# FedericoCos/PathTracer_GaussianSplatting

Hardware: AMD Instinct MI355X
Metric: Mrays/s (path trace) + Gsplats/s (3DGS) at 1920×1080, 1/2/4/8 MI355X (higher is better)
Workload: dtype f32; 1 GPU; C3 path trace: 250000-tri Sponza-like atrium, 1920x1080, 64 spp per GPU; width=1920, height=1080, spp_per_gpu=64, triangles=250000, bvh_nodes=58627, bvh_depth=13, bvh_build=host binned SAH, 113.1 ms, parallelism=single GPU

## Files before the change

include/ptgs/ptgs.h:

```cpp
#ifndef PTGS_H_
#define PTGS_H_

#include <stddef.h>
#include <stdint.h>

#ifdef __cplusplus
extern "C" {
#endif

#define PTGS_ABI_VERSION 4

#define PTGS_OK 0
#define PTGS_EINVAL (-1)
#define PTGS_EHIP (-2)
#define PTGS_ENOSCENE (-3)
#define PTGS_ERANGE (-4)
#define PTGS_EIO (-5)
#define PTGS_EINCOMPLETE (-6)
#define PTGS_EBADIDS (-7)


typedef struct ptgs_vertex {
    float pos[3];
    float pad1;
// ... 128 lines not shown
PTGS_AT(ptgs_material, uv_albedo, 144);
PTGS_AT(ptgs_material, emissive_factor_and_pad, 208);
PTGS_AT(ptgs_material, metallic_factor, 224);
PTGS_AT(ptgs_material, roughness_factor, 228);
PTGS_AT(ptgs_material, occlusion_strength, 232);
PTGS_AT(ptgs_material, specular_factor, 236);
PTGS_AT(ptgs_material, specular_color_factor, 240);
PTGS_AT(ptgs_material, alpha_cutoff, 252);
PTGS_AT(ptgs_material, transmission_factor, 256);
PTGS_AT(ptgs_material, clearcoat_factor, 260);
PTGS_AT(ptgs_material, clearcoat_roughness_factor, 264);
PTGS_AT(ptgs_material, pad, 268);
PTGS_AT(ptgs_material, albedo_texture_index, 272);
PTGS_AT(ptgs_material, normal_texture_index, 276);
PTGS_AT(ptgs_material, metallic_roughness_texture_index, 280);
PTGS_AT(ptgs_material, emissive_texture_index, 284);
PTGS_AT(ptgs_material, occlusion_texture_index, 288);
PTGS_AT(ptgs_material, clearcoat_texture_index, 292);
PTGS_AT(ptgs_material, clearcoat_roughness_texture_index, 296);
PTGS_AT(ptgs_material, sg_id, 300);
PTGS_AT(ptgs_material, use_specular_glossiness_workflow, 304);
PTGS_LAYOUT_ASSERT(sizeof(ptgs_ubo) == 192, "UniformBufferObject is 192 B");
PTGS_AT(ptgs_ubo, view, 0);
PTGS_AT(ptgs_ubo, proj, 64);
PTGS_AT(ptgs_ubo, camera_pos, 128);
PTGS_AT(ptgs_ubo, frame_count, 140);
PTGS_AT(ptgs_ubo, ambient_light, 144);
PTGS_AT(ptgs_ubo, emissive_flux, 160);
PTGS_AT(ptgs_ubo, punctual_flux, 164);
PTGS_AT(ptgs_ubo, total_flux, 168);
PTGS_AT(ptgs_ubo, p_emissive, 172);
PTGS_AT(ptgs_ubo, fov, 176);
PTGS_AT(ptgs_ubo, height, 180);
PTGS_AT(ptgs_ubo, use_lod, 184);
PTGS_AT(ptgs_ubo, lod_factor, 188);
PTGS_LAYOUT_ASSERT(sizeof(ptgs_punctual_light) == 64, "PunctualLight is 64 B");
PTGS_AT(ptgs_punctual_light, position, 0);
PTGS_AT(ptgs_punctual_light, intensity, 12);
PTGS_AT(ptgs_punctual_light, color, 16);
PTGS_AT(ptgs_punctual_light, range, 28);
PTGS_AT(ptgs_punctual_light, direction, 32);
PTGS_AT(ptgs_punctual_light, outer_cone_cos, 44);
PTGS_AT(ptgs_punctual_light, inner_cone_cos, 48);
PTGS_AT(ptgs_punctual_light, type, 52);
PTGS_AT(ptgs_punctual_light, padding, 56);
PTGS_LAYOUT_ASSERT(sizeof(ptgs_mesh_info) == 16, "MeshInfo is 16 B");
PTGS_AT(ptgs_mesh_info, material_index, 0);
PTGS_AT(ptgs_mesh_info, vertex_offset, 4);
PTGS_AT(ptgs_mesh_info, index_offset, 8);
PTGS_LAYOUT_ASSERT(sizeof(ptgs_light_triangle) == 16, "LightTriangle is 16 B");
PTGS_AT(ptgs_light_triangle, material_index, 12);
PTGS_LAYOUT_ASSERT(sizeof(ptgs_light_cdf) == 16, "LightCDF is 16 B");
PTGS_AT(ptgs_light_cdf, triangle_index, 4);
PTGS_LAYOUT_ASSERT(sizeof(ptgs_punctual_cdf) == 16, "PunctualLightCDF is 16 B");
PTGS_AT(ptgs_punctual_cdf, light_index, 4);
PTGS_LAYOUT_ASSERT(sizeof(ptgs_hitdata) == 48, "HitDataGPU is 48 B");
PTGS_AT(ptgs_hitdata, pos, 0);
PTGS_AT(ptgs_hitdata, flag, 12);
PTGS_AT(ptgs_hitdata, color, 16);
PTGS_AT(ptgs_hitdata, normal, 32);
PTGS_AT(ptgs_hitdata, padding, 44);
PTGS_LAYOUT_ASSERT(sizeof(ptgs_ray_sample) == 8, "RaySample is 8 B");
PTGS_LAYOUT_ASSERT(sizeof(ptgs_ray_push) == 80, "RayPushConstant / PC is 80 B");
PTGS_AT(ptgs_ray_push, model, 0);
PTGS_AT(ptgs_ray_push, mode, 64);
PTGS_AT(ptgs_ray_push, major_radius, 68);
PTGS_AT(ptgs_ray_push, minor_radius, 72);
PTGS_AT(ptgs_ray_push, height, 76);
#undef PTGS_AT


typedef struct ptgs_texture {
    const uint8_t* rgba8;
    uint32_t width;
    uint32_t height;
    uint32_t srgb;
    uint32_t reserved;
} ptgs_texture;

typedef struct ptgs_scene_desc {
    const ptgs_vertex* vertices;
    uint32_t num_vertices;
    const uint32_t* indices;
    uint32_t num_indices;
    const ptgs_mesh_info* meshes;
    const uint32_t* mesh_index_count;
    uint32_t num_meshes;
    const ptgs_material* materials;
    uint32_t num_materials;
    const ptgs_light_triangle* light_triangles;
    uint32_t num_light_triangles;
    const ptgs_light_cdf* light_cdf;
    uint32_t num_light_cdf;
    const ptgs_punctual_light* punctual_lights;
    uint32_t num_punctual_lights;
    const ptgs_punctual_cdf* punctual_cdf;
    uint32_t num_punctual_cdf;
    const float* blue_noise_rgba32f;
    uint32_t blue_noise_size;
    const ptgs_texture* textures;
    uint32_t num_textures;
} ptgs_scene_desc;

typedef struct ptgs_scene_info {
    uint32_t num_triangles;
    uint32_t num_bvh_nodes;
    uint32_t bvh_depth;
    uint32_t max_leaf_size;
    double build_ms;
    uint64_t device_bytes;
} ptgs_scene_info;


typedef struct ptgs_ctx ptgs_ctx;

int ptgs_create(int hip_device, ptgs_ctx** out);
void ptgs_destroy(ptgs_ctx* ctx);
const char* ptgs_last_error(const ptgs_ctx* ctx);
int ptgs_abi_version(void);
const char* ptgs_device_arch(void);

int ptgs_scene_upload(ptgs_ctx* ctx, const ptgs_scene_desc* desc);
int ptgs_scene_get_info(const ptgs_ctx* ctx, ptgs_scene_info* out);
typedef struct ptgs_bvh_buffers {
    const float* nodes;
    uint32_t num_nodes;
    const float* triangles;
    uint32_t num_triangles;
} ptgs_bvh_buffers;
int ptgs_scene_get_bvh(const ptgs_ctx* ctx, ptgs_bvh_buffers* out);
#define PTGS_BUILDER_HOST_SAH 0u
#define PTGS_BUILDER_GPU_SAH 1u
#define PTGS_BUILDER_GPU_LBVH 2u
typedef struct ptgs_scene_build {
    uint32_t builder;
    uint32_t leaf, fan;
    uint32_t depth_budget;
    uint32_t stack_need;
    uint32_t deep_stack;
} ptgs_scene_build;
int ptgs_scene_get_build(const ptgs_ctx* ctx, ptgs_scene_build* out);
typedef struct ptgs_scene_tree_opt {
    uint32_t applied;
    uint32_t num_nodes;
    uint32_t stack_need;
    uint32_t depth;
    uint32_t fan;
    uint32_t passes;
    double area_before;
    double area_after;
    double ms;
} ptgs_scene_tree_opt;
int ptgs_scene_get_tree_opt(const ptgs_ctx* ctx, ptgs_scene_tree_opt* out);


#define PTGS_ACCUM_RUNNING_MEAN 0u
#define PTGS_ACCUM_SUM 1u

int ptgs_trace_camera(ptgs_ctx* ctx, const ptgs_ubo* ubo, uint32_t width, uint32_t height,
                      float* accum_rgba32f, uint32_t spp, uint32_t frame_stride, uint32_t accum_mode,
                      void* hip_stream);

int ptgs_trace_camera_rows(ptgs_ctx* ctx, const ptgs_ubo* ubo, uint32_t width, uint32_t height,
                           uint32_t row_begin, uint32_t row_end, float* accum_rgba32f, uint32_t spp,
                           uint32_t frame_stride, uint32_t accum_mode, void* hip_stream);

int ptgs_trace_depth(ptgs_ctx* ctx, const ptgs_ubo* ubo, uint32_t width, uint32_t height, float* depth,
                     void* hip_stream);
int ptgs_trace_depth_rows(ptgs_ctx* ctx, const ptgs_ubo* ubo, uint32_t width, uint32_t height, uint32_t row_begin,
                          uint32_t row_end, float* depth, void* hip_stream);

int ptgs_trace_torus(ptgs_ctx* ctx, const ptgs_ubo* ubo, const ptgs_ray_push* push,
                     const ptgs_ray_sample* samples, uint32_t n, ptgs_hitdata* hits,
                     void* hip_stream);

typedef struct ptgs_trace_stats {
    uint64_t extension_rays;
    uint64_t shadow_rays;
    uint64_t samples;
    uint64_t node_visits;
    uint64_t tri_tests;
    uint64_t closest_hits;
} ptgs_trace_stats;

#define PTGS_FLAG_COUNT_TRAVERSAL 1u
#define PTGS_FLAG_TIME_STAGES 2u
#define PTGS_FLAG_GPU_BVH 4u
#define PTGS_FLAG_SPLAT_PUBLISH 8u
#define PTGS_FLAG_SPLAT_PUBLISH_TIGHT 64u
#define PTGS_FLAG_PT_WAVEFRONT 16u
#define PTGS_FLAG_GPU_LBVH 32u
#define PTGS_FLAG_SPLAT_OVERLAP 128u
int ptgs_set_flags(ptgs_ctx* ctx, uint32_t flags);
int ptgs_stats_reset(ptgs_ctx* ctx, void* hip_stream);
int ptgs_stats_read(ptgs_ctx* ctx, ptgs_trace_stats* out);


int ptgs_splat_points(ptgs_ctx* ctx, const ptgs_ubo* ubo, const ptgs_ray_push* push,
                      const ptgs_hitdata* hits, const ptgs_ray_sample* samples, uint32_t n,
                      uint32_t width, uint32_t height, uint32_t* rgba8_srgb, float* depth,
                      void* hip_stream);

typedef struct ptgs_gaussians {
    const float* means;
    const float* scales;
    const float* rotations;
    const float* opacities;
    const float* colors;
    uint32_t count;
    const uint32_t* ids;
    const float* chunk_bounds;
} ptgs_gaussians;

typedef struct ptgs_splat_stats {
    uint32_t num_rendered;
    uint32_t tiles_x, tiles_y;
    uint32_t num_visible;
    uint32_t fused;
} ptgs_splat_stats;

int ptgs_splat_gaussians(ptgs_ctx* ctx, const ptgs_gaussians* g, const ptgs_ubo* ubo,
                         uint32_t width, uint32_t height, const float bg[3],
                         uint32_t tile_row_begin, uint32_t tile_row_end, float* out_rgba32f,
                         ptgs_splat_stats* stats, void* hip_stream);

#define PTGS_MAX_VIEWS 8
int ptgs_splat_gaussians_views(ptgs_ctx* ctx, const ptgs_gaussians* g, uint32_t n_views, const ptgs_ubo* ubos,
                               uint32_t width, uint32_t height, const float bg[3], float* const* outs,
                               void* hip_stream);

int ptgs_gaussians_sort_spatial(ptgs_ctx* ctx, const ptgs_gaussians* g, float* means, float* scales, float* rotations,
                                float* opacities, float* colors, uint32_t* ids, void* hip_stream);

int ptgs_gaussians_chunk_bounds(ptgs_ctx* ctx, const ptgs_gaussians* g, float* bounds, void* hip_stream);

int ptgs_gaussians_sh_colors(ptgs_ctx* ctx, const float* means, const float* sh, uint32_t count,
                             uint32_t sh_degree, uint32_t active_degree, const float camera_pos[3],
                             float* colors, void* hip_stream);
int ptgs_gaussians_activate(ptgs_ctx* ctx, const float* log_scales, const float* opacity_logits,
                            uint32_t count, float* scales, float* opacities, void* hip_stream);
int ptgs_gaussians_sh_colors_backward(ptgs_ctx* ctx, const float* means, const float* sh, uint32_t count,
                                      uint32_t sh_degree, uint32_t active_degree, const float camera_pos[3],
                                      const float* dL_dcolors, float* dL_dsh, float* dL_dmeans, void* hip_stream);
int ptgs_gaussians_sh_colors_backward_eye(ptgs_ctx* ctx, const float* means, const float* sh, uint32_t count,
                                          uint32_t sh_degree, uint32_t active_degree, const float camera_pos[3],
                                          const float* dL_dcolors, float* dL_dsh, float* dL_dmeans,
                                          float* dL_dcamera_pos, void* hip_stream);
int ptgs_gaussians_activate_backward(ptgs_ctx* ctx, const float* scales, const float* opacities, uint32_t count,
                                     const float* dL_dscales, const float* dL_dopacities, float* dL_dlog_scales,
                                     float* dL_dlogits, void* hip_stream);
int ptgs_gaussians_permute_sh(ptgs_ctx* ctx, const float* sh, uint32_t sh_degree, const uint32_t* ids,
                              uint32_t count, float* out, void* hip_stream);

typedef struct ptgs_gaussian_grads {
    float* means;
    float* scales;
    float* rotations;
    float* opacities;
    float* colors;
    float* means2d;
    float* conics;
} ptgs_gaussian_grads;
int ptgs_splat_gaussians_backward(ptgs_ctx* ctx, const ptgs_gaussians* g, const ptgs_ubo* ubo,
                                  uint32_t width, uint32_t height, const float bg[3],
                                  const float* dL_dout_rgba32f, const ptgs_gaussian_grads* grads,
                                  void* hip_stream);

int ptgs_splat_gaussians_invdepth(ptgs_ctx* ctx, uint32_t width, uint32_t height, float* out_invdepth,
                                  void* hip_stream);
int ptgs_splat_gaussians_backward_depth(ptgs_ctx* ctx, const ptgs_gaussians* g, const ptgs_ubo* ubo,
                                        uint32_t width, uint32_t height, const float bg[3],
                                        const float* dL_dout_rgba32f, const float* dL_dinvdepth,
                                        const ptgs_gaussian_grads* grads, void* hip_stream);

int ptgs_splat_gaussians_backward_pose(ptgs_ctx* ctx, const ptgs_gaussians* g, const ptgs_ubo* ubo,
                                       uint32_t width, uint32_t height, const float bg[3],
                                       const float* dL_dout_rgba32f, const float* dL_dinvdepth,
                                       const ptgs_gaussian_grads* grads, float* dL_dview, void* hip_stream);

typedef struct ptgs_densify_params {
    float grad_threshold;
    float scale_split;
    float min_opacity;
    float max_scale;
    float max_screen_radius;
} ptgs_densify_params;
typedef struct ptgs_densify_counts {
    uint32_t survivors;
    uint32_t clones;
    uint32_t split_sources;
    uint32_t pruned_originals;
    uint32_t pruned_children;
    uint32_t total;
} ptgs_densify_counts;
typedef struct ptgs_densify_rows {
    const float* src;
    float* dst;
    uint32_t width;
    uint32_t zero_new;
} ptgs_densify_rows;
#define PTGS_DENSIFY_MAX_ROWS 16
int ptgs_densify_accumulate(ptgs_ctx* ctx, const float* g2d, const int32_t* radii, uint32_t n, uint32_t width,
                            uint32_t height, float* accum, float* denom, float* max_radii, void* hip_stream);
int ptgs_gaussians_densify_plan(ptgs_ctx* ctx, const float* scales, const float* opacities, const float* accum,
                                const float* denom, const float* max_radii, uint32_t n,
                                const ptgs_densify_params* params, ptgs_densify_counts* out, void* hip_stream);
// ... 128 lines not shown
```

pathtracer_gaussiansplatting_amd/_abi.py:

```python
from __future__ import annotations

import ctypes as C
import os

import numpy as np

ABI_VERSION = 4
_HERE = os.path.dirname(os.path.abspath(__file__))
LIB_PATH = os.path.join(_HERE, "libptgs.so")

PTGS_OK = 0
ERRORS = {-1: "PTGS_EINVAL", -2: "PTGS_EHIP", -3: "PTGS_ENOSCENE", -4: "PTGS_ERANGE", -5: "PTGS_EIO",
          -6: "PTGS_EINCOMPLETE", -7: "PTGS_EBADIDS"}
PTGS_EINVAL = -1
PTGS_EINCOMPLETE = -6
PTGS_EBADIDS = -7
ACCUM_RUNNING_MEAN = 0
ACCUM_SUM = 1
FLAG_COUNT_TRAVERSAL = 1
FLAG_TIME_STAGES = 2
FLAG_GPU_BVH = 4
FLAG_GPU_LBVH = 32
FLAG_SPLAT_PUBLISH = 8
FLAG_PT_WAVEFRONT = 16
# ... 47 lines not shown
                ("frame_count", C.c_uint32), ("ambient_light", C.c_float * 4), ("emissive_flux", C.c_float),
                ("punctual_flux", C.c_float), ("total_flux", C.c_float), ("p_emissive", C.c_float),
                ("fov", C.c_float), ("height", C.c_float), ("use_lod", C.c_float), ("lod_factor", C.c_float)]


class RayPush(C.Structure):
    _fields_ = [("model", C.c_float * 16), ("mode", C.c_int32), ("major_radius", C.c_float),
                ("minor_radius", C.c_float), ("height", C.c_float)]


class CaptureDesc(C.Structure):
    _fields_ = [("out_dir", C.c_char_p), ("width", C.c_uint32), ("height", C.c_uint32),
                ("total_positions", C.c_uint32), ("accumulation_steps", C.c_uint32), ("min_beta", C.c_float),
                ("max_beta", C.c_float), ("fov_deg", C.c_float), ("major_radius", C.c_float),
                ("torus_height", C.c_float), ("image_divisor", C.c_float), ("seed", C.c_uint32),
                ("capture_images", C.c_uint32), ("capture_pointcloud", C.c_uint32), ("ubo", C.c_void_p),
                ("torus", RayPush), ("samples", C.c_void_p), ("num_samples", C.c_uint32), ("hip_stream", C.c_void_p)]


class SceneDesc(C.Structure):
    _fields_ = [("vertices", C.c_void_p), ("num_vertices", C.c_uint32), ("indices", C.c_void_p),
                ("num_indices", C.c_uint32), ("meshes", C.c_void_p), ("mesh_index_count", C.c_void_p),
                ("num_meshes", C.c_uint32), ("materials", C.c_void_p), ("num_materials", C.c_uint32),
                ("light_triangles", C.c_void_p), ("num_light_triangles", C.c_uint32), ("light_cdf", C.c_void_p),
                ("num_light_cdf", C.c_uint32), ("punctual_lights", C.c_void_p), ("num_punctual_lights", C.c_uint32),
                ("punctual_cdf", C.c_void_p), ("num_punctual_cdf", C.c_uint32), ("blue_noise_rgba32f", C.c_void_p),
                ("blue_noise_size", C.c_uint32), ("textures", C.c_void_p), ("num_textures", C.c_uint32)]


class Texture(C.Structure):
    _fields_ = [("rgba8", C.c_void_p), ("width", C.c_uint32), ("height", C.c_uint32), ("srgb", C.c_uint32),
                ("reserved", C.c_uint32)]


class SceneSettings(C.Structure):
    _fields_ = [("ambient_light", C.c_float * 4), ("use_rt_box", C.c_int32), ("render_torus", C.c_int32),
                ("render_pointcloud", C.c_int32), ("torus_major_radius", C.c_float),
                ("torus_minor_radius", C.c_float), ("torus_height", C.c_float),
                ("torus_major_segments", C.c_int32), ("torus_minor_segments", C.c_int32),
                ("num_rays", C.c_uint32), ("use_lod", C.c_float), ("lod_factor", C.c_float),
                ("accumulation_steps", C.c_uint32), ("total_positions", C.c_uint32), ("min_beta", C.c_float),
                ("max_beta", C.c_float), ("image_divisor", C.c_float), ("capture_images", C.c_int32),
                ("capture_pointcloud", C.c_int32), ("num_objects", C.c_uint32)]


INGEST_MISSING_IMAGES_WHITE = 1


class SceneInfo(C.Structure):
    _fields_ = [("num_triangles", C.c_uint32), ("num_bvh_nodes", C.c_uint32), ("bvh_depth", C.c_uint32),
                ("max_leaf_size", C.c_uint32), ("build_ms", C.c_double), ("device_bytes", C.c_uint64)]


class TraceStats(C.Structure):
    _fields_ = [("extension_rays", C.c_uint64), ("shadow_rays", C.c_uint64), ("samples", C.c_uint64),
                ("node_visits", C.c_uint64), ("tri_tests", C.c_uint64), ("closest_hits", C.c_uint64)]


class Gaussians(C.Structure):
    _fields_ = [("means", C.c_void_p), ("scales", C.c_void_p), ("rotations", C.c_void_p),
                ("opacities", C.c_void_p), ("colors", C.c_void_p), ("count", C.c_uint32), ("ids", C.c_void_p),
                ("chunk_bounds", C.c_void_p)]


class GaussianGrads(C.Structure):
    _fields_ = [("means", C.c_void_p), ("scales", C.c_void_p), ("rotations", C.c_void_p),
                ("opacities", C.c_void_p), ("colors", C.c_void_p), ("means2d", C.c_void_p), ("conics", C.c_void_p)]


class DensifyParams(C.Structure):
    _fields_ = [("grad_threshold", C.c_float), ("scale_split", C.c_float), ("min_opacity", C.c_float),
                ("max_scale", C.c_float), ("max_screen_radius", C.c_float)]


class DensifyCounts(C.Structure):
    _fields_ = [("survivors", C.c_uint32), ("clones", C.c_uint32), ("split_sources", C.c_uint32),
                ("pruned_originals", C.c_uint32), ("pruned_children", C.c_uint32), ("total", C.c_uint32)]


class DensifyRows(C.Structure):
    _fields_ = [("src", C.c_void_p), ("dst", C.c_void_p), ("width", C.c_uint32), ("zero_new", C.c_uint32)]


DENSIFY_MAX_ROWS = 16


class AdamRows(C.Structure):
    _fields_ = [("param", C.c_void_p), ("grad", C.c_void_p), ("exp_avg", C.c_void_p), ("exp_avg_sq", C.c_void_p),
                ("width", C.c_uint32), ("head", C.c_uint32), ("lr", C.c_float), ("lr_head", C.c_float)]


class AdamParams(C.Structure):
    _fields_ = [("beta1", C.c_float), ("beta2", C.c_float), ("eps", C.c_float), ("step", C.c_uint32)]


ADAM_MAX_ROWS = 16


class SplatStats(C.Structure):
    _fields_ = [("num_rendered", C.c_uint32), ("tiles_x", C.c_uint32), ("tiles_y", C.c_uint32),
                ("num_visible", C.c_uint32), ("fused", C.c_uint32)]


class SplatStatus(C.Structure):
    _fields_ = [("frames", C.c_uint64), ("views", C.c_uint32 * 8), ("pair_capacity", C.c_uint32),
                ("last_pairs", C.c_uint32), ("touched_runs", C.c_uint32), ("fused", C.c_uint32),
                ("spilled_tiles", C.c_uint64), ("incomplete_tiles", C.c_uint64), ("spill_capacity", C.c_uint32),
                ("spill_demand", C.c_uint32)]


class SplatBuffers(C.Structure):
    _fields_ = [("radii", C.c_void_p), ("tiles_touched", C.c_void_p), ("sorted_keys", C.c_void_p),
                ("sorted_values", C.c_void_p), ("tile_ranges", C.c_void_p), ("means2d", C.c_void_p),
                ("depths", C.c_void_p), ("conic_opacity", C.c_void_p), ("num_gaussians", C.c_uint32),
                ("num_rendered", C.c_uint32), ("num_tiles", C.c_uint32)]


class BvhBuffers(C.Structure):
    _fields_ = [("nodes", C.c_void_p), ("num_nodes", C.c_uint32), ("triangles", C.c_void_p),
                ("num_triangles", C.c_uint32)]


BUILDER_HOST_SAH, BUILDER_GPU_SAH, BUILDER_GPU_LBVH = 0, 1, 2


class SceneBuild(C.Structure):
    _fields_ = [("builder", C.c_uint32), ("leaf", C.c_uint32), ("fan", C.c_uint32), ("depth_budget", C.c_uint32),
                ("stack_need", C.c_uint32), ("deep_stack", C.c_uint32)]


class SceneTreeOpt(C.Structure):
    _fields_ = [("applied", C.c_uint32), ("num_nodes", C.c_uint32), ("stack_need", C.c_uint32), ("depth", C.c_uint32),
                ("fan", C.c_uint32), ("passes", C.c_uint32), ("area_before", C.c_double), ("area_after", C.c_double),
                ("ms", C.c_double)]


assert C.sizeof(Ubo) == 192 and C.sizeof(RayPush) == 80

_P = C.c_void_p
_U = C.c_uint32
_I = C.c_int
_FP = C.POINTER(C.c_float)
SYMBOLS = {
    "ptgs_abi_version": (_I, []),
    "ptgs_device_arch": (C.c_char_p, []),
    "ptgs_create": (_I, [_I, C.POINTER(_P)]),
    "ptgs_destroy": (None, [_P]),
    "ptgs_last_error": (C.c_char_p, [_P]),
    "ptgs_scene_upload": (_I, [_P, C.POINTER(SceneDesc)]),
    "ptgs_scene_get_info": (_I, [_P, C.POINTER(SceneInfo)]),
    "ptgs_scene_get_bvh": (_I, [_P, C.POINTER(BvhBuffers)]),
    "ptgs_scene_get_build": (_I, [_P, C.POINTER(SceneBuild)]),
    "ptgs_scene_get_tree_opt": (_I, [_P, C.POINTER(SceneTreeOpt)]),
    "ptgs_trace_camera": (_I, [_P, C.POINTER(Ubo), _U, _U, _P, _U, _U, _U, _P]),
    "ptgs_trace_camera_rows": (_I, [_P, C.POINTER(Ubo), _U, _U, _U, _U, _P, _U, _U, _U, _P]),
    "ptgs_trace_torus": (_I, [_P, C.POINTER(Ubo), C.POINTER(RayPush), _P, _U, _P, _P]),
    "ptgs_trace_depth": (_I, [_P, C.POINTER(Ubo), _U, _U, _P, _P]),
    "ptgs_set_flags": (_I, [_P, _U]),
    "ptgs_stats_reset": (_I, [_P, _P]),
    "ptgs_stats_read": (_I, [_P, C.POINTER(TraceStats)]),
    "ptgs_splat_points": (_I, [_P, C.POINTER(Ubo), C.POINTER(RayPush), _P, _P, _U, _U, _U, _P, _P, _P]),
    "ptgs_splat_gaussians": (_I, [_P, C.POINTER(Gaussians), C.POINTER(Ubo), _U, _U, _FP, _U, _U, _P,
                                  C.POINTER(SplatStats), _P]),
    "ptgs_splat_gaussians_views": (_I, [_P, C.POINTER(Gaussians), _U, C.POINTER(Ubo), _U, _U, _FP,
                                        C.POINTER(C.c_void_p), _P]),
    "ptgs_splat_gaussians_over": (_I, [_P, C.POINTER(Gaussians), C.POINTER(Ubo), _U, _U, _P, _P, _U, _U, _P,
                                       C.POINTER(SplatStats), _P]),
    "ptgs_splat_get_buffers": (_I, [_P, C.POINTER(SplatBuffers)]),
    "ptgs_splat_get_tile_rows": (_I, [_P, C.POINTER(C.c_void_p), C.POINTER(C.c_uint32)]),
    "ptgs_splat_status_read": (_I, [_P, C.POINTER(SplatStatus), _P]),
    "ptgs_splat_reserve": (_I, [_P, _U]),
    "ptgs_gaussians_sort_spatial": (_I, [_P, C.POINTER(Gaussians), _P, _P, _P, _P, _P, _P, _P]),
    "ptgs_gaussians_chunk_bounds": (_I, [_P, C.POINTER(Gaussians), _P, _P]),
    "ptgs_gaussians_sh_colors": (_I, [_P, _P, _P, _U, _U, _U, _FP, _P, _P]),
    "ptgs_gaussians_activate": (_I, [_P, _P, _P, _U, _P, _P, _P]),
    "ptgs_gaussians_sh_colors_backward": (_I, [_P, _P, _P, _U, _U, _U, _FP, _P, _P, _P, _P]),
    "ptgs_gaussians_activate_backward": (_I, [_P, _P, _P, _U, _P, _P, _P, _P, _P]),
    "ptgs_gaussians_permute_sh": (_I, [_P, _P, _U, _P, _U, _P, _P]),
    "ptgs_splat_gaussians_backward": (_I, [_P, C.POINTER(Gaussians), C.POINTER(Ubo), _U, _U, _FP, _P,
                                           C.POINTER(GaussianGrads), _P]),
    "ptgs_splat_gaussians_invdepth": (_I, [_P, _U, _U, _P, _P]),
    "ptgs_splat_gaussians_backward_depth": (_I, [_P, C.POINTER(Gaussians), C.POINTER(Ubo), _U, _U, _FP, _P, _P,
                                                 C.POINTER(GaussianGrads), _P]),
    "ptgs_splat_gaussians_backward_pose": (_I, [_P, C.POINTER(Gaussians), C.POINTER(Ubo), _U, _U, _FP, _P, _P,
                                                C.POINTER(GaussianGrads), _P, _P]),
    "ptgs_gaussians_sh_colors_backward_eye": (_I, [_P, _P, _P, _U, _U, _U, _FP, _P, _P, _P, _P, _P]),
    "ptgs_densify_accumulate": (_I, [_P, _P, _P, _U, _U, _U, _P, _P, _P, _P]),
    "ptgs_gaussians_densify_plan": (_I, [_P, _P, _P, _P, _P, _P, _U, C.POINTER(DensifyParams),
                                         C.POINTER(DensifyCounts), _P]),
    "ptgs_gaussians_densify_apply": (_I, [_P, _U, _U, _P, _P, _P, _P, _P, _P, _P, C.POINTER(DensifyRows), _U, _P,
                                          _P]),
    "ptgs_image_loss_l1_dssim": (_I, [_P, _P, _P, _U, _U, _U, C.c_float, C.c_float, _P, _P, _P]),
    "ptgs_image_loss_invdepth_l1": (_I, [_P, _P, _P, _U, _U, C.c_float, C.c_float, _P, _P, _P]),
    "ptgs_gaussians_adam_step": (_I, [_P, _U, C.POINTER(AdamRows), _U, C.POINTER(AdamParams), _P, _P]),
    "ptgs_gaussians_opacity_reset": (_I, [_P, _P, _U, C.c_float, _P, _P, _P]),
    "ptgs_gaussians_checkpoint_init": (_I, [_P, _P, _P, _P, _U, _U, _P, _P, _P, _P]),
    "ptgs_image_mse": (_I, [_P, _P, _P, _U, _U, _U, _P, _P]),
    "ptgs_trace_depth_rows": (_I, [_P, C.POINTER(Ubo), _U, _U, _U, _U, _P, _P]),
    "ptgs_knn3_mean_dist2": (_I, [_P, _P, _U, _P, _P]),
    "ptgs_gaussians_from_points": (_I, [_P, _P, _P, _U, _P, _P, _P, _P, _P, _P]),
    "ptgs_comm_unique_id": (_I, [_P]),
    "ptgs_comm_create": (_I, [_P, _P, C.c_int, C.c_int]),
    "ptgs_comm_destroy": (_I, [_P]),
    "ptgs_reduce_radiance": (_I, [_P, _P, C.c_size_t, C.c_int, _P]),
    "ptgs_allreduce_radiance": (_I, [_P, _P, C.c_size_t, _P]),
    "ptgs_gather_rows": (_I, [_P, _P, C.c_uint32, C.c_uint32, _P, C.c_int, _P]),
    "ptgs_reduce_scatter_rows": (_I, [_P, _P, C.c_uint32, C.c_uint32, _P, _P]),
    "ptgs_splat_stage_ms": (_I, [_P, _FP]),
    "ptgs_encode_srgb8": (_I, [_P, _P, _U, _U, _P, _P]),
    "ptgs_device_alloc": (_I, [_P, C.c_size_t, C.POINTER(_P)]),
    "ptgs_device_free": (_I, [_P, _P]),
    "ptgs_memcpy_h2d": (_I, [_P, _P, _P, C.c_size_t]),
    "ptgs_memcpy_d2h": (_I, [_P, _P, _P, C.c_size_t]),
    "ptgs_memset_d32": (_I, [_P, _P, _U, C.c_size_t, _P]),
    "ptgs_synchronize": (_I, [_P]),
    "ptgs_camera_toroidal": (_I, [C.c_float] * 8 + [_FP, _FP, _FP]),
    "ptgs_camera_lookat": (_I, [_FP, _FP, _FP, _FP]),
    "ptgs_camera_perspective": (_I, [C.c_float] * 4 + [_FP]),
    "ptgs_mat4_inverse": (_I, [_FP, _FP]),
    "ptgs_mat4_inverse_glm": (_I, [_FP, _FP]),
    "ptgs_capture_poses": (_I, [_U, _U, C.c_float, C.c_float, _FP]),
    "ptgs_write_transforms_json": (_I, [C.c_char_p, C.c_float, C.c_float, _U, C.POINTER(C.c_char_p), _FP]),
    "ptgs_write_ply": (_I, [C.c_char_p, _P, _U, C.POINTER(C.c_uint32)]),
    "ptgs_write_jpeg": (_I, [C.c_char_p, _P, _U, _U, _U, C.c_int]),
    "ptgs_capture_dataset": (_I, [_P, _P]),
    "ptgs_builder_create": (_I, [C.POINTER(_P)]),
    "ptgs_builder_destroy": (None, [_P]),
    "ptgs_builder_add_rtbox_json": (_I, [_P, C.c_char_p]),
    "ptgs_builder_add_object": (_I, [_P, _P, _U, _P, _U, _P, _U, _P, _U, _P, _U, _U]),
    "ptgs_builder_finalize": (_I, [_P, C.POINTER(SceneDesc), C.POINTER(Ubo)]),
    "ptgs_builder_last_error": (C.c_char_p, [_P]),
    "ptgs_image_decode_rgba8": (_I, [_P, C.c_size_t, _P, C.c_size_t, C.POINTER(_U), C.POINTER(_U), C.POINTER(_U)]),
    "ptgs_read_ply": (_I, [C.c_char_p, _P, _P, _P, _U, C.POINTER(_U)]),
    "ptgs_read_gaussian_ply": (_I, [C.c_char_p, _P, _P, _P, _P, _P, _U, C.POINTER(_U), C.POINTER(_U)]),
    "ptgs_write_gaussian_ply": (_I, [C.c_char_p, _P, _P, _P, _P, _P, _U, _U]),
    "ptgs_generate_samples": (_I, [_I, _U, _P, _U, _P, _U, _U, _I, _P]),
    "ptgs_sort_samples": (_I, [_P, _U]),
    "ptgs_morton2d": (_U, [C.c_float, C.c_float]),
    "ptgs_builder_add_gltf": (_I, [_P, C.c_char_p, _FP, _FP, _FP, _U]),
    "ptgs_builder_add_punctual_light": (_I, [_P, _P]),
    "ptgs_builder_load_scene_json": (_I, [_P, C.c_char_p, C.c_char_p, _U, C.POINTER(SceneSettings)]),
}

_lib = None


class PtgsError(RuntimeError):
    def __init__(self, msg: str, code: int = 0):
        super().__init__(msg)
        self.code = code


def load_library(path: str | None = None) -> C.CDLL:
    global _lib
    if _lib is not None and path is None:
        return _lib
    p = path or LIB_PATH
    if not os.path.exists(p):
        raise PtgsError(f"native library not built: {p} (run pathtracer_gaussiansplatting_amd/build.py)")
    try:
        import torch
    except Exception:
        pass
    lib = C.CDLL(p, mode=C.RTLD_GLOBAL if path is None else C.RTLD_LOCAL)
    for name, (res, args) in SYMBOLS.items():
        fn = getattr(lib, name)
        fn.restype = res
        fn.argtypes = args
    v = lib.ptgs_abi_version()
    if v != ABI_VERSION:
        raise PtgsError(f"libptgs ABI version {v} != expected {ABI_VERSION}")
    if path is None:
        _lib = lib
    return lib


def check(rc: int, what: str, err: str = "") -> None:
    if rc != PTGS_OK:
        raise PtgsError(f"{what} failed: {ERRORS.get(rc, rc)} {err}", rc)


def fptr(a: np.ndarray):
    return a.ctypes.data_as(_FP)
```

pathtracer_gaussiansplatting_amd/csrc/api.cpp:

```cpp
#include <hip/hip_runtime.h>

#include <algorithm>
#include <chrono>
#include <cmath>
#include <cstdarg>
#include <cstdio>
#include <cstring>
#include <string>
#include <vector>

#include "../../include/ptgs/ptgs.h"
#include "bvh.h"
#include "bvh_gpu.h"
#include "bvh_opt.h"
#include "bvh_tries.h"
#include "knn.h"
#include "hostmath.h"
#include "pt_launch.h"
#include "pt_wavefront.h"
#include "scene_flatten.h"
#include "comm.h"
#include "dev_buf.h"
#include "splat.h"
#include "splat_adam.h"
#include "splat_adam_math.h"
#include "splat_backward.h"
#include "splat_densify.h"
#include "splat_frames.h"
#include "splat_loss.h"
#include "splat_sh.h"
#include "splat_train.h"
#include "textures.h"

using namespace ptgs;

static_assert(kSplatReportIncomplete == SPLAT_REPORT_INCOMPLETE && kSplatReportBadIds == SPLAT_REPORT_BAD_IDS,
              "splat_run.h names the bits of SplatReport");

struct ptgs_ctx {
  int device = 0;
  std::string err;
  uint32_t flags = 0;
  bool has_scene = false;
  DevScene dsc{};
  std::vector<void*> scene_allocs;
  ptgs_scene_info info{};
  ptgs_scene_build build{};
  ptgs_scene_tree_opt tree_opt{};
  unsigned long long* counters = nullptr;
  SplatFrames frames;
  DensifyWorkspace* densify = nullptr;
  LossWorkspace* loss = nullptr;
  ptgs::DevBuf sh_eye_partials;
  ptgs::DevBuf mse_partials;
  ptgs::WfWorkspace wf;
  ptgs::PtSched pt_sched;
  void* comm = nullptr;
  int comm_ranks = 0, comm_rank = 0;
};

namespace {

int fail(ptgs_ctx* c, int code, const char* fmt, ...) {
  char buf[512];
  va_list ap;
  va_start(ap, fmt);
  vsnprintf(buf, sizeof(buf), fmt, ap);
  va_end(ap);
  if (c) c->err = buf;
  return code;
}

#define HIPCHK(ctx, expr)                                                                   \
  do {                                                                                      \
    hipError_t e_ = (expr);                                                                 \
    if (e_ != hipSuccess) return fail(ctx, PTGS_EHIP, "%s: %s", #expr, hipGetErrorString(e_)); \
  } while (0)

int hip_rc(ptgs_ctx* c, hipError_t e, const char* what) {
  if (e != hipSuccess) return fail(c, PTGS_EHIP, "%s: %s", what, hipGetErrorString(e));
  return PTGS_OK;
}

int check_image_size(ptgs_ctx* c, uint32_t w, uint32_t h) {
  if (w == 0 || h == 0 || w > 32768 || h > 32768) return fail(c, PTGS_EINVAL, "bad image size %ux%u", w, h);
  return PTGS_OK;
}

int check_row_ranges(ptgs_ctx* c, const uint32_t* row_ranges, uint32_t height) {
  for (int g = 0; g < c->comm_ranks; ++g)
    if (row_ranges[2 * g] > row_ranges[2 * g + 1] || row_ranges[2 * g + 1] > height)
      return fail(c, PTGS_EINVAL, "bad row range of rank %d", g);
  return PTGS_OK;
}

void free_scene(ptgs_ctx* c) {
  for (void* p : c->scene_allocs) (void)hipFree(p);
  c->scene_allocs.clear();
  c->has_scene = false;
  c->dsc = DevScene{};
}

template <typename T>
int upload(ptgs_ctx* c, const T* src, size_t count, const T** dst) {
  if (count == 0) { *dst = nullptr; return PTGS_OK; }
  void* p = nullptr;
  HIPCHK(c, hipMalloc(&p, count * sizeof(T)));
  c->scene_allocs.push_back(p);
  HIPCHK(c, hipMemcpy(p, src, count * sizeof(T), hipMemcpyHostToDevice));
  c->info.device_bytes += count * sizeof(T);
  *dst = (const T*)p;
  return PTGS_OK;
}

bool is_device_ptr(const void* p) {
  if (!p) return false;
  hipPointerAttribute_t a;
  if (hipPointerGetAttributes(&a, p) != hipSuccess) { (void)hipGetLastError(); return false; }
  return a.type == hipMemoryTypeDevice || a.type == hipMemoryTypeManaged || a.devicePointer != nullptr;
}

int fill_cam(ptgs_ctx* c, const ptgs_ubo* ubo, CamParams& cp) {
  if (!inverse4(ubo->view, cp.inv_view)) return fail(c, PTGS_EINVAL, "ubo.view is singular");
  if (!inverse4(ubo->proj, cp.inv_proj)) return fail(c, PTGS_EINVAL, "ubo.proj is singular");
  for (int k = 0; k < 4; ++k) cp.ambient[k] = ubo->ambient_light[k];
  cp.emissive_flux = ubo->emissive_flux;
  cp.punctual_flux = ubo->punctual_flux;
  cp.p_emissive = ubo->p_emissive;
  cp.fov = ubo->fov;
  cp.win_height = ubo->height;
  cp.use_lod = ubo->use_lod;
  cp.lod_factor = ubo->lod_factor;
  return PTGS_OK;
}


void bvh_log(const char* how, const BvhTry& t, uint32_t depth, uint32_t need) {
  if (getenv("PTGS_BVH_LOG"))
    fprintf(stderr, "[ptgs] %s tree: leaf %d fan %d depth budget %u -> depth %u, stack need %u%s\n", how, t.leaf, t.fan,
            t.depth, depth, need, need >= PTGS_STACK ? (need < PTGS_STACK_TOTAL ? " (DEEP)" : " (does not fit)") : "");
}

double ms_between(std::chrono::steady_clock::time_point t0, std::chrono::steady_clock::time_point t1) {
  return std::chrono::duration<double, std::milli>(t1 - t0).count();
}

constexpr size_t kTriDeviceBytes = 3 * sizeof(float4) + sizeof(uint32_t);

struct HostSahBuilder {
  const std::vector<BuildTri>& tris;
  BvhOut bvh;
  std::vector<float> n4;
  uint32_t num4 = 0;
  BvhStep build(int leaf, uint32_t depth, uint32_t stack_lds) {
    build_bvh(tris, leaf, depth, bvh);
    return bvh.depth >= stack_lds ? BvhStep::TooDeep : BvhStep::Ok;
  }
  BvhStep collapse(int fan, uint32_t& need, uint32_t& depth4) {
    need = 0;
    collapse_bvh4(bvh.nodes, n4, num4, need, depth4, fan);
    return BvhStep::Ok;
  }
};

struct GpuTree {
  GpuBvh g;
  float4* n4 = nullptr;
  uint32_t num4 = 0;
  float ms = 0.0f;
  hipError_t err = hipSuccess;
  GpuTree() = default;
  GpuTree(const GpuTree&) = delete;
  GpuTree& operator=(const GpuTree&) = delete;
  ~GpuTree() {
    release_bvh2();
    (void)hipFree(n4);
  }
  void release_bvh2() {
    (void)hipFree(g.nodes);
    (void)hipFree(g.tris);
    (void)hipFree(g.tri_flags);
    g = GpuBvh{};
  }
  BvhStep step(hipError_t e) {
    err = e;
    return e == hipSuccess ? BvhStep::Ok : e == hipErrorNotSupported ? BvhStep::NotSupported : BvhStep::Error;
  }
  BvhStep collapse(int fan, uint32_t& need, uint32_t& depth4) {
    const auto t0 = std::chrono::steady_clock::now();
    (void)hipFree(n4);
    n4 = nullptr;
    const hipError_t e = collapse_bvh4_gpu(g.nodes, g.num_nodes, fan, &n4, &num4, &need, &depth4);
    ms += (float)ms_between(t0, std::chrono::steady_clock::now());
    return step(e);
  }
  void hand_over(std::vector<void*>& allocs, DevScene& s) {
    (void)hipFree(g.nodes);
    for (void* p : {(void*)n4, (void*)g.tris, (void*)g.tri_flags}) allocs.push_back(p);
    s.nodes = n4;
    s.tris = g.tris;
    s.tri_flags = g.tri_flags;
    n4 = nullptr;
    g = GpuBvh{};
  }
};
struct GpuSahBuilder : GpuTree {
  static constexpr uint32_t kId = PTGS_BUILDER_GPU_SAH;
  const std::vector<BuildTri>& tris;
  explicit GpuSahBuilder(const std::vector<BuildTri>& t) : tris(t) {}
  BvhStep build(int leaf, uint32_t depth, uint32_t) {
    release_bvh2();
    float bms = 0.0f;
    const hipError_t e = build_bvh_sah_gpu(tris, leaf, depth, g, &bms);
    ms += bms;
    return step(e);
  }
  uint32_t max_leaf() const { return g.max_leaf; }
};
struct GpuLbvhBuilder : GpuTree {
  static constexpr uint32_t kId = PTGS_BUILDER_GPU_LBVH;
  const std::vector<BuildTri>& tris;
  explicit GpuLbvhBuilder(const std::vector<BuildTri>& t) : tris(t) {}
  BvhStep build(int, uint32_t depth, uint32_t) {
    release_bvh2();
    float bms = 0.0f;
    const hipError_t e = build_bvh_gpu(tris, depth, g, &bms);
    ms += bms;
    return step(e);
  }
  uint32_t max_leaf() const { return 4u; }
};

void publish_tree(ptgs_ctx* c, DevScene& s, uint32_t builder, const BvhTriesResult& r, uint32_t num4, uint32_t max_leaf,
                  double build_ms) {
  s.deep_stack = r.need >= PTGS_STACK ? 1 : 0;
  c->info.num_bvh_nodes = num4;
  c->info.bvh_depth = r.depth4;
  c->info.max_leaf_size = max_leaf;
  c->info.build_ms = build_ms;
  c->build = ptgs_scene_build{builder, (uint32_t)r.kept.leaf, (uint32_t)r.kept.fan, r.kept.depth, r.need,
                              (uint32_t)s.deep_stack};
}

template <class Builder>
int build_tree_gpu(ptgs_ctx* c, const std::vector<BuildTri>& tris, const std::vector<BvhTry>& tries, DevScene& s,
                   bool* built) {
  Builder b(tris);
  const BvhTriesResult r =
      run_bvh_tries(b, tries, PTGS_STACK, PTGS_STACK_TOTAL,
                    [](const BvhTry& t, uint32_t depth4, uint32_t need) { bvh_log("GPU", t, depth4, need); });
  if (r.fit == BvhFit::Error) return fail(c, PTGS_EHIP, "GPU BVH build: %s", hipGetErrorString(b.err));
  if (r.fit != BvhFit::Fits) return PTGS_OK;
  publish_tree(c, s, Builder::kId, r, b.num4, b.max_leaf(), b.ms);
  c->info.device_bytes += (size_t)b.num4 * PTGS_NODE4_BYTES + tris.size() * kTriDeviceBytes;
  b.hand_over(c->scene_allocs, s);
  *built = true;
  return PTGS_OK;
}

int build_tree_host(ptgs_ctx* c, const std::vector<BuildTri>& tris, DevScene& s, std::vector<float>& host_n4) {
  const auto t0 = std::chrono::steady_clock::now();
  HostSahBuilder b{tris};
  const BvhTriesResult r =
      run_bvh_tries(b, parse_bvh_tries(getenv("PTGS_BVH_TRIES"), PTGS_STACK), PTGS_STACK, PTGS_STACK_TOTAL,
                    [](const BvhTry& t, uint32_t depth4, uint32_t need) { bvh_log("host", t, depth4, need); });
  const auto t1 = std::chrono::steady_clock::now();
  if (r.fit != BvhFit::Fits) return fail(c, PTGS_ERANGE, "BVH depth %u exceeds the traversal stack", b.bvh.depth);
  int rc;
  if ((rc = upload(c, (const float4*)b.n4.data(), b.n4.size() / 4, &s.nodes))) return rc;
  if ((rc = upload(c, (const float4*)b.bvh.tris.data(), b.bvh.tris.size() / 4, &s.tris))) return rc;
  if ((rc = upload(c, b.bvh.tri_flags.data(), b.bvh.tri_flags.size(), &s.tri_flags))) return rc;
  publish_tree(c, s, PTGS_BUILDER_HOST_SAH, r, b.num4, b.bvh.max_leaf, ms_between(t0, t1));
  host_n4.swap(b.n4);
  return PTGS_OK;
}

int check_node_window(ptgs_ctx* c) {
  const uint32_t limit = bvh_node_limit(getenv("PTGS_BVH_NODE_LIMIT"));
  if (c->info.num_bvh_nodes > limit)
    return fail(c, PTGS_ERANGE, "BVH of %u 4-wide nodes exceeds the traversal's 2 GiB node window (%u nodes)",
                c->info.num_bvh_nodes, limit);
  return PTGS_OK;
}

int upload_traversal_nodes(ptgs_ctx* c, std::vector<float>& host_n4, DevScene& s) {
  const size_t nf = (size_t)c->info.num_bvh_nodes * 32;
  if (host_n4.size() != nf) {
    host_n4.resize(nf);
    HIPCHK(c, hipMemcpy(host_n4.data(), s.nodes, nf * sizeof(float), hipMemcpyDeviceToHost));
  }
  int force = -1;
  if (const char* e = getenv("PTGS_PT_STACK_KEY_BITS")) force = std::max(0, atoi(e));
  bool optimise = c->build.builder != PTGS_BUILDER_GPU_LBVH;
  if (const char* e = getenv("PTGS_PT_TREE_OPT")) optimise = atoi(e) != 0;
  std::vector<uint32_t> n64;
  StackLayout sl;
  TreeOptInfo oi;
  if (!make_opt_traversal_nodes(host_n4.data(), c->info.num_bvh_nodes, (int)c->build.fan,
                                s.deep_stack ? PTGS_STACK_TOTAL : PTGS_STACK, optimise, force, n64, sl, oi))
    return fail(c, PTGS_ERANGE, "BVH node extents beyond the compact nodes' step range (2^-100 .. 2^100)");
  c->tree_opt = ptgs_scene_tree_opt{oi.applied, oi.num_nodes, oi.need, oi.depth, oi.fan, oi.passes,
                                    oi.area_before, oi.area_after, oi.ms};
  s.stk_key_mask = sl.key_mask;
  s.leaf_shift = sl.leaf_shift;
  s.leaf_start_mask = sl.leaf_start_mask;
  if (getenv("PTGS_BVH_LOG")) {
    if (optimise)
      fprintf(stderr, "[ptgs] traversal tree: %s in %.1f ms (%u passes): nodes %u -> %u, stack need %u -> %u, depth %u -> %u, "
              "fan %u, area sum %.3f -> %.3f\n", oi.applied ? "optimised" : "not applied", oi.ms, oi.passes,
              c->info.num_bvh_nodes, oi.num_nodes, c->build.stack_need, oi.need, c->info.bvh_depth, oi.depth, oi.fan,
              oi.area_before, oi.area_after);
    fprintf(stderr, "[ptgs] stack word:%u link bits, %u key bits (mask %08x), leaf shift %u\n", sl.ref_bits, sl.key_bits,
            sl.key_mask, sl.leaf_shift);
  }
  return upload(c, (const uint4*)n64.data(), n64.size() / 4, &s.nodes64);
}

int upload_scene_arrays(ptgs_ctx* c, const ptgs_scene_desc* d, const FlatScene& flat, const TexturePool& texpool,
                        DevScene& s) {
  int rc;
  ptgs_vertex dummy_v{};
  uint32_t dummy_i = 0;
  ptgs_mesh_info dummy_m{};
  if ((rc = upload(c, d->num_vertices ? d->vertices : &dummy_v, d->num_vertices ? d->num_vertices : 1, &s.vertices))) return rc;
  if ((rc = upload(c, d->num_indices ? d->indices : &dummy_i, d->num_indices ? d->num_indices : 1, &s.indices))) return rc;
  if ((rc = upload(c, d->num_meshes ? d->meshes : &dummy_m, d->num_meshes ? d->num_meshes : 1, &s.meshes))) return rc;
  if ((rc = upload(c, d->materials, d->num_materials, &s.materials))) return rc;
  const std::vector<uint32_t>& hitrec = flat.hitrec;
  const uint32_t zero4[4] = {0, 0, 0, 0};
  if ((rc = upload(c, (const uint4*)(hitrec.empty() ? zero4 : hitrec.data()), hitrec.empty() ? 1 : hitrec.size() / 4,
                   &s.hitrec)))
    return rc;
  if ((rc = upload(c, d->light_triangles, d->num_light_triangles, &s.light_tris))) return rc;
  if ((rc = upload(c, d->light_cdf, d->num_light_cdf, &s.light_cdf))) return rc;
  if ((rc = upload(c, d->punctual_lights, d->num_punctual_lights, &s.plights))) return rc;
  if ((rc = upload(c, d->punctual_cdf, d->num_punctual_cdf, &s.pcdf))) return rc;
  const size_t bn = d->blue_noise_size;
  if ((rc = upload(c, (const float4*)d->blue_noise_rgba32f, bn * bn, &s.blue_noise))) return rc;
  if ((rc = upload(c, texpool.texels.data(), texpool.texels.size(), &s.tex.texels))) return rc;
  if ((rc = upload(c, texpool.info.data(), texpool.info.size(), &s.tex.info))) return rc;
  return upload(c, texpool.lut.data(), texpool.lut.size(), &s.tex.lut);
}

void publish_scene(ptgs_ctx* c, const ptgs_scene_desc* d, const FlatScene& flat, DevScene& s) {
  s.tex.count = d->num_textures;
  s.uses_textures = 0;
  for (uint32_t i = 0; i < d->num_materials; ++i) {
    const ptgs_material& m = d->materials[i];
    if (m.albedo_texture_index > 0 || m.normal_texture_index > 0 || m.metallic_roughness_texture_index > 0 ||
        m.emissive_texture_index > 0 || m.clearcoat_texture_index > 0 || m.clearcoat_roughness_texture_index > 0 ||
        m.sg_id > 0)
      s.uses_textures = 1;
  }
  s.num_light_cdf = d->num_light_cdf;
  s.num_plights = d->num_punctual_lights;
  s.bn_size = (int32_t)d->blue_noise_size;
  s.has_transparent = flat.has_transparent ? 1 : 0;
  c->dsc = s;
  c->has_scene = true;
  c->info.num_triangles = (uint32_t)flat.tris.size();
}

}

extern "C" {

int ptgs_abi_version(void) { return PTGS_ABI_VERSION; }
const char* ptgs_device_arch(void) { return "gfx950"; }

int ptgs_create(int hip_device, ptgs_ctx** out) {
  if (!out) return PTGS_EINVAL;
  *out = nullptr;
  int n = 0;
  hipError_t e = hipGetDeviceCount(&n);
  if (e != hipSuccess || n == 0) return PTGS_EHIP;
  if (hip_device < 0 || hip_device >= n) return PTGS_EINVAL;
  ptgs_ctx* c = new ptgs_ctx();
  c->device = hip_device;
  if (hipSetDevice(hip_device) != hipSuccess) { delete c; return PTGS_EHIP; }
  if (hipMalloc(&c->counters, 8 * sizeof(unsigned long long)) != hipSuccess) { delete c; return PTGS_EHIP; }
  if (hipMemset(c->counters, 0, 8 * sizeof(unsigned long long)) != hipSuccess) { delete c; return PTGS_EHIP; }
  c->densify = densify_workspace_create();
  c->loss = loss_workspace_create();
  if (c->mse_partials.ensure(TRAIN_MSE_MAX_WG * sizeof(double), 0) != hipSuccess) {
    ptgs_destroy(c);
    return PTGS_EHIP;
  }
  *out = c;
  return PTGS_OK;
}

void ptgs_destroy(ptgs_ctx* c) {
  if (!c) return;
  (void)hipSetDevice(c->device);
  free_scene(c);
  if (c->counters) (void)hipFree(c->counters);
  ptgs::wf_workspace_free(c->wf);
  ptgs::free_pt_sched(c->pt_sched);
  densify_workspace_destroy(c->densify);
  loss_workspace_destroy(c->loss);
  if (c->comm) (void)comm_destroy(c->comm);
  delete c;
}

int ptgs_comm_unique_id(uint8_t id[PTGS_COMM_ID_BYTES]) {
  if (!id) return PTGS_EINVAL;
  if (!comm_available()) return PTGS_EHIP;
  return comm_unique_id(id) == 0 ? PTGS_OK : PTGS_EHIP;
}

int ptgs_comm_create(ptgs_ctx* c, const uint8_t id[PTGS_COMM_ID_BYTES], int nranks, int rank) {
  if (!c || !id) return PTGS_EINVAL;
  if (nranks < 1 || rank < 0 || rank >= nranks) return fail(c, PTGS_EINVAL, "bad rank %d of %d", rank, nranks);
  if (!comm_available()) return fail(c, PTGS_EHIP, "RCCL (librccl.so.1) could not be loaded");
  HIPCHK(c, hipSetDevice(c->device));
  if (c->comm) {
    (void)comm_destroy(c->comm);
    c->comm = nullptr;
  }
  int e = comm_create(id, nranks, rank, &c->comm);
  if (e) return fail(c, PTGS_EHIP, "ncclCommInitRank: %s", comm_error(e));
  c->comm_ranks = nranks;
  c->comm_rank = rank;
  return PTGS_OK;
}

int ptgs_comm_destroy(ptgs_ctx* c) {
  if (!c) return PTGS_EINVAL;
  if (c->comm) {
    int e = comm_destroy(c->comm);
    c->comm = nullptr;
    if (e) return fail(c, PTGS_EHIP, "ncclCommDestroy: %s", comm_error(e));
  }
  return PTGS_OK;
}

static int reduce_common(ptgs_ctx* c, float* accum, size_t n, int root, bool all, void* stream) {
  if (!c || !accum) return PTGS_EINVAL;
  if (!c->comm) return fail(c, PTGS_EINVAL, "no communicator (ptgs_comm_create)");
  if (!is_device_ptr(accum)) return fail(c, PTGS_EINVAL, "accum is not a device pointer");
  HIPCHK(c, hipSetDevice(c->device));
  int e = all ? comm_allreduce_sum(c->comm, accum, n, (hipStream_t)stream)
              : comm_reduce_sum(c->comm, accum, n, root, (hipStream_t)stream);
  if (e) return fail(c, PTGS_EHIP, "%s: %s", all ? "ncclAllReduce" : "ncclReduce", comm_error(e));
  return PTGS_OK;
}

int ptgs_reduce_radiance(ptgs_ctx* c, float* accum, size_t n_floats, int root, void* stream) {
  return reduce_common(c, accum, n_floats, root, false, stream);
}

int ptgs_allreduce_radiance(ptgs_ctx* c, float* accum, size_t n_floats, void* stream) {
  return reduce_common(c, accum, n_floats, 0, true, stream);
}

int ptgs_gather_rows(ptgs_ctx* c, float* image, uint32_t width, uint32_t height, const uint32_t* row_ranges,
                     int root, void* stream) {
  if (!c || !image || !row_ranges) return PTGS_EINVAL;
  if (!c->comm) return fail(c, PTGS_EINVAL, "no communicator (ptgs_comm_create)");
  if (root < 0 || root >= c->comm_ranks) return fail(c, PTGS_EINVAL, "bad root %d", root);
  if (!is_device_ptr(image)) return fail(c, PTGS_EINVAL, "image is not a device pointer");
  if (const int bad = check_row_ranges(c, row_ranges, height)) return bad;
  HIPCHK(c, hipSetDevice(c->device));
  int e = comm_gather_rows(c->comm, image, (size_t)width * 4u, row_ranges, c->comm_ranks, c->comm_rank, root,
                           (hipStream_t)stream);
  if (e) return fail(c, PTGS_EHIP, "ncclSend/ncclRecv: %s", comm_error(e));
  return PTGS_OK;
}

int ptgs_reduce_scatter_rows(ptgs_ctx* c, float* image, uint32_t width, uint32_t height, const uint32_t* row_ranges,
                             void* stream) {
  if (!c || !image || !row_ranges) return PTGS_EINVAL;
  if (!c->comm) return fail(c, PTGS_EINVAL, "no communicator (ptgs_comm_create)");
  if (!is_device_ptr(image)) return fail(c, PTGS_EINVAL, "image is not a device pointer");
  if (const int bad = check_row_ranges(c, row_ranges, height)) return bad;
  HIPCHK(c, hipSetDevice(c->device));
  int e = comm_reduce_rows(c->comm, image, (size_t)width * 4u, row_ranges, c->comm_ranks, (hipStream_t)stream);
  if (e) return fail(c, PTGS_EHIP, "ncclReduce: %s", comm_error(e));
  return PTGS_OK;
}

const char* ptgs_last_error(const ptgs_ctx* c) { return c ? c->err.c_str() : "null context"; }

int ptgs_scene_upload(ptgs_ctx* c, const ptgs_scene_desc* d) {
  if (!c || !d) return PTGS_EINVAL;
  HIPCHK(c, hipSetDevice(c->device));
  int rc;
  std::string msg;
  if ((rc = validate_scene_desc(d, msg))) return fail(c, rc, "%s", msg.c_str());
  TexturePool texpool;
  if (!build_texture_pool(d->textures, d->num_textures, texpool, msg)) return fail(c, PTGS_EINVAL, "%s", msg.c_str());
  if (texpool.texels.size() >= (1ull << 32)) return fail(c, PTGS_ERANGE, "texture pool exceeds 2^32 texels");
  FlatScene flat;
  if ((rc = flatten_scene(d, flat, msg))) return fail(c, rc, "%s", msg.c_str());

  free_scene(c);
  c->info = ptgs_scene_info{};
  c->build = ptgs_scene_build{};
  c->tree_opt = ptgs_scene_tree_opt{};
  DevScene s{};
  bool built = false;
  if ((c->flags & PTGS_FLAG_GPU_BVH) && flat.tris.size() >= 16) {
    rc = (c->flags & PTGS_FLAG_GPU_LBVH)
             ? build_tree_gpu<GpuLbvhBuilder>(c, flat.tris, lbvh_bvh_tries(PTGS_STACK), s, &built)
             : build_tree_gpu<GpuSahBuilder>(c, flat.tris, parse_bvh_tries(getenv("PTGS_BVH_TRIES"), PTGS_STACK), s,
                                             &built);
    if (rc) return rc;
  }
  std::vector<float> host_n4;
  if (!built && (rc = build_tree_host(c, flat.tris, s, host_n4))) return rc;
  if ((rc = check_node_window(c))) return rc;
  if ((rc = upload_traversal_nodes(c, host_n4, s))) return rc;
  if ((rc = upload_scene_arrays(c, d, flat, texpool, s))) return rc;
  publish_scene(c, d, flat, s);
  return PTGS_OK;
}

int ptgs_scene_get_info(const ptgs_ctx* c, ptgs_scene_info* out) {
  if (!c || !out) return PTGS_EINVAL;
  if (!c->has_scene) return PTGS_ENOSCENE;
  *out = c->info;
  return PTGS_OK;
}

int ptgs_scene_get_build(const ptgs_ctx* c, ptgs_scene_build* out) {
  if (!c || !out) return PTGS_EINVAL;
  if (!c->has_scene) return PTGS_ENOSCENE;
  *out = c->build;
  return PTGS_OK;
}

int ptgs_scene_get_tree_opt(const ptgs_ctx* c, ptgs_scene_tree_opt* out) {
  if (!c || !out) return PTGS_EINVAL;
  if (!c->has_scene) return PTGS_ENOSCENE;
  *out = c->tree_opt;
  return PTGS_OK;
}

int ptgs_scene_get_bvh(const ptgs_ctx* c, ptgs_bvh_buffers* out) {
  if (!c || !out) return PTGS_EINVAL;
  if (!c->has_scene) return PTGS_ENOSCENE;
  out->nodes = (const float*)c->dsc.nodes;
  out->num_nodes = c->info.num_bvh_nodes;
  out->triangles = (const float*)c->dsc.tris;
  out->num_triangles = c->info.num_triangles;
  return PTGS_OK;
}

int ptgs_trace_camera_rows(ptgs_ctx* c, const ptgs_ubo* ubo, uint32_t w, uint32_t h, uint32_t row_begin,
                           uint32_t row_end, float* accum, uint32_t spp, uint32_t frame_stride,
                           uint32_t accum_mode, void* stream) {
  if (!c || !ubo || !accum) return fail(c, PTGS_EINVAL, "null argument");
  if (!c->has_scene) return fail(c, PTGS_ENOSCENE, "no scene uploaded");
  if (const int bad = check_image_size(c, w, h)) return bad;
  if (row_end > h) row_end = h;
  if (row_begin > row_end) return fail(c, PTGS_EINVAL, "bad row range");
  if (frame_stride == 0) return fail(c, PTGS_EINVAL, "frame_stride must be >= 1");
  if (accum_mode > PTGS_ACCUM_SUM) return fail(c, PTGS_EINVAL, "bad accum mode");
  if (!is_device_ptr(accum)) return fail(c, PTGS_EINVAL, "accum is not a device pointer");
  HIPCHK(c, hipSetDevice(c->device));
  CamParams cp;
  int rc = fill_cam(c, ubo, cp);
  if (rc) return rc;
  const bool stats = (c->flags & PTGS_FLAG_COUNT_TRAVERSAL) != 0;
  hipError_t e;
  if (c->flags & PTGS_FLAG_PT_WAVEFRONT) {
    e = ptgs::launch_pt_wavefront(c->wf, c->dsc, cp, accum, w, h, row_begin, row_end, spp, ubo->frame_count,
                                  frame_stride, accum_mode, c->counters, stats, (hipStream_t)stream);
    return hip_rc(c, e, "wavefront path tracer");
  }
  e = launch_pt_camera(c->dsc, cp, accum, w, h, row_begin, row_end, spp, ubo->frame_count, frame_stride, accum_mode,
                       c->counters, stats, &c->pt_sched, (hipStream_t)stream);
  return hip_rc(c, e, "pt_camera launch");
}

int ptgs_trace_camera(ptgs_ctx* c, const ptgs_ubo* ubo, uint32_t w, uint32_t h, float* accum, uint32_t spp,
                      uint32_t frame_stride, uint32_t accum_mode, void* stream) {
  return ptgs_trace_camera_rows(c, ubo, w, h, 0, h, accum, spp, frame_stride, accum_mode, stream);
}

int ptgs_trace_depth(ptgs_ctx* c, const ptgs_ubo* ubo, uint32_t w, uint32_t h, float* depth, void* stream) {
  return ptgs_trace_depth_rows(c, ubo, w, h, 0, h, depth, stream);
}

int ptgs_trace_depth_rows(ptgs_ctx* c, const ptgs_ubo* ubo, uint32_t w, uint32_t h, uint32_t row_begin,
                          uint32_t row_end, float* depth, void* stream) {
  if (!c || !ubo || !depth) return fail(c, PTGS_EINVAL, "null argument");
  if (!c->has_scene) return fail(c, PTGS_ENOSCENE, "no scene uploaded");
  if (const int bad = check_image_size(c, w, h)) return bad;
  if (!is_device_ptr(depth)) return fail(c, PTGS_EINVAL, "depth is not a device pointer");
  HIPCHK(c, hipSetDevice(c->device));
  CamParams cp;
  int rc = fill_cam(c, ubo, cp);
  if (rc) return rc;
  ViewMat vm;
  std::memcpy(vm.m, ubo->view, sizeof(vm.m));
  hipError_t e = launch_pt_depth(c->dsc, cp, vm, depth, w, h, row_begin, row_end, ubo->frame_count, (hipStream_t)stream);
  return hip_rc(c, e, "pt_depth launch");
}

int ptgs_trace_torus(ptgs_ctx* c, const ptgs_ubo* ubo, const ptgs_ray_push* push, const ptgs_ray_sample* samples,
                     uint32_t n, ptgs_hitdata* hits, void* stream) {
  if (!c || !ubo || !push) return fail(c, PTGS_EINVAL, "null argument");
  if (!c->has_scene) return fail(c, PTGS_ENOSCENE, "no scene uploaded");
  if (n == 0) return PTGS_OK;
  if (!is_device_ptr(samples) || !is_device_ptr(hits)) return fail(c, PTGS_EINVAL, "samples/hits must be device pointers");
  HIPCHK(c, hipSetDevice(c->device));
  CamParams cp;
  int rc = fill_cam(c, ubo, cp);
  if (rc) return rc;
  TorusParams tp;
  std::memcpy(tp.model, push->model, sizeof(tp.model));
  tp.major_radius = push->major_radius;
  tp.minor_radius = push->minor_radius;
  tp.height = push->height;
  uint32_t side = (uint32_t)std::ceil(std::sqrt((double)n));
  while ((uint64_t)side * side < n) side++;
  hipError_t e = launch_pt_torus(c->dsc, cp, tp, samples, n, side, ubo->frame_count, hits, c->counters,
                                 (c->flags & PTGS_FLAG_COUNT_TRAVERSAL) != 0, (hipStream_t)stream);
  return hip_rc(c, e, "pt_torus launch");
}

int ptgs_set_flags(ptgs_ctx* c, uint32_t flags) {
  if (!c) return PTGS_EINVAL;
  c->flags = flags;
  return PTGS_OK;
}

int ptgs_stats_reset(ptgs_ctx* c, void* stream) {
  if (!c) return PTGS_EINVAL;
  HIPCHK(c, hipSetDevice(c->device));
  HIPCHK(c, hipMemsetAsync(c->counters, 0, 8 * sizeof(unsigned long long), (hipStream_t)stream));
  return PTGS_OK;
}

int ptgs_stats_read(ptgs_ctx* c, ptgs_trace_stats* out) {
  if (!c || !out) return PTGS_EINVAL;
  HIPCHK(c, hipSetDevice(c->device));
  HIPCHK(c, hipDeviceSynchronize());
  unsigned long long v[8];
  HIPCHK(c, hipMemcpy(v, c->counters, sizeof(v), hipMemcpyDeviceToHost));
  out->extension_rays = v[0];
  out->shadow_rays = v[1];
  out->samples = v[2];
  out->node_visits = v[3];
  out->tri_tests = v[4];
  out->closest_hits = v[5];
  return PTGS_OK;
}

int ptgs_device_alloc(ptgs_ctx* c, size_t bytes, void** out) {
  if (!c || !out) return PTGS_EINVAL;
  HIPCHK(c, hipSetDevice(c->device));
  HIPCHK(c, hipMalloc(out, bytes ? bytes : 16));
  return PTGS_OK;
}
int ptgs_device_free(ptgs_ctx* c, void* p) {
  if (!c) return PTGS_EINVAL;
  HIPCHK(c, hipFree(p));
  return PTGS_OK;
}
int ptgs_memcpy_h2d(ptgs_ctx* c, void* dst, const void* src, size_t bytes) {
  if (!c) return PTGS_EINVAL;
  HIPCHK(c, hipMemcpy(dst, src, bytes, hipMemcpyHostToDevice));
  return PTGS_OK;
}
int ptgs_memcpy_d2h(ptgs_ctx* c, void* dst, const void* src, size_t bytes) {
  if (!c) return PTGS_EINVAL;
  HIPCHK(c, hipMemcpy(dst, src, bytes, hipMemcpyDeviceToHost));
  return PTGS_OK;
}
int ptgs_memset_d32(ptgs_ctx* c, void* dst, uint32_t value, size_t count, void* stream) {
  if (!c) return PTGS_EINVAL;
  HIPCHK(c, hipMemsetD32Async((hipDeviceptr_t)dst, (int)value, count, (hipStream_t)stream));
  return PTGS_OK;
}
int ptgs_synchronize(ptgs_ctx* c) {
  if (!c) return PTGS_EINVAL;
  HIPCHK(c, hipDeviceSynchronize());
  return PTGS_OK;
}

}

#include "raster.h"

extern "C" {

// ... 767 lines not shown
```

pathtracer_gaussiansplatting_amd/csrc/bvh_opt.cpp:

```cpp
#include "bvh_opt.h"

#include <algorithm>
#include <chrono>
#include <cmath>
#include <cstring>
#include <limits>
#include <utility>

#include "bvh.h"

namespace ptgs {

namespace {

constexpr float kFar = 1e29f;

struct Node2 {
  float lo[3], hi[3];
  int32_t parent = -1;
  int32_t c[2] = {-1, -1};
  int32_t link = 0;
  bool leaf() const { return link < 0; }
};

// ... 20 lines not shown
  std::vector<double> area;
  int32_t root = -1;

  int32_t add(const Node2& x) {
    n.push_back(x);
    area.push_back(half_area(x.lo, x.hi));
    return (int32_t)n.size() - 1;
  }
  int32_t join(int32_t a, int32_t b) {
    Node2 x;
    for (int k = 0; k < 3; ++k) { x.lo[k] = std::min(n[a].lo[k], n[b].lo[k]); x.hi[k] = std::max(n[a].hi[k], n[b].hi[k]); }
    x.c[0] = a; x.c[1] = b;
    const int32_t i = add(x);
    n[a].parent = i; n[b].parent = i;
    return i;
  }
  void refit(int32_t x) {
    for (; x >= 0; x = n[x].parent) {
      Node2& p = n[x];
      const Node2 &a = n[p.c[0]], &b = n[p.c[1]];
      bool same = true;
      for (int k = 0; k < 3; ++k) {
        const float lo = std::min(a.lo[k], b.lo[k]), hi = std::max(a.hi[k], b.hi[k]);
        same = same && lo == p.lo[k] && hi == p.hi[k];
        p.lo[k] = lo; p.hi[k] = hi;
      }
      if (same) return;
      area[x] = half_area(p.lo, p.hi);
    }
  }
  void replace_child(int32_t parent, int32_t was, int32_t now) {
    if (parent < 0) root = now;
    else n[parent].c[n[parent].c[0] == was ? 0 : 1] = now;
    n[now].parent = parent;
  }
};

struct Binarise {
  const float* n4;
  uint32_t num;
  Tree2& t;
  std::vector<uint8_t> seen;
  bool ok = true;

  int32_t node(uint32_t i, uint32_t depth) {
    if (i >= num || seen[i] || depth > 4096) { ok = false; return -1; }
    seen[i] = 1;
    const float* f = n4 + 32 * (size_t)i;
    int32_t e[4];
    int cnt = 0;
    for (int j = 0; j < 4 && ok; ++j) {
      int32_t link;
      std::memcpy(&link, &f[24 + j], 4);
      if (link == 0) continue;
      if (link < 0) {
        if (!real_box(f, j)) { ok = false; break; }
        Node2 x;
        for (int a = 0; a < 3; ++a) { x.lo[a] = f[(2 * a) * 4 + j]; x.hi[a] = f[(2 * a + 1) * 4 + j]; }
        x.link = link;
        e[cnt++] = t.add(x);
      } else {
        e[cnt++] = node((uint32_t)link, depth + 1);
      }
    }
    if (!ok || cnt < 2) { ok = false; return -1; }
    while (cnt > 1) {
      int ba = 0, bb = 1;
      double best = std::numeric_limits<double>::infinity();
      for (int a = 0; a < cnt; ++a)
        for (int b = a + 1; b < cnt; ++b) {
          const double u = union_area(t.n[e[a]], t.n[e[b]]);
          if (u < best) { best = u; ba = a; bb = b; }
        }
      e[ba] = t.join(e[ba], e[bb]);
      for (int k = bb; k + 1 < cnt; ++k) e[k] = e[k + 1];
      --cnt;
    }
    return e[0];
  }
};

typedef std::pair<double, int32_t> Cand;

void reinsertion_pass(Tree2& t, std::vector<Cand>& heap) {
  std::vector<int32_t> order;
  order.reserve(t.n.size());
  for (int32_t i = 0; i < (int32_t)t.n.size(); ++i)
    if (i != t.root) order.push_back(i);
  std::sort(order.begin(), order.end(), [&](int32_t a, int32_t b) {
    return t.area[a] != t.area[b] ? t.area[a] > t.area[b] : a < b;
  });
  for (const int32_t x : order) {
    const int32_t p = t.n[x].parent;
    if (x == t.root || p == t.root) continue;
    const int32_t g = t.n[p].parent;
    const int32_t s = t.n[p].c[t.n[p].c[0] == x ? 1 : 0];
    t.replace_child(g, p, s);
    t.refit(g);
    const double ax = t.area[x];
    double best = union_area(t.n[s], t.n[x]);
    for (int32_t a = g; a >= 0; a = t.n[a].parent) best += union_area(t.n[a], t.n[x]) - t.area[a];
    int32_t at = s;
    heap.clear();
    heap.push_back(Cand(0.0, t.root));
    while (!heap.empty()) {
      std::pop_heap(heap.begin(), heap.end(), std::greater<Cand>());
      const Cand c = heap.back();
      heap.pop_back();
      if (c.first + ax >= best) break;
      const Node2& y = t.n[c.second];
      const double cost = c.first + union_area(y, t.n[x]);
      if (cost < best) { best = cost; at = c.second; }
      const double below = cost - t.area[c.second];
      if (!y.leaf() && below + ax < best)
        for (int k = 0; k < 2; ++k) {
          heap.push_back(Cand(below, y.c[k]));
          std::push_heap(heap.begin(), heap.end(), std::greater<Cand>());
        }
    }
    t.replace_child(t.n[at].parent, at, p);
    t.n[p].c[0] = at; t.n[p].c[1] = x;
    t.n[at].parent = p; t.n[x].parent = p;
    for (int k = 0; k < 3; ++k) { t.n[p].lo[k] = 1.0f; t.n[p].hi[k] = 0.0f; }
    t.refit(p);
  }
}

void emit_bvh2(const Tree2& t, std::vector<float>& n2) {
  std::vector<int32_t> queue;
  queue.push_back(t.root);
  std::vector<int32_t> index(t.n.size(), -1);
  index[t.root] = 0;
  for (size_t q = 0; q < queue.size(); ++q)
    for (int k = 0; k < 2; ++k) {
      const int32_t c = t.n[queue[q]].c[k];
      if (t.n[c].leaf()) continue;
      index[c] = (int32_t)queue.size();
      queue.push_back(c);
    }
  n2.assign(queue.size() * 16, 0.0f);
  for (size_t q = 0; q < queue.size(); ++q) {
    float* f = &n2[16 * q];
    const Node2& p = t.n[queue[q]];
    for (int k = 0; k < 2; ++k) {
      const Node2& c = t.n[p.c[k]];
      f[4 * k + 0] = c.lo[0]; f[4 * k + 1] = c.hi[0]; f[4 * k + 2] = c.lo[1]; f[4 * k + 3] = c.hi[1];
      f[8 + 2 * k] = c.lo[2]; f[9 + 2 * k] = c.hi[2];
      const int32_t link = c.leaf() ? c.link : index[p.c[k]];
      std::memcpy(&f[12 + k], &link, 4);
    }
  }
}

}

double bvh4_area_sum(const float* n4, uint32_t num) {
  double sum = 0.0, root = 0.0;
  for (uint32_t i = 0; i < num; ++i) {
    const float* f = n4 + 32 * (size_t)i;
    float lo[3] = {1.0f, 1.0f, 1.0f}, hi[3] = {0.0f, 0.0f, 0.0f};
    bool any = false;
    for (int j = 0; j < 4; ++j) {
      int32_t link;
      std::memcpy(&link, &f[24 + j], 4);
      if (link == 0 || !real_box(f, j)) continue;
      for (int a = 0; a < 3; ++a) {
        const float l = f[(2 * a) * 4 + j], h = f[(2 * a + 1) * 4 + j];
        lo[a] = any ? std::min(lo[a], l) : l;
        hi[a] = any ? std::max(hi[a], h) : h;
      }
      any = true;
    }
    const double a = any ? half_area(lo, hi) : 0.0;
    if (i == 0) root = a;
    sum += a;
  }
  return root > 0.0 ? sum / root : 0.0;
}

bool optimize_bvh4(const float* n4, uint32_t num, int fan, uint32_t need_limit, std::vector<float>& out,
                   TreeOptInfo& info, int passes) {
  const auto t0 = std::chrono::steady_clock::now();
  info = TreeOptInfo{};
  out.clear();
  info.area_before = bvh4_area_sum(n4, num);
  auto done = [&](bool applied) {
    info.applied = applied ? 1u : 0u;
    if (!applied) out.clear();
    info.ms = std::chrono::duration<double, std::milli>(std::chrono::steady_clock::now() - t0).count();
    return applied;
  };
  if (num == 0) return done(false);
  Tree2 t;
  t.n.reserve((size_t)num * 8);
  t.area.reserve((size_t)num * 8);
  Binarise b{n4, num, t, std::vector<uint8_t>(num, 0)};
  t.root = b.node(0, 0);
  if (!b.ok) return done(false);
  std::vector<Cand> heap;
  for (int p = 0; p < passes; ++p) reinsertion_pass(t, heap);
  info.passes = (uint32_t)std::max(0, passes);
  std::vector<float> n2;
  emit_bvh2(t, n2);
  for (int f = std::max(2, std::min(4, fan)); f >= 2; --f) {
    uint32_t num4 = 0, need = 0, depth4 = 0;
    collapse_bvh4(n2, out, num4, need, depth4, f);
    if (need >= need_limit) continue;
    info.num_nodes = num4;
    info.need = need;
    info.depth = depth4;
    info.fan = (uint32_t)f;
    info.area_after = bvh4_area_sum(out.data(), num4);
    return done(true);
  }
  return done(false);
}

bool make_opt_traversal_nodes(const float* n4, uint32_t num, int fan, uint32_t need_limit, bool optimise,
                              int force_key_bits, std::vector<uint32_t>& n64, StackLayout& layout, TreeOptInfo& info,
                              std::vector<float>* walked) {
  info = TreeOptInfo{};
  std::vector<float> opt;
  if (optimise && optimize_bvh4(n4, num, fan, need_limit, opt, info)) {
    if (make_traversal_nodes(opt.data(), info.num_nodes, force_key_bits, n64, layout)) {
      if (walked) walked->swap(opt);
      return true;
    }
    info.applied = 0;
  }
  if (!optimise) info.area_before = bvh4_area_sum(n4, num);
  if (walked) walked->assign(n4, n4 + (size_t)num * 32);
  return make_traversal_nodes(n4, num, force_key_bits, n64, layout);
}

}
```

pathtracer_gaussiansplatting_amd/csrc/bvh_opt.h:

```cpp
#pragma once

#include <stdint.h>
#include <vector>

#include "bvh.h"

namespace ptgs {

constexpr int kTreeOptPasses = 2;

struct TreeOptInfo {
  uint32_t applied = 0;
  uint32_t num_nodes = 0;
  uint32_t need = 0;
  uint32_t depth = 0;
  uint32_t fan = 0;
  uint32_t passes = 0;
  double area_before = 0.0;
  double area_after = 0.0;
  double ms = 0.0;
};

double bvh4_area_sum(const float* nodes4, uint32_t num_nodes);

bool optimize_bvh4(const float* nodes4, uint32_t num_nodes, int fan, uint32_t need_limit, std::vector<float>& out,
                   TreeOptInfo& info, int passes = kTreeOptPasses);

bool make_opt_traversal_nodes(const float* nodes4, uint32_t num_nodes, int fan, uint32_t need_limit, bool optimise,
                              int force_key_bits, std::vector<uint32_t>& nodes64, StackLayout& layout, TreeOptInfo& info,
                              std::vector<float>* walked = nullptr);

}
```

pathtracer_gaussiansplatting_amd/csrc/pt_device.h:

```cpp
#pragma once

#include <hip/hip_runtime.h>
#include "detmath.h"
#include "texture.h"
#include "stack_key.h"
#include "../../include/ptgs/ptgs.h"

namespace ptgs {

struct DevScene {
  const float4* nodes;
  const uint4* nodes64;
  const float4* tris;
  const uint32_t* tri_flags;
  const ptgs_vertex* vertices;
  const uint32_t* indices;
  const ptgs_mesh_info* meshes;
  const ptgs_material* materials;
  const uint4* hitrec;
  const ptgs_light_triangle* light_tris;
  const ptgs_light_cdf* light_cdf;
  const ptgs_punctual_light* plights;
  const ptgs_punctual_cdf* pcdf;
  const float4* blue_noise;
  DevTextures tex;
  int32_t uses_textures;
  int32_t deep_stack;
  uint32_t num_light_cdf;
  uint32_t num_plights;
  int32_t bn_size;
  int32_t has_transparent;
  uint32_t stk_key_mask;
  uint32_t leaf_shift;
  uint32_t leaf_start_mask;
};

struct CamParams {
  float inv_view[16];
  float inv_proj[16];
  float ambient[4];
  float emissive_flux, punctual_flux, p_emissive;
  float fov, win_height, use_lod, lod_factor;
};

struct Hit {
  float t, u, v;
  uint32_t gid;
  uint32_t slot;
};

struct TraversalCounters {
  uint32_t nodes;
  uint32_t tris;
  uint32_t hits;
#ifdef PT_LANES
  struct PtLaneCounts* lanes_p;
#endif
};

enum PtLoop { PT_L_NODE = 0, PT_L_LEAF, PT_L_TRI, PT_L_ANY_NODE, PT_L_ANY_TRI, PT_L_BOUNCE, PT_L_SAMPLE, PT_L_COUNT };
#ifdef PT_LANES
__device__ unsigned long long g_pt_lanes[2 * PT_L_COUNT];
struct PtLaneCounts {
  uint32_t w[PT_L_COUNT], l[PT_L_COUNT];
};
__device__ __forceinline__ void pt_lane_tick(PtLaneCounts& c, int i) {
  const unsigned long long ex = __builtin_amdgcn_read_exec();
  c.l[i] += 1u;
  if (__lane_id() == (uint32_t)__builtin_ctzll(ex)) c.w[i] += 1u;
}
__device__ __forceinline__ void pt_lanes_flush(const PtLaneCounts& c) {
  for (int i = 0; i < PT_L_COUNT; ++i) {
    atomicAdd(&g_pt_lanes[2 * i], (unsigned long long)c.w[i]);
    atomicAdd(&g_pt_lanes[2 * i + 1], (unsigned long long)c.l[i]);
  }
}
#define PT_LANE_TICK(cnt, i) pt_lane_tick(*(cnt).lanes_p, (i))
#define PT_LANES_INIT(tc) PtLaneCounts tc##_lanes = {}; (tc).lanes_p = &tc##_lanes
#define PT_LANES_FLUSH(tc) pt_lanes_flush(tc##_lanes)
#else
#define PT_LANE_TICK(cnt, i) ((void)0)
#define PT_LANES_INIT(tc) ((void)0)
#define PT_LANES_FLUSH(tc) ((void)0)
#endif

#ifndef PTGS_STACK
#define PTGS_STACK 39
#endif
#ifndef PTGS_STACK_OVF
#define PTGS_STACK_OVF 9
#endif
#define PTGS_STACK_TOTAL (PTGS_STACK + PTGS_STACK_OVF)
#define PTGS_BLOCK 256

PTGS_HD float i2f(int x) { union { int i; float f; } c; c.i = x; return c.f; }
__device__ __forceinline__ int f2i(float x) { return __float_as_int(x); }
__device__ __forceinline__ uint32_t f2u(float x) { return __float_as_uint(x); }

__device__ __forceinline__ float rnd(uint32_t& state) {
  uint32_t prev = state;
  state = prev * 747796405u + 2891336453u;
  uint32_t word = ((state >> ((state >> 28u) + 4u)) ^ state) * 277803737u;
  return (float)((word >> 22u) ^ word) / 4294967296.0f;
}

__device__ __forceinline__ float alpha_hash(uint32_t seed, uint32_t gid) {
  uint32_t s = seed ^ (gid * 0x9E3779B9u);
  return rnd(s);
}

__device__ __forceinline__ v3 ld3(const float* p) { return mk3(p[0], p[1], p[2]); }

#ifndef PTGS_PT_NEARFAR
#define PTGS_PT_NEARFAR 1
#endif
#ifndef PTGS_PT_ASM_MIN
#define PTGS_PT_ASM_MIN 1
#endif

struct Ray {
  v3 o, d, inv;
  v3 oinv;
  float tmin, tmax;
#if PTGS_PT_NEARFAR
  uint32_t nx, ny, nz;
#endif
};

__device__ __forceinline__ float safe_inv(float d) {
  const float eps = 1e-20f;
  float a = absx(d) < eps ? (d < 0.0f ? -eps : eps) : d;
  return 1.0f / a;
}

__device__ __forceinline__ Ray make_ray(v3 o, v3 d, float tmin, float tmax) {
  Ray r; r.o = o; r.d = d; r.tmin = tmin; r.tmax = tmax;
  r.inv = mk3(safe_inv(d.x), safe_inv(d.y), safe_inv(d.z));
  r.oinv = mk3(o.x * r.inv.x, o.y * r.inv.y, o.z * r.inv.z);
#if PTGS_PT_NEARFAR
  r.nx = r.inv.x < 0.0f ? 16u : 0u;
  r.ny = r.inv.y < 0.0f ? 48u : 32u;
  r.nz = r.inv.z < 0.0f ? 80u : 64u;
#endif
  return r;
}

__device__ __forceinline__ bool tri_isect(const Ray& r, v3 v0, v3 e1, v3 e2, float& t, float& u, float& v) {
  v3 pvec = cross3(r.d, e2);
  float det = dot3(e1, pvec);
  if (det == 0.0f) return false;
  float inv_det = 1.0f / det;
  v3 tvec = r.o - v0;
  u = dot3(tvec, pvec) * inv_det;
  if (u < 0.0f || u > 1.0f) return false;
  v3 qvec = cross3(tvec, e1);
  v = dot3(r.d, qvec) * inv_det;
  if (v < 0.0f || u + v > 1.0f) return false;
  t = dot3(e2, qvec) * inv_det;
  return true;
}

template <bool TEX>
__device__ __forceinline__ bool anyhit_accept(const DevScene& sc, uint32_t mesh, uint32_t prim, float u, float v,
                                              uint32_t seed, uint32_t gid) {
  const ptgs_mesh_info info = sc.meshes[mesh];
  const ptgs_material& m = sc.materials[info.material_index];
  float alpha_cutoff = m.alpha_cutoff;
  bool is_blend = m.pad > 0.5f;
  if (alpha_cutoff == 0.0f && !is_blend) return true;
  float alpha = m.base_color_factor[3];
  if (TEX && m.albedo_texture_index > 0) {
    const uint32_t i0 = sc.indices[info.index_offset + prim * 3u + 0u];
    const uint32_t i1 = sc.indices[info.index_offset + prim * 3u + 1u];
    const uint32_t i2 = sc.indices[info.index_offset + prim * 3u + 2u];
    const ptgs_vertex& v0 = sc.vertices[info.vertex_offset + i0];
    const ptgs_vertex& v1 = sc.vertices[info.vertex_offset + i1];
    const ptgs_vertex& v2 = sc.vertices[info.vertex_offset + i2];
    const float bx = (1.0f - u) - v;
    const float tu = (v0.tex_coord[0] * bx + v1.tex_coord[0] * u) + v2.tex_coord[0] * v;
    const float tv = (v0.tex_coord[1] * bx + v1.tex_coord[1] * u) + v2.tex_coord[1] * v;
    alpha = alpha * sample_texture(sc.tex, m.albedo_texture_index, tu, tv, 0.0f).w;
  }
  if (alpha_cutoff > 0.0f) return !(alpha < alpha_cutoff);
  return !(alpha_hash(seed, gid) > alpha);
}

__device__ __noinline__ bool anyhit_accept_call(const DevScene& sc, uint32_t mesh, uint32_t prim, float u, float v,
                                                uint32_t seed, uint32_t gid) {
  return anyhit_accept<true>(sc, mesh, prim, u, v, seed, gid);
}

template <bool PK>
__device__ __forceinline__ void leaf_range(const DevScene& sc, int leaf, uint32_t& start, uint32_t& count) {
  if (PK) {
    start = (uint32_t)leaf & sc.leaf_start_mask;
    count = (((uint32_t)leaf & 0x7fffffffu) >> sc.leaf_shift) + 1u;
  } else {
    const uint32_t L = (uint32_t)(~leaf);
    start = L & 0x07ffffffu;
    count = (L >> 27) + 1u;
  }
}

template <bool STATS, bool TEX, bool AH_CALL = false, bool PK = false>
__device__ __forceinline__ void leaf_closest(const DevScene& sc, const Ray& r, int leaf, Hit& h,
                                             uint32_t seed, TraversalCounters& cnt) {
  uint32_t start, count;
  leaf_range<PK>(sc, leaf, start, count);
  float4 na = sc.tris[3u * start], nb = sc.tris[3u * start + 1u], nc = sc.tris[3u * start + 2u];
  for (uint32_t k = 0; k < count; ++k) {
    PT_LANE_TICK(cnt, PT_L_TRI);
    float4 a = na, b = nb, c = nc;
    asm volatile("" : "+v"(a.x), "+v"(a.y), "+v"(a.z), "+v"(a.w), "+v"(b.x), "+v"(b.y), "+v"(b.z), "+v"(b.w),
                      "+v"(c.x), "+v"(c.y), "+v"(c.z), "+v"(c.w));
    if (k + 1 < count) {
      const float4* tn = sc.tris + 3u * (start + k + 1u);
      na = tn[0]; nb = tn[1]; nc = tn[2];
    }
    if (STATS) cnt.tris++;
    float t, u, v;
    if (!tri_isect(r, mk3(a.x, a.y, a.z), mk3(b.x, b.y, b.z), mk3(c.x, c.y, c.z), t, u, v)) continue;
    if (!(t >= r.tmin && t <= h.t)) continue;
    uint32_t gid = f2u(c.w);
    if (t == h.t && gid >= h.gid) continue;
    if (sc.has_transparent && (sc.tri_flags[start + k] & 1u)) {
      const bool acc = (AH_CALL && TEX) ? anyhit_accept_call(sc, f2u(a.w), f2u(b.w), u, v, seed, gid)
                                        : anyhit_accept<TEX>(sc, f2u(a.w), f2u(b.w), u, v, seed, gid);
      if (!acc) continue;
    }
    h.t = t; h.u = u; h.v = v; h.gid = gid; h.slot = start + k;
  }
}

struct Box4 {
  float tn[4];
  int c[4];
  unsigned long long hm[4];
};
#if PTGS_PT_NEARFAR
__device__ __forceinline__ float4 node_ld(__amdgpu_buffer_rsrc_t rs, uint32_t off) {
  typedef unsigned int u4 __attribute__((ext_vector_type(4)));
  const u4 v = __builtin_amdgcn_raw_buffer_load_b128(rs, (int)off, 0, 0);
  return make_float4(__uint_as_float(v.x), __uint_as_float(v.y), __uint_as_float(v.z), __uint_as_float(v.w));
}
__device__ __forceinline__ void box4(const Ray& r, const DevScene& sc, int node, float tcap, Box4& o) {
// ... 41 lines not shown
#pragma unroll
  for (int j = 0; j < 4; ++j) {
    const float x0 = __builtin_fmaf(LX[j], r.inv.x, -r.oinv.x), x1 = __builtin_fmaf(HX[j], r.inv.x, -r.oinv.x);
    const float y0 = __builtin_fmaf(LY[j], r.inv.y, -r.oinv.y), y1 = __builtin_fmaf(HY[j], r.inv.y, -r.oinv.y);
    const float z0 = __builtin_fmaf(LZ[j], r.inv.z, -r.oinv.z), z1 = __builtin_fmaf(HZ[j], r.inv.z, -r.oinv.z);
    const float tn = fmaxf(fmaxf(fminf(x0, x1), fminf(y0, y1)), fmaxf(fminf(z0, z1), r.tmin));
    const float tf = fminf(fminf(fmaxf(x0, x1), fmaxf(y0, y1)), fminf(fmaxf(z0, z1), tcap));
    const bool h = tn <= tf * 1.0000004f;
    o.tn[j] = h ? tn : __builtin_huge_valf();
    o.c[j] = f2i(CH[j]);
    o.hm[j] = __builtin_amdgcn_ballot_w64(h);
  }
}
#endif
#ifndef PTGS_PT_NODE64
#define PTGS_PT_NODE64 1
#endif
#ifndef PTGS_PT_NODE64_PIN
#define PTGS_PT_NODE64_PIN 1
#endif
#ifndef PTGS_PT_PK_SLAB
#define PTGS_PT_PK_SLAB 0
#endif
#ifndef PTGS_PT_PK_SLAB_MUL
#define PTGS_PT_PK_SLAB_MUL 1
#endif
template <bool N64>
__device__ __forceinline__ Ray node64_ray(const Ray& r) {
  Ray q = r;
  if (N64 && PTGS_PT_NODE64_PIN) asm volatile("" : "+v"(q.oinv.x), "+v"(q.oinv.y), "+v"(q.oinv.z));
  return q;
}
__device__ __forceinline__ float node64_q(uint32_t w, int j) { return (float)((w >> (8 * j)) & 0xffu); }
__device__ __forceinline__ void box4_q(const Ray& r, const DevScene& sc, int node, float tcap, Box4& o) {
  typedef unsigned int u4 __attribute__((ext_vector_type(4)));
  const __amdgpu_buffer_rsrc_t rs = __builtin_amdgcn_make_buffer_rsrc((void*)sc.nodes64, 0, 0x7fffffff, 0x00020000);
  const uint32_t base = (uint32_t)node << 6;
  const u4 a = __builtin_amdgcn_raw_buffer_load_b128(rs, (int)base, 0, 0);
  const u4 b = __builtin_amdgcn_raw_buffer_load_b128(rs, (int)(base + 16u), 0, 0);
  const u4 p = __builtin_amdgcn_raw_buffer_load_b128(rs, (int)(base + 32u), 0, 0);
  u4 ch = __builtin_amdgcn_raw_buffer_load_b128(rs, (int)(base + 48u), 0, 0);
  asm volatile("" : "+v"(ch.x), "+v"(ch.y), "+v"(ch.z), "+v"(ch.w));
  const float sx = __uint_as_float(a.w) * r.inv.x, sy = __uint_as_float(b.x) * r.inv.y, sz = __uint_as_float(b.y) * r.inv.z;
  const float cx = __builtin_fmaf(__uint_as_float(a.x), r.inv.x, -r.oinv.x);
  const float cy = __builtin_fmaf(__uint_as_float(a.y), r.inv.y, -r.oinv.y);
  const float cz = __builtin_fmaf(__uint_as_float(a.z), r.inv.z, -r.oinv.z);
#if PTGS_PT_NEARFAR
  const bool gx = (r.nx & 16u) != 0u, gy = (r.ny & 16u) != 0u, gz = (r.nz & 16u) != 0u;
#else
  const bool gx = r.inv.x < 0.0f, gy = r.inv.y < 0.0f, gz = r.inv.z < 0.0f;
#endif
  const uint32_t nX = gx ? b.w : b.z, fX = gx ? b.z : b.w;
  const uint32_t nY = gy ? p.y : p.x, fY = gy ? p.x : p.y;
  const uint32_t nZ = gz ? p.w : p.z, fZ = gz ? p.z : p.w;
  const uint32_t CH[4] = {ch.x, ch.y, ch.z, ch.w};
#if PTGS_PT_PK_SLAB
  typedef float f2 __attribute__((ext_vector_type(2)));
  const f2 SX = {sx, sx}, SY = {sy, sy}, SZ = {sz, sz}, CX = {cx, cx}, CY = {cy, cy}, CZ = {cz, cz};
  float TN[4], TF[4];
#pragma unroll
  for (int j = 0; j < 4; ++j) {
    const f2 qx = {node64_q(nX, j), node64_q(fX, j)}, qy = {node64_q(nY, j), node64_q(fY, j)};
    const f2 qz = {node64_q(nZ, j), node64_q(fZ, j)};
    const f2 x = __builtin_elementwise_fma(qx, SX, CX);
    const f2 y = __builtin_elementwise_fma(qy, SY, CY);
    const f2 z = __builtin_elementwise_fma(qz, SZ, CZ);
    TN[j] = fmaxf(fmaxf(x.x, y.x), fmaxf(z.x, r.tmin));
#if PTGS_PT_ASM_MIN
    float tf;
    asm("v_min3_f32 %0, %1, %2, %3" : "=v"(tf) : "v"(x.y), "v"(y.y), "v"(z.y));
    asm("v_min_f32 %0, %1, %2" : "=v"(tf) : "v"(tf), "v"(tcap));
    TF[j] = tf;
#else
    TF[j] = fminf(fminf(x.y, y.y), fminf(z.y, tcap));
#endif
  }
#if PTGS_PT_PK_SLAB_MUL
  const f2 K = {1.0000004f, 1.0000004f};
  const f2 f01 = (f2){TF[0], TF[1]} * K, f23 = (f2){TF[2], TF[3]} * K;
  const float TFK[4] = {f01.x, f01.y, f23.x, f23.y};
#else
  const float TFK[4] = {TF[0] * 1.0000004f, TF[1] * 1.0000004f, TF[2] * 1.0000004f, TF[3] * 1.0000004f};
#endif
#pragma unroll
  for (int j = 0; j < 4; ++j) {
    unsigned long long hm = __builtin_amdgcn_ballot_w64(TN[j] <= TFK[j]);
    if (j >= 2) hm &= __builtin_amdgcn_ballot_w64(CH[j] != 0u);
    o.tn[j] = __builtin_amdgcn_inverse_ballot_w64(hm) ? TN[j] : __builtin_huge_valf();
    o.c[j] = (int)CH[j];
    o.hm[j] = hm;
  }
#else
#pragma unroll
  for (int j = 0; j < 4; ++j) {
    const float x0 = __builtin_fmaf(node64_q(nX, j), sx, cx), x1 = __builtin_fmaf(node64_q(fX, j), sx, cx);
    const float y0 = __builtin_fmaf(node64_q(nY, j), sy, cy), y1 = __builtin_fmaf(node64_q(fY, j), sy, cy);
    const float z0 = __builtin_fmaf(node64_q(nZ, j), sz, cz), z1 = __builtin_fmaf(node64_q(fZ, j), sz, cz);
    const float tn = fmaxf(fmaxf(x0, y0), fmaxf(z0, r.tmin));
#if PTGS_PT_ASM_MIN
    float tf;
    asm("v_min3_f32 %0, %1, %2, %3" : "=v"(tf) : "v"(x1), "v"(y1), "v"(z1));
    asm("v_min_f32 %0, %1, %2" : "=v"(tf) : "v"(tf), "v"(tcap));
#else
    const float tf = fminf(fminf(x1, y1), fminf(z1, tcap));
#endif
    unsigned long long hm = __builtin_amdgcn_ballot_w64(tn <= tf * 1.0000004f);
    if (j >= 2) hm &= __builtin_amdgcn_ballot_w64(CH[j] != 0u);
    o.tn[j] = __builtin_amdgcn_inverse_ballot_w64(hm) ? tn : __builtin_huge_valf();
    o.c[j] = (int)CH[j];
    o.hm[j] = hm;
  }
#endif
}
template <bool N64>
__device__ __forceinline__ void box4_sel(const Ray& r, const DevScene& sc, int node, float tcap, Box4& o) {
  if (N64) box4_q(r, sc, node, tcap, o);
  else box4(r, sc, node, tcap, o);
}
__device__ __forceinline__ void cswap4(Box4& b, int i, int j) {
  const bool sw = b.tn[j] < b.tn[i];
  const float ti = b.tn[i], tj = b.tn[j];
  const int ci = b.c[i], cj = b.c[j];
  b.tn[i] = sw ? tj : ti; b.tn[j] = sw ? ti : tj;
  b.c[i] = sw ? cj : ci; b.c[j] = sw ? ci : cj;
}
template <typename Push>
__device__ __forceinline__ int enter_box4_hit(Box4& b, Push push) {
  const unsigned long long h0 = b.hm[0], h1 = b.hm[1], h2 = b.hm[2], h3 = b.hm[3];
  cswap4(b, 0, 1); cswap4(b, 2, 3); cswap4(b, 0, 2); cswap4(b, 1, 3); cswap4(b, 1, 2);
  const unsigned long long a01 = h0 & h1, o01 = h0 | h1, a23 = h2 & h3, o23 = h2 | h3;
  if (__builtin_amdgcn_inverse_ballot_w64(a01 & a23)) push(b.c[3], b.tn[3]);
  if (__builtin_amdgcn_inverse_ballot_w64((a01 & o23) | (o01 & a23))) push(b.c[2], b.tn[2]);
  if (__builtin_amdgcn_inverse_ballot_w64(a01 | a23 | (o01 & o23))) push(b.c[1], b.tn[1]);
  return b.c[0];
}
template <typename Push, typename Pop>
__device__ __forceinline__ int enter_box4(Box4& b, Push push, Pop pop) {
  if (!__builtin_amdgcn_inverse_ballot_w64(b.hm[0] | b.hm[1] | b.hm[2] | b.hm[3])) return pop();
  return enter_box4_hit(b, push);
}

#ifndef PTGS_PT_STACK_CULL
#define PTGS_PT_STACK_CULL 1
#endif
#ifndef PTGS_PT_ONE_POP
#define PTGS_PT_ONE_POP 0
#endif
#ifndef PTGS_PT_ULOOP
#define PTGS_PT_ULOOP 1
#endif
#ifndef PTGS_PT_ULOOP_ANY
#define PTGS_PT_ULOOP_ANY PTGS_PT_ULOOP
#endif
template <bool STATS, bool TEX, int SS = PTGS_BLOCK, int OVF = PTGS_STACK_OVF, bool N64 = false, bool CULL = false>
__device__ __forceinline__ Hit trace_closest(const DevScene& sc, const Ray& r, uint32_t seed, int* stack,
                                             TraversalCounters& cnt) {
  static_assert(!CULL || N64, "the distance key needs the compact nodes' packed links");
  Hit h; h.t = r.tmax; h.u = 0.f; h.v = 0.f; h.gid = 0xffffffffu; h.slot = 0;
  const Ray rq = node64_ray<N64>(r);
  int sp = 0;
  int node = 0;
  const uint32_t kmask = sc.stk_key_mask;
  const int DONE = CULL ? (int)(0x7fffffffu & ~kmask) : 0x7fffffff;
  int leaf = DONE;
  int ovf[OVF > 0 ? OVF : 1];
  auto push = [&](int c, float tn) {
    const int x = CULL ? (int)stack_pack((uint32_t)c, tn, kmask) : c;
    if (OVF == 0 || sp < PTGS_STACK) stack[sp * SS] = x;
    else ovf[sp - PTGS_STACK] = x;
    ++sp;
  };
  auto pop = [&]() -> int {
    if (!CULL) {
      if (!sp) return DONE;
      --sp;
      return (OVF == 0 || sp < PTGS_STACK) ? stack[sp * SS] : ovf[sp - PTGS_STACK];
    }
    const float cap = h.t * 1.0000004f;
    uint32_t x;
    do {
      x = (uint32_t)DONE;
      if (sp) {
        --sp;
        x = (uint32_t)((OVF == 0 || sp < PTGS_STACK) ? stack[sp * SS] : ovf[sp - PTGS_STACK]);
      }
    } while (stack_bound(x, kmask) > cap);
    return (int)stack_link(x, kmask);
  };
  auto pop_park = [&]() -> int {
    const float cap = h.t * 1.0000004f;
    int n;
    bool again;
    do {
      uint32_t x = (uint32_t)DONE;
      if (sp) {
        --sp;
        x = (uint32_t)((OVF == 0 || sp < PTGS_STACK) ? stack[sp * SS] : ovf[sp - PTGS_STACK]);
      }
      n = CULL ? (int)stack_link(x, kmask) : (int)x;
      again = CULL && stack_bound(x, kmask) > cap;
      if (!again && n < 0 && leaf == DONE) {
        leaf = n;
        again = true;
      }
    } while (again);
    return n;
  };
  for (;;) {
#if PTGS_PT_ULOOP
    while ((uint32_t)node < (uint32_t)DONE) {
#else
    while (node >= 0 && node != DONE) {
#endif
      PT_LANE_TICK(cnt, PT_L_NODE);
      Box4 b;
      box4_sel<N64>(rq, sc, node, h.t, b);
      if (STATS) cnt.nodes += 4;
#if PTGS_PT_ONE_POP
      bool need = !__builtin_amdgcn_inverse_ballot_w64(b.hm[0] | b.hm[1] | b.hm[2] | b.hm[3]);
      if (!need) {
        node = enter_box4_hit(b, push);
        if (node < 0 && leaf == DONE) {
          leaf = node;
          need = true;
        }
      }
      if (need) node = PTGS_PT_ONE_POP == 1 ? pop_park() : pop();
#else
      node = enter_box4(b, push, pop);
      if (node < 0 && leaf == DONE) {
        leaf = node;
        node = pop();
      }
#endif
#if PTGS_PT_ONE_POP == 2
      if ((__builtin_amdgcn_ballot_w64(leaf != DONE) | __builtin_amdgcn_ballot_w64((uint32_t)node >= (uint32_t)DONE)) ==
          __builtin_amdgcn_read_exec())
        break;
#else
      if ((__builtin_amdgcn_ballot_w64(leaf != DONE) | __builtin_amdgcn_ballot_w64(node == DONE)) ==
          __builtin_amdgcn_read_exec())
        break;
#endif
    }
    if (leaf != DONE) {
      PT_LANE_TICK(cnt, PT_L_LEAF);
      leaf_closest<STATS, TEX, false, N64>(sc, r, leaf, h, seed, cnt);
      leaf = DONE;
    }
    if (node < 0) {
      leaf_closest<STATS, TEX, false, N64>(sc, r, node, h, seed, cnt);
      node = pop();
    }
    if (node == DONE) return h;
  }
}

#ifndef PTGS_PT_ANY_SINGLE_EXIT
#define PTGS_PT_ANY_SINGLE_EXIT 1
#endif
#ifndef PTGS_PT_ANY_PARK
#define PTGS_PT_ANY_PARK 0
#endif
#ifndef PTGS_PT_ANY_TRI_FOLD
#define PTGS_PT_ANY_TRI_FOLD 1
#endif
#ifndef PTGS_PT_ANY_TRI_PREFETCH
#define PTGS_PT_ANY_TRI_PREFETCH 0
#endif
template <bool STATS, bool TEX, bool PK>
__device__ __forceinline__ bool leaf_any(const DevScene& sc, const Ray& r, int leaf, uint32_t seed,
                                         TraversalCounters& cnt) {
  uint32_t start, count;
  leaf_range<PK>(sc, leaf, start, count);
  bool occ = false;
#if PTGS_PT_ANY_TRI_PREFETCH
  float4 na = sc.tris[3u * start], nb = sc.tris[3u * start + 1u], nc = sc.tris[3u * start + 2u];
#endif
  for (uint32_t k = 0; k < count && !occ; ++k) {
    PT_LANE_TICK(cnt, PT_L_ANY_TRI);
#if PTGS_PT_ANY_TRI_PREFETCH
    float4 a = na, bb = nb, c = nc;
    asm volatile("" : "+v"(a.x), "+v"(a.y), "+v"(a.z), "+v"(a.w), "+v"(bb.x), "+v"(bb.y), "+v"(bb.z), "+v"(bb.w),
                      "+v"(c.x), "+v"(c.y), "+v"(c.z), "+v"(c.w));
    if (k + 1 < count) {
      const float4* tn = sc.tris + 3u * (start + k + 1u);
      na = tn[0]; nb = tn[1]; nc = tn[2];
    }
#else
    const float4* tp = sc.tris + 3u * (start + k);
    float4 a = tp[0], bb = tp[1], c = tp[2];
#endif
    if (STATS) cnt.tris++;
#if PTGS_PT_ANY_TRI_FOLD
    const v3 e1 = mk3(bb.x, bb.y, bb.z), e2 = mk3(c.x, c.y, c.z);
    const v3 pvec = cross3(r.d, e2);
    const float det = dot3(e1, pvec);
    const float inv_det = 1.0f / det;
    const v3 tvec = r.o - mk3(a.x, a.y, a.z);
    const float u = dot3(tvec, pvec) * inv_det;
    const v3 qvec = cross3(tvec, e1);
    const float v = dot3(r.d, qvec) * inv_det;
    const float t = dot3(e2, qvec) * inv_det;
    bool hit = (det != 0.0f) & !(u < 0.0f) & !(u > 1.0f) & !(v < 0.0f) & !(u + v > 1.0f) & (t >= r.tmin) & (t <= r.tmax);
#else
    float t, u, v;
    bool hit = tri_isect(r, mk3(a.x, a.y, a.z), mk3(bb.x, bb.y, bb.z), mk3(c.x, c.y, c.z), t, u, v);
    hit = hit && t >= r.tmin && t <= r.tmax;
#endif
    if (hit && sc.has_transparent && (sc.tri_flags[start + k] & 1u))
      hit = anyhit_accept<TEX>(sc, f2u(a.w), f2u(bb.w), u, v, seed, f2u(c.w));
    occ = hit;
  }
  return occ;
}

template <bool STATS, bool TEX, int SS = PTGS_BLOCK, int OVF = PTGS_STACK_OVF, bool N64 = false>
__device__ __forceinline__ bool trace_any(const DevScene& sc, const Ray& r, uint32_t seed, int* stack,
                                          TraversalCounters& cnt) {
  const Ray rq = node64_ray<N64>(r);
  int sp = 0;
  int node = 0;
  int ovf[OVF > 0 ? OVF : 1];
#if PTGS_PT_ANY_SINGLE_EXIT
  const int DONE = 0x7fffffff;
  bool occluded = false;
  auto push = [&](int c) {
    if (OVF == 0 || sp < PTGS_STACK) stack[sp * SS] = c;
    else ovf[sp - PTGS_STACK] = c;
    ++sp;
  };
  auto pop = [&]() -> int {
    if (!sp) return DONE;
    --sp;
    return (OVF == 0 || sp < PTGS_STACK) ? stack[sp * SS] : ovf[sp - PTGS_STACK];
  };
  int leaf = DONE;
  for (;;) {
#if PTGS_PT_ULOOP_ANY
    while ((uint32_t)node < (uint32_t)DONE) {
#else
    while (node >= 0 && node != DONE) {
#endif
      PT_LANE_TICK(cnt, PT_L_ANY_NODE);
      Box4 b;
      box4_sel<N64>(rq, sc, node, r.tmax, b);
      if (STATS) cnt.nodes += 4;
      const unsigned long long h0 = b.hm[0], h1 = b.hm[1], h2 = b.hm[2], h3 = b.hm[3];
      const unsigned long long o01 = h0 | h1, o012 = o01 | h2;
      if (__builtin_amdgcn_inverse_ballot_w64(o012 | h3)) {
        if (__builtin_amdgcn_inverse_ballot_w64(h0 & h1)) push(b.c[1]);
        if (__builtin_amdgcn_inverse_ballot_w64(o01 & h2)) push(b.c[2]);
        if (__builtin_amdgcn_inverse_ballot_w64(o012 & h3)) push(b.c[3]);
        node = b.c[3];
        node = __builtin_amdgcn_inverse_ballot_w64(h2) ? b.c[2] : node;
        node = __builtin_amdgcn_inverse_ballot_w64(h1) ? b.c[1] : node;
        node = __builtin_amdgcn_inverse_ballot_w64(h0) ? b.c[0] : node;
      } else {
        node = pop();
      }
      if (PTGS_PT_ANY_PARK) {
        if (node < 0 && leaf == DONE) {
          leaf = node;
          node = pop();
        }
        if ((__builtin_amdgcn_ballot_w64(leaf != DONE) | __builtin_amdgcn_ballot_w64(node == DONE)) ==
            __builtin_amdgcn_read_exec())
          break;
      }
    }
    if (PTGS_PT_ANY_PARK) {
      if (leaf != DONE) {
        occluded = leaf_any<STATS, TEX, N64>(sc, r, leaf, seed, cnt);
        leaf = DONE;
        if (occluded) node = DONE;
      }
      if (node < 0) {
        leaf = node;
        node = pop();
      }
      if (node == DONE && leaf == DONE) return occluded;
    } else {
      if (node < 0) {
        occluded = leaf_any<STATS, TEX, N64>(sc, r, node, seed, cnt);
        node = pop();
        if (occluded) node = DONE;
      }
      if (node == DONE) return occluded;
    }
  }
#else
  auto pop_nz = [&]() -> int {
    --sp;
    return (OVF == 0 || sp < PTGS_STACK) ? stack[sp * SS] : ovf[sp - PTGS_STACK];
  };
  while (true) {
    while (node >= 0) {
      PT_LANE_TICK(cnt, PT_L_ANY_NODE);
      Box4 b;
      box4_sel<N64>(rq, sc, node, r.tmax, b);
      if (STATS) cnt.nodes += 4;
      int next = -0x7fffffff - 1;
      bool have = false;
#pragma unroll
      for (int j = 0; j < 4; ++j)
        if (b.tn[j] != __builtin_huge_valf()) {
          if (!have) {
            next = b.c[j];
            have = true;
          } else {
            if (OVF == 0 || sp < PTGS_STACK) stack[sp * SS] = b.c[j];
            else ovf[sp - PTGS_STACK] = b.c[j];
            ++sp;
          }
        }
      if (!have) {
        if (sp == 0) return false;
        node = pop_nz();
        continue;
      }
      node = next;
    }
    uint32_t start, count;
    leaf_range<N64>(sc, node, start, count);
    for (uint32_t k = 0; k < count; ++k) {
      PT_LANE_TICK(cnt, PT_L_ANY_TRI);
      const float4* tp = sc.tris + 3u * (start + k);
      float4 a = tp[0], bb = tp[1], c = tp[2];
      if (STATS) cnt.tris++;
      float t, u, v;
      if (!tri_isect(r, mk3(a.x, a.y, a.z), mk3(bb.x, bb.y, bb.z), mk3(c.x, c.y, c.z), t, u, v)) continue;
      if (!(t >= r.tmin && t <= r.tmax)) continue;
      if (sc.has_transparent && (sc.tri_flags[start + k] & 1u)) {
        if (!anyhit_accept<TEX>(sc, f2u(a.w), f2u(bb.w), u, v, seed, f2u(c.w))) continue;
      }
      return true;
    }
    if (sp == 0) return false;
    node = pop_nz();
  }
#endif
}

__device__ __forceinline__ v4 matvec(const float* m, v4 v) {
  return mk4(((m[0] * v.x + m[4] * v.y) + m[8] * v.z) + m[12] * v.w,
             ((m[1] * v.x + m[5] * v.y) + m[9] * v.z) + m[13] * v.w,
             ((m[2] * v.x + m[6] * v.y) + m[10] * v.z) + m[14] * v.w,
             ((m[3] * v.x + m[7] * v.y) + m[11] * v.z) + m[15] * v.w);
}

__device__ __forceinline__ float4 blue_noise_texel(const DevScene& sc, uint32_t lx, uint32_t ly, uint32_t frame) {
  const float a1 = 0.75487766624669276f;
  const float a2 = 0.56984029099805327f;
  float rx = fractx((float)frame * a1);
  float ry = fractx((float)frame * a2);
  int ox = (int)(rx * (float)sc.bn_size);
  int oy = (int)(ry * (float)sc.bn_size);
  int px = ((int)lx + ox) & (sc.bn_size - 1);
  int py = ((int)ly + oy) & (sc.bn_size - 1);
  return sc.blue_noise[py * sc.bn_size + px];
}

__device__ __forceinline__ void primary_ray(const DevScene& sc, const CamParams& cp, uint32_t x, uint32_t y,
                                            uint32_t W, uint32_t H, uint32_t frame, v3& ro, v3& rd, float4& blue,
                                            uint32_t& seed) {
  blue = blue_noise_texel(sc, x, y, frame);
  seed = (y * W + x) + frame * 719393u;
  const float pcx = (float)x + blue.x, pcy = (float)y + blue.y;
  const float ux = pcx / (float)W, uy = pcy / (float)H;
  const float dx = ux * 2.0f - 1.0f, dy = uy * 2.0f - 1.0f;
  const v4 origin = matvec(cp.inv_view, mk4(0.f, 0.f, 0.f, 1.f));
  const v4 target = matvec(cp.inv_proj, mk4(dx, dy, 1.f, 1.f));
  const v3 dirc = normalize3(mk3(target.x, target.y, target.z) / target.w);
  const v4 direction = matvec(cp.inv_view, mk4(dirc.x, dirc.y, dirc.z, 0.f));
  ro = mk3(origin.x, origin.y, origin.z);
  rd = normalize3(mk3(direction.x, direction.y, direction.z));
}

struct Payload {
  v3 color;
  v3 next_o;
  v3 next_d;
  float hit_flag;
  v3 weight;
  uint32_t seed;
  float last_pdf;
  v2 blue;
  int depth;
  v3 hit_pos;
  v3 normal;
};

struct ShadeCtx {
  const DevScene* sc;
  const CamParams* cp;
  int* stack;
  uint32_t shadow_rays;
};

#define PT_PI 3.14159265359f
#define PT_PHI 1.61803398875f

__device__ __forceinline__ float blue_noise_dim(const Payload& p, int dim) {
  float base = (dim % 2 == 0) ? p.blue.x : p.blue.y;
  return fractx((base + ((float)p.depth * PT_PHI)) + ((float)dim * 0.754877f));
}

__device__ __forceinline__ v3 safe_normalize(v3 v) {
  float len = length3(v);
  return sel3(len < 1e-6f, mk3(0.0f, 1.0f, 0.0f), v / len);
}

__device__ __forceinline__ v3 f_schlick(float cos_theta, v3 f0) {
  float p = pow5(clampf(1.0f - cos_theta, 0.0f, 1.0f));
  return f0 + (1.0f - f0) * p;
}

__device__ __forceinline__ void ortho_basis(v3 n, v3& t, v3& b) {
  v3 up = sel3(absx(n.z) < 0.999f, mk3(0.f, 0.f, 1.f), mk3(1.f, 0.f, 0.f));
  t = safe_normalize(cross3(up, n));
  b = cross3(n, t);
}

__device__ __forceinline__ v3 sample_cosine(const Payload& p, v3 n) {
  float r1 = blue_noise_dim(p, 0);
  float r2 = blue_noise_dim(p, 1);
  float phi = (2.0f * PT_PI) * r1;
  float sq = sqrtx(r2);
  float s, c; sincosx(phi, &s, &c);
  v3 local = mk3(c * sq, s * sq, sqrtx(1.0f - r2));
  v3 t, b; ortho_basis(n, t, b);
  return safe_normalize((t * local.x + b * local.y) + n * local.z);
}

__device__ __forceinline__ float d_ggx(v3 n, v3 h, float roughness) {
  float a = roughness * roughness;
  float a2 = a * a;
  float ndh = fmaxx(dot3(n, h), 0.0f);
  float ndh2 = ndh * ndh;
  float denom = ndh2 * (a2 - 1.0f) + 1.0f;
  return a2 / (((PT_PI * denom) * denom) + 0.0001f);
}

__device__ __forceinline__ float v_smith(float ndv, float ndl, float roughness) {
  float a = roughness * roughness;
  float ggxv = ndl * (ndv * (1.0f - a) + a);
  float ggxl = ndv * (ndl * (1.0f - a) + a);
  return 0.5f / fmaxx(ggxv + ggxl, 0.0001f);
}

__device__ __forceinline__ v3 sample_ggx(const Payload& p, v3 n, float roughness) {
  float r1 = blue_noise_dim(p, 2);
  float r2 = blue_noise_dim(p, 3);
  float a = roughness * roughness;
  float phi = (2.0f * PT_PI) * r1;
  float denom = 1.0f + (a * a - 1.0f) * r2;
  float cos_t = sqrtx((1.0f - r2) / fmaxx(denom, 0.0001f));
  float sin_t = sqrtx(1.0f - cos_t * cos_t);
  float s, c; sincosx(phi, &s, &c);
  v3 hl = mk3(sin_t * c, sin_t * s, cos_t);
  v3 t, b; ortho_basis(n, t, b);
  return safe_normalize((t * hl.x + b * hl.y) + n * hl.z);
}

__device__ __forceinline__ float pdf_ggx(v3 n, v3 v, v3 l, float roughness) {
  v3 h = safe_normalize(v + l);
  float ndh = fmaxx(dot3(n, h), 0.0f);
  float vdh = fmaxx(dot3(v, h), 0.0f);
  float dn = d_ggx(n, h, roughness) * ndh;
  return dn / (4.0f * vdh + 0.0001f);
}

__device__ __forceinline__ float pdf_lambert(v3 n, v3 l) { return fmaxx(dot3(n, l), 0.0f) / PT_PI; }

#define SQ_TRACE 1u
#define SQ_VALID 2u
#define SQ_MIXED 4u
struct ShadowQuery {
  v3 o, d;
  float tmax;
  v3 pre;
  float post;
  float scale;
  float trans;
  uint32_t flags;
};

__device__ __forceinline__ void shadow_towards(ShadowQuery& q, v3 o, v3 light_pos) {
  v3 l = light_pos - o;
  float dist = length3(l);
  q.o = o;
  q.d = safe_normalize(l);
  q.tmax = dist - 0.005f;
}

template <bool STATS, bool TEX, int SS = PTGS_BLOCK, int OVF = PTGS_STACK_OVF, bool N64 = false>
__device__ __forceinline__ void resolve_shadow(ShadeCtx& c, v3& color, uint32_t seed, const ShadowQuery& q,
                                               TraversalCounters& cnt) {
  if (!(q.flags & SQ_TRACE)) return;
  c.shadow_rays++;
  const Ray r = make_ray(q.o, q.d, 0.001f, q.tmax);
  float vis = trace_any<STATS, TEX, SS, OVF, N64>(*c.sc, r, seed, c.stack, cnt) ? 0.0f : 1.0f;
  vis = fmaxx(vis, q.trans);
  if (vis > 0.0f && (q.flags & SQ_VALID)) {
    v3 contrib = (q.pre * vis) * q.post;
    if (q.flags & SQ_MIXED) contrib = (mk3(0.0f) + contrib) * q.scale;
    color = color + contrib;
  }
}

template <typename CDF>
__device__ __forceinline__ uint32_t cdf_search(const CDF* cdf, uint32_t n, float r) {
  uint32_t idx = 0, left = 0, right = n;
  while (left < right) {
    uint32_t mid = (left + right) >> 1;
    if (cdf[mid].cumulative_probability < r) left = mid + 1;
    else { idx = mid; right = mid; }
  }
  return idx;
}

__device__ void sample_punctual(const ShadeCtx& c, const Payload& p, v3 hit_pos, v3 n, v3 n_geo, v3 v, v3 albedo,
                                float roughness, v3 f0, float transmission, ShadowQuery& q) {
  const DevScene& sc = *c.sc;
  uint32_t num_lights = sc.num_plights;
  float r_select = blue_noise_dim(p, 4);
  uint32_t li = cdf_search(sc.pcdf, num_lights, r_select);
  const ptgs_punctual_light& light = sc.plights[li];
  v3 l;
  float attenuation = 1.0f;
  v3 lpos = ld3(light.position);
  v3 ldir = ld3(light.direction);
  if (light.type == 1) {
    l = normalize3(-ldir);
    attenuation = 1.0f;
  } else {
    v3 off = lpos - hit_pos;
    float dist_sq = dot3(off, off);
    dist_sq = fmaxx(dist_sq, 0.01f);
    float dist = sqrtx(dist_sq);
    l = off / dist;
    attenuation = 1.0f / dist_sq;
    if (light.range > 0.0f) {
      float ra = fmaxx(fminx(1.0f - pow4(dist / light.range), 1.0f), 0.0f) / dist_sq;
      attenuation = ra / dist_sq;
    }
    if (light.type == 2) {
      float cos_dir = dot3(-l, normalize3(ldir));
      float spot_scale = 1.0f / fmaxx(light.inner_cone_cos - light.outer_cone_cos, 0.001f);
      float spot_offset = -light.outer_cone_cos * spot_scale;
      float sa = clampf(cos_dir * spot_scale + spot_offset, 0.0f, 1.0f);
      attenuation = attenuation * (sa * sa);
    }
  }
  v3 le = (ld3(light.color) * light.intensity) * attenuation;
  float ndl = fmaxx(dot3(n, l), 0.0f);
  if (ndl < 0.001f) return;
  if (ndl > 0.0f && length3(le) > 0.0f) {
    v3 so = hit_pos + n_geo * 0.001f;
    if (light.type == 1) {
      q.o = so;
      q.d = l;
      q.tmax = 10000.0f;
    } else {
      shadow_towards(q, so, lpos);
    }
    q.trans = transmission;
    float weight = (float)num_lights;
    v3 h = safe_normalize(v + l);
    float ndf = d_ggx(n, h, roughness);
    float vis_t = v_smith(dot3(n, v), ndl, roughness);
    v3 f = f_schlick(dot3(h, v), f0);
    v3 kd = (mk3(1.0f) - f) * (1.0f - transmission);
    v3 spec = f * (ndf * vis_t);
    v3 diff = ((kd * albedo) / PT_PI) * (1.0f - transmission);
    q.pre = ((diff + spec) * le) * ndl;
    q.post = weight;
    q.flags = SQ_TRACE | SQ_VALID;
  }
}

__device__ void sample_emissive(const ShadeCtx& c, const Payload& p, bool sg, v3 hit_pos, v3 n, v3 n_geo, v3 v,
                                v3 albedo, float roughness, float metallic, v3 f0, float transmission, ShadowQuery& q) {
  const DevScene& sc = *c.sc;
  uint32_t num = sc.num_light_cdf;
  float r_select = blue_noise_dim(p, sg ? 4 : 7);
  uint32_t idx = cdf_search(sc.light_cdf, num, r_select);
  uint32_t tri_idx = sc.light_cdf[idx].triangle_index;
  ptgs_light_triangle tri = sc.light_tris[tri_idx];
  const uint32_t light_mat = tri.material_index;
  v3 p0 = ld3(sc.vertices[tri.v0].pos);
  v3 p1 = ld3(sc.vertices[tri.v1].pos);
  v3 p2 = ld3(sc.vertices[tri.v2].pos);
  float u = blue_noise_dim(p, sg ? 5 : 8);
  float w = blue_noise_dim(p, sg ? 6 : 9);
  if (u + w > 1.0f) { u = 1.0f - u; w = 1.0f - w; }
  v3 lp = (p0 * ((1.0f - u) - w) + p1 * u) + p2 * w;
  v3 cr = cross3(p1 - p0, p2 - p0);
  v3 ln = sg ? normalize3(cr) : safe_normalize(cr);
  v3 l = lp - hit_pos;
  float dist_sq = dot3(l, l);
  dist_sq = fmaxx(dist_sq, 0.0001f);
  float dist = sqrtx(dist_sq);
  l = l / dist;
  float ndl = fmaxx(dot3(n, l), 0.0f);
  if (ndl < 0.001f) return;
  float ldn = absx(dot3(-l, ln));
  if (ndl > 0.0f && ldn > 0.0f) {
    v3 so = hit_pos + n_geo * 0.001f;
    shadow_towards(q, so, lp);
    q.trans = transmission;
    q.flags = SQ_TRACE;
    const ptgs_material& lm = sc.materials[light_mat];
    v3 le = ld3(lm.emissive_factor_and_pad);
    float es = fmaxx(le.x, fmaxx(le.y, le.z));
    float pdf_nee = (es / c.cp->emissive_flux) * (dist_sq / ldn);
    float prob_spec;
    float pdf_spec, pdf_diff;
    if (sg) {
      pdf_spec = pdf_ggx(n, v, l, roughness);
      pdf_diff = pdf_lambert(n, l);
      prob_spec = clampf(length3(f0), 0.05f, 0.95f);
    } else {
      prob_spec = mixf(0.04f, 1.0f, metallic);
      pdf_spec = pdf_ggx(n, v, l, roughness);
      pdf_diff = pdf_lambert(n, l);
    }
    float prob_diff = 1.0f - prob_spec;
    float pdf_bsdf = pdf_spec * prob_spec + pdf_diff * prob_diff;
    float mis = (pdf_nee * pdf_nee) / (pdf_nee * pdf_nee + pdf_bsdf * pdf_bsdf);
    v3 h = safe_normalize(v + l);
    float ndf = d_ggx(n, h, roughness);
    float vis_t = v_smith(dot3(n, v), ndl, roughness);
    v3 f = f_schlick(dot3(h, v), f0);
    v3 kd = mk3(1.0f) - f;
    v3 spec = f * (ndf * vis_t);
    v3 diff = ((kd * albedo) / PT_PI) * (1.0f - transmission);
    v3 brdf = diff + spec;
    if (pdf_nee > 1e-10f) {
      q.pre = (((brdf * le) * ndl) * (1.0f / pdf_nee)) * mis;
      q.post = c.cp->ambient[3];
      q.flags |= SQ_VALID;
    }
  }
}

}
```

pathtracer_gaussiansplatting_amd/csrc/pt_kernels.hip:

```cpp
#include <hip/hip_runtime.h>

#include "pt_shade.h"
#include "pt_launch.h"
#include "xcd.h"

#ifndef PTGS_PT_XCD_REMAP
#define PTGS_PT_XCD_REMAP 0
#endif
#ifndef PTGS_PT_WG
#define PTGS_PT_WG 64
#endif
#ifndef PTGS_PT_PAIR
#define PTGS_PT_PAIR 1
#endif
#ifndef PTGS_PT_LPP
#define PTGS_PT_LPP 2
#endif
#ifndef PTGS_PT_SCHED
#define PTGS_PT_SCHED 1
#endif
#ifndef PTGS_PT_SCHED_MIN
#define PTGS_PT_SCHED_MIN (1u << 22)
#endif

namespace ptgs {

__device__ __forceinline__ unsigned long long wave_sum(uint32_t v) {
  unsigned long long x = v;
#pragma unroll
  for (int off = 32; off > 0; off >>= 1) x += __shfl_xor(x, off, 64);
  return x;
}

__device__ __forceinline__ void flush_counters(unsigned long long* counters, uint32_t ext, uint32_t shadow,
                                               uint32_t samples, const TraversalCounters& tc, bool stats) {
  unsigned long long a = wave_sum(ext), b = wave_sum(shadow), c = wave_sum(samples);
  unsigned long long d = 0, e = 0, f = 0;
  if (stats) { d = wave_sum(tc.nodes); e = wave_sum(tc.tris); f = wave_sum(tc.hits); }
  if ((threadIdx.x & 63) == 0) {
    atomicAdd(counters + 0, a);
    atomicAdd(counters + 1, b);
    atomicAdd(counters + 2, c);
    if (stats) { atomicAdd(counters + 3, d); atomicAdd(counters + 4, e); atomicAdd(counters + 5, f); }
  }
}

#ifndef PTGS_PT_MIN_WAVES
#define PTGS_PT_MIN_WAVES 4
#endif

#ifdef PT_STAMP
#define PT_STAMP_WG 65536
__device__ unsigned long long g_pt_stamps[PT_STAMP_WG * 2];
#endif

__host__ __device__ __forceinline__ uint32_t pt_lanes_log2(uint32_t spp) {
  if (PTGS_PT_WG != 64 || !PTGS_PT_PAIR) return 0u;
  return (PTGS_PT_LPP >= 4 && spp >= 4u) ? 2u : (PTGS_PT_LPP >= 2 && spp >= 2u) ? 1u : 0u;
}

template <bool STATS, bool TEX, bool DEEP>
__global__ __launch_bounds__(PTGS_PT_WG, PTGS_PT_MIN_WAVES) void pt_camera_kernel(DevScene sc, CamParams cp, float4* __restrict__ accum,
                                                        uint32_t W, uint32_t H, uint32_t row0, uint32_t row1,
                                                        uint32_t spp, uint32_t frame0, uint32_t stride,
                                                        uint32_t mode, unsigned long long* counters,
                                                        const uint32_t* __restrict__ order, uint32_t* __restrict__ cost) {
  const uint32_t lid = threadIdx.x;
  const uint32_t wave = lid >> 6, lane = lid & 63u;
#ifdef PT_STAMP
  const uint32_t swg = blockIdx.y * gridDim.x + blockIdx.x;
  if (lid == 0 && swg < PT_STAMP_WG) g_pt_stamps[2 * swg] = __builtin_amdgcn_s_memrealtime();
#endif
#if PTGS_PT_XCD_REMAP
  static_assert(PTGS_PT_WG == 256, "the XCD remap maps 16x16 tiles");
  const uint32_t tl = xcd_tile(blockIdx.y * gridDim.x + blockIdx.x, gridDim.x * gridDim.y);
  const uint32_t bx = tl % gridDim.x, by = tl / gridDim.x;
#else
  uint32_t bx = blockIdx.x, by = blockIdx.y;
  if (order) {
    const uint32_t tl = (uint32_t)__builtin_amdgcn_readfirstlane((int)order[blockIdx.y * gridDim.x + blockIdx.x]);
    by = tl / gridDim.x;
    bx = tl - by * gridDim.x;
  }
  const unsigned long long t_start = cost ? __builtin_amdgcn_s_memrealtime() : 0ull;
#endif
#if PTGS_PT_WG == 64
  const uint32_t llpp = pt_lanes_log2(spp);
  const bool pair = llpp != 0u;
  const uint32_t lpp = 1u << llpp, pw = 64u >> llpp;
  const uint32_t half = lane >> (6u - llpp);
  const uint32_t pl = lane & (pw - 1u);
  const uint32_t x = bx * 8u + (pl & 7u);
  const uint32_t y = row0 + by * (8u >> llpp) + (pl >> 3);
#else
  const bool pair = false;
  const uint32_t lpp = 1u, pw = 64u;
  const uint32_t half = 0;
  const uint32_t x = bx * 16u + (wave & 1u) * 8u + (lane & 7u);
  const uint32_t y = row0 + by * 16u + (wave >> 1) * 8u + (lane >> 3);
#endif
  const bool active = (x < W) && (y < row1);

  __shared__ int s_stack[PTGS_STACK * PTGS_PT_WG];
  ShadeCtx c; c.sc = &sc; c.cp = &cp; c.stack = s_stack + threadIdx.x; c.shadow_rays = 0;
  TraversalCounters tc; tc.nodes = 0; tc.tris = 0; tc.hits = 0;
  PT_LANES_INIT(tc);
  uint32_t ext_rays = 0, samples = 0;

  const size_t pix = (size_t)y * W + x;
  v3 state = mk3(0.0f);
  float state_a = 0.0f;
  if (active && half == 0u && (mode == PTGS_ACCUM_SUM || frame0 > 0)) {
    float4 prev = accum[pix];
    state = mk3(prev.x, prev.y, prev.z);
    state_a = prev.w;
  }
  auto fold = [&](const v3& acc, uint32_t s) {
    const uint32_t frame = frame0 + s * stride;
    if (mode == PTGS_ACCUM_SUM) {
      state = state + acc;
      state_a = state_a + 1.0f;
    } else if (frame > 0) {
      float blend = 1.0f / (float)(frame + 1u);
      state = mix3(state, acc, blend);
    } else {
      state = acc;
    }
  };
  const uint32_t iters = (spp + lpp - 1u) / lpp;
  for (uint32_t k = 0; k < iters; ++k) {
    const uint32_t s = k * lpp + half;
    v3 acc = mk3(0.0f);
    if (active && s < spp) {
      PT_LANE_TICK(tc, PT_L_SAMPLE);
      const uint32_t frame = frame0 + s * stride;
      v3 ro, rd;
      float4 blue;
      uint32_t seed;
      primary_ray(sc, cp, x, y, W, H, frame, ro, rd, blue, seed);

      v3 thr = mk3(1.0f);
      Payload p;
      p.seed = seed;
      p.blue = mk2(blue.z, blue.w);
      p.last_pdf = 0.0f;
      p.hit_flag = 0.0f;
      p.color = mk3(0.0f); p.weight = mk3(1.0f); p.next_o = ro; p.next_d = rd;
      int max_depth = 12;
      for (int depth = 0; depth < max_depth; ++depth) {
        PT_LANE_TICK(tc, PT_L_BOUNCE);
        p.depth = depth;
        Ray ray = make_ray(ro, rd, 0.001f, 10000.0f);
        ext_rays++;
        Hit h = trace_closest<STATS, TEX, PTGS_PT_WG, DEEP ? PTGS_STACK_OVF : 0, PTGS_PT_NODE64 != 0,
                              PTGS_PT_NODE64 != 0 && PTGS_PT_STACK_CULL != 0>(sc, ray, p.seed, c.stack, tc);
        if (STATS && h.gid != 0xffffffffu) tc.hits++;
        ShadowQuery q;
        q.flags = 0;
        if (h.gid == 0xffffffffu) miss<false>(cp, p);
        else closest_hit<false, TEX>(c, p, ray, h, q);
        resolve_shadow<STATS, TEX, PTGS_PT_WG, DEEP ? PTGS_STACK_OVF : 0, PTGS_PT_NODE64 != 0>(c, p.color, p.seed, q, tc);
        acc = acc + p.color * thr;
        acc = vmin(acc, 5.0f);
        if (p.hit_flag < 0.0f) break;
        if (depth == 0 && p.hit_flag < 1.5f) max_depth = 4;
        thr = thr * p.weight;
        ro = p.next_o;
        rd = p.next_d;
        float mt = fmaxx(fmaxx(thr.x, thr.y), thr.z);
        if (mt < 0.001f) break;
        if (depth >= 4) {
          float pr = clampf(mt, 0.05f, 0.95f);
          if (rnd(p.seed) > pr) break;
          thr = thr / pr;
        }
      }
      samples++;
    }
    if (pair) {
      v3 got[4];
      got[0] = acc;
#pragma unroll
      for (uint32_t j = 1; j < 4; ++j) {
        const int src = (int)((lane + j * pw) & 63u);
        got[j] = mk3(__shfl(acc.x, src), __shfl(acc.y, src), __shfl(acc.z, src));
        if (j + 1u >= lpp) break;
      }
      if (active && half == 0u) {
#pragma unroll
        for (uint32_t j = 0; j < 4; ++j)
          if (j < lpp && s + j < spp) fold(got[j], s + j);
      }
    } else if (active) {
      fold(acc, s);
    }
  }
  if (active && half == 0u) {
    if (mode == PTGS_ACCUM_SUM) accum[pix] = make_float4(state.x, state.y, state.z, state_a);
    else accum[pix] = make_float4(state.x, state.y, state.z, 1.0f);
  }
  flush_counters(counters, ext_rays, c.shadow_rays, samples, tc, STATS);
  PT_LANES_FLUSH(tc);
#if !PTGS_PT_XCD_REMAP
  if (cost) {
    __syncthreads();
    if (lid == 0) cost[by * gridDim.x + bx] = (uint32_t)min(__builtin_amdgcn_s_memrealtime() - t_start, 0xFFFFFFFFull);
  }
#endif
#ifdef PT_STAMP
  __syncthreads();
  if (lid == 0 && swg < PT_STAMP_WG) g_pt_stamps[2 * swg + 1] = __builtin_amdgcn_s_memrealtime();
#endif
}

#ifndef PTGS_TORUS_MIN_WAVES
#define PTGS_TORUS_MIN_WAVES 4
#endif
template <bool STATS, bool TEX, bool DEEP>
__global__ __launch_bounds__(256, TEX ? 1 : PTGS_TORUS_MIN_WAVES) void pt_torus_kernel(DevScene sc, CamParams cp, TorusParams tp,
                                                       const ptgs_ray_sample* __restrict__ samples,
                                                       uint32_t n, uint32_t side, uint32_t frame,
                                                       ptgs_hitdata* __restrict__ hits,
                                                       unsigned long long* counters) {
  const uint32_t index = blockIdx.x * blockDim.x + threadIdx.x;
  __shared__ int s_stack[PTGS_STACK * PTGS_BLOCK];
  ShadeCtx c; c.sc = &sc; c.cp = &cp; c.stack = s_stack + threadIdx.x; c.shadow_rays = 0;
  TraversalCounters tc; tc.nodes = 0; tc.tris = 0; tc.hits = 0;
  PT_LANES_INIT(tc);
  uint32_t ext_rays = 0, nsamp = 0;
  if (index < n) {
    const uint32_t lx = index % side, ly = index / side;
    uint32_t light_seed = index + frame * 719393u;
    ptgs_ray_sample smp = samples[index];
    float u = (smp.uv[0] * 2.0f) * PT_PI;
    float v = (smp.uv[1] * 2.0f) * PT_PI;
    float R = tp.major_radius, r = tp.minor_radius, hh = tp.height;
    float su, cu, sv, cv;
    sincosx(u, &su, &cu);
    sincosx(v, &sv, &cv);
    v3 lp = mk3((R + r * cv) * cu, r * sv + hh, (R + r * cv) * su);
    v3 ln = mk3(cv * cu, sv, cv * su);
    v4 wo = matvec(tp.model, mk4(lp.x, lp.y, lp.z, 1.0f));
    v4 wn4 = matvec(tp.model, mk4(ln.x, ln.y, ln.z, 0.0f));
    v3 wn = normalize3(mk3(wn4.x, wn4.y, wn4.z));
    v3 rd = wn;
    v3 so = mk3(wo.x, wo.y, wo.z) + rd * 0.05f;

    float4 blue = blue_noise_texel(sc, lx, ly, frame);
    v3 acc = mk3(0.0f);
    v3 thr = mk3(1.0f);
    Payload p;
    p.seed = light_seed;
    p.last_pdf = 0.0f;
    p.blue = mk2(blue.z, blue.w);
    p.depth = 0;
    p.hit_flag = 0.0f;
    p.color = mk3(0.0f); p.weight = mk3(1.0f); p.next_o = so; p.next_d = rd;
    p.hit_pos = mk3(0.0f); p.normal = mk3(0.0f, 1.0f, 0.0f);
    v3 fpos, fnorm;
    float fflag;
    for (int depth = 0; depth < 12; ++depth) {
      if (depth > 0) {
        p.depth = depth;
        thr = thr * p.weight;
        float mt = fmaxx(fmaxx(thr.x, thr.y), thr.z);
        if (mt < 0.001f) break;
        if (depth >= 4) {
          float pr = clampf(mt, 0.05f, 0.95f);
          if (rnd(p.seed) > pr) break;
          thr = thr / pr;
        }
      }
      Ray ray = make_ray(p.next_o, p.next_d, depth == 0 ? 0.0f : 0.001f, 10000.0f);
      ext_rays++;
      Hit h = trace_closest<STATS, TEX, PTGS_BLOCK, DEEP ? PTGS_STACK_OVF : 0>(sc, ray, p.seed, c.stack, tc);
      if (STATS && h.gid != 0xffffffffu) tc.hits++;
      ShadowQuery q;
      q.flags = 0;
      if (h.gid == 0xffffffffu) miss<true>(cp, p);
      else closest_hit<true, TEX>(c, p, ray, h, q);
      resolve_shadow<STATS, TEX, PTGS_BLOCK, DEEP ? PTGS_STACK_OVF : 0>(c, p.color, p.seed, q, tc);
      if (depth == 0) {
        fpos = p.hit_pos;
        fflag = p.hit_flag;
        fnorm = p.normal;
        if (!(p.hit_flag > 0.5f)) break;
        acc = acc + p.color * thr;
      } else {
        acc = acc + p.color * thr;
        acc = vmin(acc, 5.0f);
        if (p.hit_flag < 1.5f) break;
      }
    }
    v3 cur = acc;
    ptgs_hitdata hd = hits[index];
    if (frame > 0) {
      v3 prev = mk3(hd.color[0], hd.color[1], hd.color[2]);
      float bf = 1.0f / (float)(frame + 1u);
      cur = mix3(prev, cur, bf);
    }
    hd.pos[0] = fpos.x; hd.pos[1] = fpos.y; hd.pos[2] = fpos.z;
    hd.flag = fflag;
    hd.normal[0] = fnorm.x; hd.normal[1] = fnorm.y; hd.normal[2] = fnorm.z;
    hd.color[0] = cur.x; hd.color[1] = cur.y; hd.color[2] = cur.z; hd.color[3] = 1.0f;
    hits[index] = hd;
    nsamp = 1;
  }
  flush_counters(counters, ext_rays, c.shadow_rays, nsamp, tc, STATS);
}

template <bool TEX, bool DEEP>
__global__ __launch_bounds__(256) void pt_depth_kernel(DevScene sc, CamParams cp, ViewMat vm, float* __restrict__ depth,
                                                       uint32_t W, uint32_t H, uint32_t row0, uint32_t row1,
                                                       uint32_t frame) {
  const uint32_t lid = threadIdx.x;
  const uint32_t wave = lid >> 6, lane = lid & 63u;
  const uint32_t x = blockIdx.x * 16u + (wave & 1u) * 8u + (lane & 7u);
  const uint32_t y = row0 + blockIdx.y * 16u + (wave >> 1) * 8u + (lane >> 3);
  __shared__ int s_stack[PTGS_STACK * PTGS_BLOCK];
  if (x >= W || y >= row1) return;
  TraversalCounters tc; tc.nodes = 0; tc.tris = 0; tc.hits = 0;
  PT_LANES_INIT(tc);
  const uint32_t seed = y * W + x + frame * 719393u;
  const float ux = ((float)x + 0.5f) / (float)W, uy = ((float)y + 0.5f) / (float)H;
  const float dx = ux * 2.0f - 1.0f, dy = uy * 2.0f - 1.0f;
  const v4 origin = matvec(cp.inv_view, mk4(0.f, 0.f, 0.f, 1.f));
  const v4 target = matvec(cp.inv_proj, mk4(dx, dy, 1.f, 1.f));
  const v3 dirc = normalize3(mk3(target.x, target.y, target.z) / target.w);
  const v4 direction = matvec(cp.inv_view, mk4(dirc.x, dirc.y, dirc.z, 0.f));
  const v3 ro = mk3(origin.x, origin.y, origin.z);
  const v3 rd = normalize3(mk3(direction.x, direction.y, direction.z));
  const Ray ray = make_ray(ro, rd, 0.001f, 10000.0f);
  const Hit h = trace_closest<false, TEX, PTGS_BLOCK, DEEP ? PTGS_STACK_OVF : 0>(sc, ray, seed, s_stack + threadIdx.x, tc);
  float d = __builtin_huge_valf();
  if (h.gid != 0xffffffffu) {
    const v3 hp = ro + rd * h.t;
    const v4 pv = matvec(vm.m, mk4(hp.x, hp.y, hp.z, 1.0f));
    d = -pv.z;
  }
  depth[(size_t)y * W + x] = d;
}

#define PT_ORDER_THREADS 1024
__global__ __launch_bounds__(PT_ORDER_THREADS) void pt_order_kernel(const uint32_t* __restrict__ cost,
                                                                    uint32_t* __restrict__ order, uint32_t n) {
  __shared__ uint32_t s_h[256];
  __shared__ uint32_t s_max[PT_ORDER_THREADS / 64];
  const uint32_t tid = threadIdx.x, lane = tid & 63u;
  uint32_t mx = 0;
  for (uint32_t t = tid; t < n; t += PT_ORDER_THREADS) mx = max(mx, cost[t]);
  for (int off = 32; off > 0; off >>= 1) mx = max(mx, (uint32_t)__shfl_xor((int)mx, off));
  if (lane == 0) s_max[tid >> 6] = mx;
  if (tid < 256) s_h[tid] = 0;
  __syncthreads();
  mx = 0;
  for (uint32_t w = 0; w < PT_ORDER_THREADS / 64; ++w) mx = max(mx, s_max[w]);
  const float scale = 255.99f / (float)max(mx, 1u);
  auto bucket = [&](uint32_t c) { return 255u - min(255u, (uint32_t)((float)c * scale)); };
  for (uint32_t t = tid; t < n; t += PT_ORDER_THREADS) atomicAdd(s_h + bucket(cost[t]), 1u);
  __syncthreads();
  if (tid < 64) {
    const uint32_t c0 = s_h[4 * lane], c1 = s_h[4 * lane + 1], c2 = s_h[4 * lane + 2], c3 = s_h[4 * lane + 3];
    const uint32_t sum = (c0 + c1) + (c2 + c3);
    uint32_t incl = sum;
    for (int off = 1; off < 64; off <<= 1) {
      const uint32_t y = (uint32_t)__shfl_up((int)incl, off);
      if (lane >= (uint32_t)off) incl += y;
    }
    const uint32_t ex = incl - sum;
    s_h[4 * lane] = ex;
    s_h[4 * lane + 1] = ex + c0;
    s_h[4 * lane + 2] = ex + c0 + c1;
    s_h[4 * lane + 3] = ex + c0 + c1 + c2;
  }
  __syncthreads();
  for (uint32_t t = tid; t < n; t += PT_ORDER_THREADS) order[atomicAdd(s_h + bucket(cost[t]), 1u)] = t;
}

void free_pt_sched(PtSched& ps) {
  if (ps.cost) (void)hipFree(ps.cost);
  if (ps.order) (void)hipFree(ps.order);
  ps = PtSched{};
}

hipError_t launch_pt_camera(const DevScene& sc, const CamParams& cp, float* accum, uint32_t W, uint32_t H,
                            uint32_t row0, uint32_t row1, uint32_t spp, uint32_t frame0, uint32_t stride,
                            uint32_t mode, unsigned long long* counters, bool stats, PtSched* ps,
                            hipStream_t stream) {
  if (row1 <= row0 || spp == 0) return hipSuccess;
  const uint32_t tx = PTGS_PT_WG == 64 ? 8u : 16u;
  const uint32_t ty = PTGS_PT_WG == 64 ? 8u >> pt_lanes_log2(spp) : 16u;
  dim3 grid((W + tx - 1u) / tx, (row1 - row0 + ty - 1u) / ty);
  dim3 block(PTGS_PT_WG);
  const uint32_t *order = nullptr;
  uint32_t* cost = nullptr;
#if !PTGS_PT_XCD_REMAP
  if (ps && PTGS_PT_SCHED && ps->owned && ps->stream != stream) {
    if (hipStreamQuery(ps->stream) != hipErrorNotReady) {
      ps->owned = false;
      ps->gx = ps->gy = 0;
    } else {
      ps = nullptr;
    }
  }
  if (ps && PTGS_PT_SCHED && (uint64_t)W * (row1 - row0) * spp >= (uint64_t)PTGS_PT_SCHED_MIN) {
    const uint32_t n = grid.x * grid.y;
    hipError_t e;
    ps->stream = stream;
    ps->owned = true;
    if (n > ps->cap) {
      free_pt_sched(*ps);
      if ((e = hipMalloc(&ps->cost, (size_t)n * 4)) || (e = hipMalloc(&ps->order, (size_t)n * 4))) return e;
      ps->cap = n;
    }
    if (ps->gx == grid.x && ps->gy == grid.y) {
      hipLaunchKernelGGL(pt_order_kernel, dim3(1), dim3(PT_ORDER_THREADS), 0, stream, (const uint32_t*)ps->cost,
                         ps->order, n);
      if ((e = hipGetLastError())) return e;
      order = ps->order;
    }
    ps->gx = grid.x;
    ps->gy = grid.y;
    cost = ps->cost;
  }
#endif
  static void (*const ks[8])(DevScene, CamParams, float4*, uint32_t, uint32_t, uint32_t, uint32_t, uint32_t, uint32_t,
                             uint32_t, uint32_t, unsigned long long*, const uint32_t*, uint32_t*) = {
      pt_camera_kernel<false, false, false>, pt_camera_kernel<false, false, true>, pt_camera_kernel<false, true, false>,
      pt_camera_kernel<false, true, true>,   pt_camera_kernel<true, false, false>, pt_camera_kernel<true, false, true>,
      pt_camera_kernel<true, true, false>,   pt_camera_kernel<true, true, true>};
  auto k = ks[(stats ? 4 : 0) + (sc.uses_textures ? 2 : 0) + (sc.deep_stack ? 1 : 0)];
  hipLaunchKernelGGL(k, grid, block, 0, stream, sc, cp, (float4*)accum, W, H, row0, row1, spp, frame0, stride, mode,
                     counters, order, cost);
  return hipGetLastError();
}

hipError_t launch_pt_depth(const DevScene& sc, const CamParams& cp, const ViewMat& vm, float* depth, uint32_t W,
                           uint32_t H, uint32_t row0, uint32_t row1, uint32_t frame, hipStream_t stream) {
  row1 = row1 < H ? row1 : H;
  if (row1 <= row0) return hipSuccess;
  dim3 grid((W + 15u) / 16u, (row1 - row0 + 15u) / 16u);
  auto k = sc.uses_textures ? (sc.deep_stack ? pt_depth_kernel<true, true> : pt_depth_kernel<true, false>)
                           : (sc.deep_stack ? pt_depth_kernel<false, true> : pt_depth_kernel<false, false>);
  hipLaunchKernelGGL(k, grid, dim3(256), 0, stream, sc, cp, vm, depth, W, H, row0, row1, frame);
  return hipGetLastError();
}

hipError_t launch_pt_torus(const DevScene& sc, const CamParams& cp, const TorusParams& tp,
                           const ptgs_ray_sample* samples, uint32_t n, uint32_t side, uint32_t frame,
                           ptgs_hitdata* hits, unsigned long long* counters, bool stats, hipStream_t stream) {
  if (n == 0) return hipSuccess;
  dim3 grid((n + 255u) / 256u);
  dim3 block(256);
  static void (*const ks[8])(DevScene, CamParams, TorusParams, const ptgs_ray_sample*, uint32_t, uint32_t, uint32_t,
                             ptgs_hitdata*, unsigned long long*) = {
      pt_torus_kernel<false, false, false>, pt_torus_kernel<false, false, true>, pt_torus_kernel<false, true, false>,
      pt_torus_kernel<false, true, true>,   pt_torus_kernel<true, false, false>, pt_torus_kernel<true, false, true>,
      pt_torus_kernel<true, true, false>,   pt_torus_kernel<true, true, true>};
  auto k = ks[(stats ? 4 : 0) + (sc.uses_textures ? 2 : 0) + (sc.deep_stack ? 1 : 0)];
  hipLaunchKernelGGL(k, grid, block, 0, stream, sc, cp, tp, samples, n, side, frame, hits, counters);
  return hipGetLastError();
}

}

#ifdef PT_LANES
extern "C" int ptgs_debug_pt_lanes(unsigned long long* host, unsigned int n) {
  if (n > 2u * ptgs::PT_L_COUNT) n = 2u * ptgs::PT_L_COUNT;
  hipError_t e = hipMemcpyFromSymbol(host, HIP_SYMBOL(ptgs::g_pt_lanes), (size_t)n * 8, 0, hipMemcpyDeviceToHost);
  if (e) return (int)e;
  static const unsigned long long zero[2 * ptgs::PT_L_COUNT] = {};
  return (int)hipMemcpyToSymbol(HIP_SYMBOL(ptgs::g_pt_lanes), zero, sizeof(zero), 0, hipMemcpyHostToDevice);
}
#endif
#ifdef PT_STAMP
extern "C" int ptgs_debug_pt_stamps(unsigned long long* host, unsigned int n) {
  if (n > PT_STAMP_WG * 2u) n = PT_STAMP_WG * 2u;
  return (int)hipMemcpyFromSymbol(host, HIP_SYMBOL(ptgs::g_pt_stamps), (size_t)n * 8, 0, hipMemcpyDeviceToHost);
}
#endif
```

pathtracer_gaussiansplatting_amd/renderer.py:

```python
from __future__ import annotations

import ctypes as C

import numpy as np

from . import _abi
from ._abi import (BvhBuffers, Gaussians, RayPush, SceneBuild, SceneInfo, SceneTreeOpt, SplatBuffers, SplatStats,
                   SplatStatus, TraceStats, Ubo)


def _ptr(x) -> int:
    if x is None:
        return 0
    if isinstance(x, int):
        return x
    if hasattr(x, "data_ptr"):
        if not x.is_cuda:
            raise _abi.PtgsError("expected a device tensor (got a host tensor): the renderer has no CPU path")
        if not x.is_contiguous():
            raise _abi.PtgsError("device tensor must be contiguous")
        return x.data_ptr()
    raise TypeError(f"cannot take a device pointer of {type(x)}")


def _gaussians(g: dict) -> Gaussians:
    gs = Gaussians()
    gs.means, gs.scales, gs.rotations = _ptr(g["means"]), _ptr(g["scales"]), _ptr(g["rotations"])
    gs.opacities, gs.colors = _ptr(g["opacities"]), _ptr(g["colors"])
    gs.count = int(g["means"].shape[0])
    gs.ids = _ptr(g.get("ids"))
    gs.chunk_bounds = _ptr(g.get("chunk_bounds"))
    return gs


def _stream(stream) -> int:
    if stream is None:
        try:
            import torch
            return torch.cuda.current_stream().cuda_stream
        except Exception:
            return 0
    if isinstance(stream, int):
        return stream
    return stream.cuda_stream


class Renderer:
    def __init__(self, device: int = 0, lib_path: str | None = None, publish_splat_buffers: bool = False,
                 wavefront: bool = False):
        self.lib = _abi.load_library(lib_path)
        self._publish = _abi.FLAG_PT_WAVEFRONT if wavefront else 0
        if publish_splat_buffers:
            self._publish |= _abi.FLAG_SPLAT_PUBLISH
        if publish_splat_buffers == "tight":
            self._publish |= _abi.FLAG_SPLAT_PUBLISH_TIGHT
        h = C.c_void_p()
        rc = self.lib.ptgs_create(int(device), C.byref(h))
        _abi.check(rc, f"ptgs_create(device={device})")
        self._h = h
        self.device = device
        self.scene = None
        self.set_flags(0)

    def close(self):
        if getattr(self, "_h", None):
            self.lib.ptgs_destroy(self._h)
            self._h = None

    def __del__(self):
        try:
            self.close()
        except Exception:
            pass

    def _err(self) -> str:
        return (self.lib.ptgs_last_error(self._h) or b"").decode()

    def _chk(self, rc: int, what: str):
        _abi.check(rc, what, self._err())

    def upload_scene(self, scene) -> SceneInfo:
        d = scene.desc()
        self._chk(self.lib.ptgs_scene_upload(self._h, C.byref(d)), "ptgs_scene_upload")
        self.scene = scene
        return self.scene_info()

    def scene_info(self) -> SceneInfo:
        info = SceneInfo()
        self._chk(self.lib.ptgs_scene_get_info(self._h, C.byref(info)), "ptgs_scene_get_info")
        return info

    def scene_build(self) -> SceneBuild:
        b = SceneBuild()
        self._chk(self.lib.ptgs_scene_get_build(self._h, C.byref(b)), "ptgs_scene_get_build")
        return b

    def scene_tree_opt(self) -> SceneTreeOpt:
        t = SceneTreeOpt()
        self._chk(self.lib.ptgs_scene_get_tree_opt(self._h, C.byref(t)), "ptgs_scene_get_tree_opt")
        return t

    def trace_camera(self, ubo: Ubo, width: int, height: int, accum, spp: int = 1, frame_stride: int = 1,
                     mode: int = _abi.ACCUM_RUNNING_MEAN, rows: tuple | None = None, stream=None):
        if rows is None:
            rc = self.lib.ptgs_trace_camera(self._h, C.byref(ubo), width, height, _ptr(accum), spp, frame_stride,
                                            mode, _stream(stream))
        else:
            rc = self.lib.ptgs_trace_camera_rows(self._h, C.byref(ubo), width, height, rows[0], rows[1],
                                                 _ptr(accum), spp, frame_stride, mode, _stream(stream))
        self._chk(rc, "ptgs_trace_camera")

    def trace_torus(self, ubo: Ubo, push: RayPush, samples, n: int, hits, stream=None):
        rc = self.lib.ptgs_trace_torus(self._h, C.byref(ubo), C.byref(push), _ptr(samples), n, _ptr(hits),
                                       _stream(stream))
        self._chk(rc, "ptgs_trace_torus")

    def trace_depth(self, ubo: Ubo, width: int, height: int, depth, stream=None, rows=None):
        if rows is not None:
            rc = self.lib.ptgs_trace_depth_rows(self._h, C.byref(ubo), width, height, int(rows[0]), int(rows[1]),
                                                _ptr(depth), _stream(stream))
            self._chk(rc, "ptgs_trace_depth_rows")
            return
        rc = self.lib.ptgs_trace_depth(self._h, C.byref(ubo), width, height, _ptr(depth), _stream(stream))
        self._chk(rc, "ptgs_trace_depth")

    def knn3_mean_dist2(self, xyz, dist2, stream=None):
        n = int(xyz.shape[0])
        self._chk(self.lib.ptgs_knn3_mean_dist2(self._h, _ptr(xyz), n, _ptr(dist2), _stream(stream)),
                  "ptgs_knn3_mean_dist2")

    def gaussians_from_points(self, xyz, rgb=None, stream=None) -> dict:
        import torch
        n = int(xyz.shape[0])
        dev = xyz.device
        g = {"means": torch.empty((n, 3), dtype=torch.float32, device=dev),
             "scales": torch.empty((n, 3), dtype=torch.float32, device=dev),
             "rotations": torch.empty((n, 4), dtype=torch.float32, device=dev),
             "opacities": torch.empty((n,), dtype=torch.float32, device=dev),
             "colors": torch.empty((n, 3), dtype=torch.float32, device=dev)}
        rc = self.lib.ptgs_gaussians_from_points(self._h, _ptr(xyz), _ptr(rgb), n, _ptr(g["means"]), _ptr(g["scales"]),
                                                 _ptr(g["rotations"]), _ptr(g["opacities"]), _ptr(g["colors"]),
                                                 _stream(stream))
        self._chk(rc, "ptgs_gaussians_from_points")
        return g

    def comm_unique_id(self) -> bytes:
        buf = (C.c_uint8 * 128)()
        self._chk(self.lib.ptgs_comm_unique_id(buf), "ptgs_comm_unique_id")
        return bytes(buf)

    def comm_create(self, unique_id: bytes, nranks: int, rank: int):
        buf = (C.c_uint8 * 128).from_buffer_copy(unique_id)
        self._chk(self.lib.ptgs_comm_create(self._h, buf, nranks, rank), "ptgs_comm_create")
        self.comm_world = nranks

    def comm_destroy(self):
        self._chk(self.lib.ptgs_comm_destroy(self._h), "ptgs_comm_destroy")
        self.comm_world = 0

    def reduce_radiance(self, accum, root: int = 0, stream=None):
        rc = self.lib.ptgs_reduce_radiance(self._h, _ptr(accum), accum.numel(), root, _stream(stream))
        self._chk(rc, "ptgs_reduce_radiance")

    def allreduce_radiance(self, accum, stream=None):
        rc = self.lib.ptgs_allreduce_radiance(self._h, _ptr(accum), accum.numel(), _stream(stream))
        self._chk(rc, "ptgs_allreduce_radiance")

    def gather_rows(self, image, row_ranges, root: int = 0, stream=None):
        H, W = int(image.shape[0]), int(image.shape[1])
        world = getattr(self, "comm_world", 0)
        if len(row_ranges) != world:
            raise ValueError(f"gather_rows needs one (r0, r1) per rank: {len(row_ranges)} given, world {world}")
        rr = np.asarray(row_ranges, np.uint32).reshape(-1)
        if rr.size != 2 * world:
            raise ValueError("gather_rows: every row range is a (r0, r1) pair")
        rc = self.lib.ptgs_gather_rows(self._h, _ptr(image), W, H, rr.ctypes.data, root, _stream(stream))
        self._chk(rc, "ptgs_gather_rows")

    def reduce_scatter_rows(self, image, row_ranges, stream=None):
        H, W = int(image.shape[0]), int(image.shape[1])
        world = getattr(self, "comm_world", 0)
        if len(row_ranges) != world:
            raise ValueError(f"reduce_scatter_rows needs one (r0, r1) per rank: {len(row_ranges)} given, world {world}")
        rr = np.asarray(row_ranges, np.uint32).reshape(-1)
        if rr.size != 2 * world:
            raise ValueError("reduce_scatter_rows: every row range is a (r0, r1) pair")
        rc = self.lib.ptgs_reduce_scatter_rows(self._h, _ptr(image), W, H, rr.ctypes.data, _stream(stream))
        self._chk(rc, "ptgs_reduce_scatter_rows")

    def set_flags(self, flags: int):
        self._flags = flags
        self._chk(self.lib.ptgs_set_flags(self._h, flags | self._publish), "ptgs_set_flags")

    def set_wavefront(self, on: bool):
        self._publish = (self._publish & ~_abi.FLAG_PT_WAVEFRONT) | (_abi.FLAG_PT_WAVEFRONT if on else 0)
        self.set_flags(getattr(self, "_flags", 0))

    def set_splat_overlap(self, on: bool):
        self._publish = (self._publish & ~_abi.FLAG_SPLAT_OVERLAP) | (_abi.FLAG_SPLAT_OVERLAP if on else 0)
        self.set_flags(getattr(self, "_flags", 0))

    def stats_reset(self, stream=None):
        self._chk(self.lib.ptgs_stats_reset(self._h, _stream(stream)), "ptgs_stats_reset")

    def stats(self) -> TraceStats:
        s = TraceStats()
        self._chk(self.lib.ptgs_stats_read(self._h, C.byref(s)), "ptgs_stats_read")
        return s

    def splat_points(self, ubo: Ubo, push: RayPush, hits, samples, n: int, width: int, height: int, rgba8, depth,
                     stream=None):
        rc = self.lib.ptgs_splat_points(self._h, C.byref(ubo), C.byref(push), _ptr(hits), _ptr(samples), n, width,
                                        height, _ptr(rgba8), _ptr(depth), _stream(stream))
        self._chk(rc, "ptgs_splat_points")

    def splat_gaussians(self, g: dict, ubo: Ubo, width: int, height: int, out, bg=(0.0, 0.0, 0.0),
                        tile_rows: tuple | None = None, want_stats: bool = False, stream=None, over=None):
        gs = _gaussians(g)
        bgc = np.asarray(bg, np.float32)
        t0, t1 = (0, 0xFFFFFFFF) if tile_rows is None else tile_rows
        st = SplatStats()
        if over is not None:
            rc = self.lib.ptgs_splat_gaussians_over(self._h, C.byref(gs), C.byref(ubo), width, height, _ptr(over[0]),
                                                    _ptr(over[1]), t0, t1, _ptr(out),
                                                    C.byref(st) if want_stats else None, _stream(stream))
            self._chk(rc, "ptgs_splat_gaussians_over")
            return st if want_stats else None
        rc = self.lib.ptgs_splat_gaussians(self._h, C.byref(gs), C.byref(ubo), width, height, _abi.fptr(bgc), t0,
                                           t1, _ptr(out), C.byref(st) if want_stats else None, _stream(stream))
        self._chk(rc, "ptgs_splat_gaussians")
        return st if want_stats else None

    def splat_gaussians_invdepth(self, width: int, height: int, out=None, stream=None):
        import torch
        if out is None:
            out = torch.empty((height, width), dtype=torch.float32, device=f"cuda:{torch.cuda.current_device()}")
        self._f32(("out", out, width * height))
        rc = self.lib.ptgs_splat_gaussians_invdepth(self._h, width, height, _ptr(out), _stream(stream))
        self._chk(rc, "ptgs_splat_gaussians_invdepth")
        return out

    def splat_gaussians_backward(self, g: dict, ubo: Ubo, width: int, height: int, dL_dout, bg=(0.0, 0.0, 0.0),
                                 want_means2d: bool = False, want_conics: bool = False, stream=None,
                                 dL_dinvdepth=None, want_view: bool = False) -> dict:
        import torch
        n = int(g["means"].shape[0])
        self._f32(("means", g["means"], n * 3), ("scales", g["scales"], n * 3), ("rotations", g["rotations"], n * 4),
                  ("opacities", g["opacities"], n), ("colors", g["colors"], n * 3),
                  ("dL_dout", dL_dout, width * height * 4),
                  *([("dL_dinvdepth", dL_dinvdepth, width * height)] if dL_dinvdepth is not None else []))
        dev = g["means"].device
        shapes = {"means": (n, 3), "scales": (n, 3), "rotations": (n, 4), "opacities": (n,), "colors": (n, 3)}
        if want_means2d:
# ... 387 lines not shown
```

Baseline: 6945 Mrays/s.

## Shrink megakernel LDS traversal stack with budgeted BVH4 collapse to raise occupancy

Adds a smaller LDS stack depth (PTGS_PT_STACK=30) for the path-trace megakernel and makes the tree optimiser try that limit first, including a new budget-aware BVH2-to-BVH4 collapse that keeps the worst-case stack need under the limit. When the walked tree fits, the non-deep kernel uses less shared memory per workgroup and its launch-bounds minimum waves rises from 4 to 5, aiming for higher occupancy. Deep scenes fall back to the full LDS stack plus overflow registers. The risk is that the budgeted collapse yields a worse-quality tree with more node visits, and the tighter register bound may cause spills.

```diff
diff --git a/include/ptgs/ptgs.h b/include/ptgs/ptgs.h
--- a/include/ptgs/ptgs.h
+++ b/include/ptgs/ptgs.h
@@ -304,6 +304,7 @@
     double ms;
 } ptgs_scene_tree_opt;
 int ptgs_scene_get_tree_opt(const ptgs_ctx* ctx, ptgs_scene_tree_opt* out);
+int ptgs_scene_get_pt_stack(const ptgs_ctx* ctx, uint32_t* lds_depth, uint32_t* walked_need, uint32_t* deep);
 
 
 #define PTGS_ACCUM_RUNNING_MEAN 0u
diff --git a/pathtracer_gaussiansplatting_amd/_abi.py b/pathtracer_gaussiansplatting_amd/_abi.py
--- a/pathtracer_gaussiansplatting_amd/_abi.py
+++ b/pathtracer_gaussiansplatting_amd/_abi.py
@@ -223,6 +223,7 @@
     "ptgs_scene_get_bvh": (_I, [_P, C.POINTER(BvhBuffers)]),
     "ptgs_scene_get_build": (_I, [_P, C.POINTER(SceneBuild)]),
     "ptgs_scene_get_tree_opt": (_I, [_P, C.POINTER(SceneTreeOpt)]),
+    "ptgs_scene_get_pt_stack": (_I, [_P, C.POINTER(_U), C.POINTER(_U), C.POINTER(_U)]),
     "ptgs_trace_camera": (_I, [_P, C.POINTER(Ubo), _U, _U, _P, _U, _U, _U, _P]),
     "ptgs_trace_camera_rows": (_I, [_P, C.POINTER(Ubo), _U, _U, _U, _U, _P, _U, _U, _U, _P]),
     "ptgs_trace_torus": (_I, [_P, C.POINTER(Ubo), C.POINTER(RayPush), _P, _U, _P, _P]),
diff --git a/pathtracer_gaussiansplatting_amd/csrc/api.cpp b/pathtracer_gaussiansplatting_amd/csrc/api.cpp
--- a/pathtracer_gaussiansplatting_amd/csrc/api.cpp
+++ b/pathtracer_gaussiansplatting_amd/csrc/api.cpp
@@ -47,6 +47,7 @@
   ptgs_scene_info info{};
   ptgs_scene_build build{};
   ptgs_scene_tree_opt tree_opt{};
+  uint32_t pt_walked_need = 0;
   unsigned long long* counters = nullptr;
   SplatFrames frames;
   DensifyWorkspace* densify = nullptr;
@@ -296,11 +297,14 @@
   std::vector<uint32_t> n64;
   StackLayout sl;
   TreeOptInfo oi;
-  if (!make_opt_traversal_nodes(host_n4.data(), c->info.num_bvh_nodes, (int)c->build.fan,
-                                s.deep_stack ? PTGS_STACK_TOTAL : PTGS_STACK, optimise, force, n64, sl, oi))
+  const uint32_t limits[2] = {PTGS_PT_STACK, PTGS_STACK_TOTAL};
+  if (!make_opt_traversal_nodes(host_n4.data(), c->info.num_bvh_nodes, (int)c->build.fan, limits, 2, optimise, force,
+                                n64, sl, oi))
     return fail(c, PTGS_ERANGE, "BVH node extents beyond the compact nodes' step range (2^-100 .. 2^100)");
   c->tree_opt = ptgs_scene_tree_opt{oi.applied, oi.num_nodes, oi.need, oi.depth, oi.fan, oi.passes,
                                     oi.area_before, oi.area_after, oi.ms};
+  c->pt_walked_need = oi.applied ? oi.need : c->build.stack_need;
+  s.pt_deep_stack = c->pt_walked_need >= PTGS_PT_STACK ? 1 : 0;
   s.stk_key_mask = sl.key_mask;
   s.leaf_shift = sl.leaf_shift;
   s.leaf_start_mask = sl.leaf_start_mask;
@@ -310,6 +314,8 @@
               "fan %u, area sum %.3f -> %.3f\n", oi.applied ? "optimised" : "not applied", oi.ms, oi.passes,
               c->info.num_bvh_nodes, oi.num_nodes, c->build.stack_need, oi.need, c->info.bvh_depth, oi.depth, oi.fan,
               oi.area_before, oi.area_after);
+    fprintf(stderr, "[ptgs] megakernel: walked need %u, LDS stack %u%s\n", c->pt_walked_need, (uint32_t)PTGS_PT_STACK,
+            s.pt_deep_stack ? " (DEEP)" : "");
     fprintf(stderr, "[ptgs] stack word:%u link bits, %u key bits (mask %08x), leaf shift %u\n", sl.ref_bits, sl.key_bits,
             sl.key_mask, sl.leaf_shift);
   }
@@ -534,6 +540,15 @@
   if (!c || !out) return PTGS_EINVAL;
   if (!c->has_scene) return PTGS_ENOSCENE;
   *out = c->tree_opt;
+  return PTGS_OK;
+}
+
+int ptgs_scene_get_pt_stack(const ptgs_ctx* c, uint32_t* lds_depth, uint32_t* walked_need, uint32_t* deep) {
+  if (!c) return PTGS_EINVAL;
+  if (!c->has_scene) return PTGS_ENOSCENE;
+  if (lds_depth) *lds_depth = c->dsc.pt_deep_stack ? PTGS_STACK : PTGS_PT_STACK;
+  if (walked_need) *walked_need = c->pt_walked_need;
+  if (deep) *deep = c->dsc.pt_deep_stack ? 1u : 0u;
   return PTGS_OK;
 }
 
diff --git a/pathtracer_gaussiansplatting_amd/csrc/bvh_opt.cpp b/pathtracer_gaussiansplatting_amd/csrc/bvh_opt.cpp
--- a/pathtracer_gaussiansplatting_amd/csrc/bvh_opt.cpp
+++ b/pathtracer_gaussiansplatting_amd/csrc/bvh_opt.cpp
@@ -196,6 +196,125 @@
   }
 }
 
+struct Ent4 {
+  float lo[3], hi[3];
+  int32_t ref;
+};
+void bvh2_children(const float* n, Ent4 e[2]) {
+  int32_t c0, c1;
+  std::memcpy(&c0, &n[12], 4);
+  std::memcpy(&c1, &n[13], 4);
+  e[0] = Ent4{{n[0], n[2], n[8]}, {n[1], n[3], n[9]}, c0};
+  e[1] = Ent4{{n[4], n[6], n[10]}, {n[5], n[7], n[11]}, c1};
+}
+float ent_area(const Ent4& e) {
+  float d[3];
+  for (int a = 0; a < 3; ++a) d[a] = std::max(0.0f, e.hi[a] - e.lo[a]);
+  return d[0] * d[1] + d[1] * d[2] + d[2] * d[0];
+}
+
+void bvh2_heights(const std::vector<float>& n2, std::vector<uint32_t>& h) {
+  const size_t num = n2.size() / 16;
+  h.assign(num, 0u);
+  for (size_t i = num; i-- > 0;) {
+    uint32_t m = 0;
+    for (int k = 0; k < 2; ++k) {
+      int32_t c;
+      std::memcpy(&c, &n2[16 * i + 12 + k], 4);
+      if (c >= 0) m = std::max(m, h[(size_t)c]);
+    }
+    h[i] = 1u + m;
+  }
+}
+
+}
+
+uint32_t bvh2_height(const std::vector<float>& n2) {
+  std::vector<uint32_t> h;
+  bvh2_heights(n2, h);
+  return h.empty() ? 0u : h[0];
+}
+
+bool collapse_bvh4_budget(const std::vector<float>& n2, std::vector<float>& n4, uint32_t& num4, uint32_t& max_stack,
+                          uint32_t& depth4, int max_children, uint32_t need_limit) {
+  n4.clear();
+  num4 = 0; max_stack = 0; depth4 = 0;
+  std::vector<uint32_t> h2;
+  bvh2_heights(n2, h2);
+  if (h2.empty() || need_limit == 0 || h2[0] >= need_limit) return false;
+  max_children = std::max(2, std::min(4, max_children));
+  auto height = [&](const Ent4& e) { return e.ref >= 0 ? h2[(size_t)e.ref] : 0u; };
+  struct Item { int32_t b2; uint32_t slot, budget; };
+  std::vector<Item> queue;
+  std::vector<std::vector<uint32_t>> kids;
+  std::vector<uint32_t> ncount;
+  queue.push_back(Item{0, 0u, need_limit - 1u});
+  n4.assign(32, 0.0f);
+  kids.emplace_back();
+  ncount.push_back(0);
+  for (size_t q = 0; q < queue.size(); ++q) {
+    const Item it = queue[q];
+    Ent4 list[4];
+    int cnt = 2;
+    bvh2_children(&n2[16 * (size_t)it.b2], list);
+    while (cnt < max_children) {
+      int order[4], no = 0;
+      for (int k = 0; k < cnt; ++k)
+        if (list[k].ref >= 0) order[no++] = k;
+      std::stable_sort(order, order + no, [&](int a, int b) { return ent_area(list[a]) > ent_area(list[b]); });
+      int best = -1;
+      Ent4 sub[2];
+      for (int o = 0; o < no && best < 0; ++o) {
+        if (it.budget < (uint32_t)cnt) break;
+        const uint32_t room = it.budget - (uint32_t)cnt;
+        bvh2_children(&n2[16 * (size_t)list[order[o]].ref], sub);
+        bool fits = height(sub[0]) <= room && height(sub[1]) <= room;
+        for (int k = 0; k < cnt && fits; ++k)
+          if (k != order[o]) fits = height(list[k]) <= room;
+        if (fits) best = order[o];
+      }
+      if (best < 0) break;
+      list[best] = sub[0];
+      list[cnt++] = sub[1];
+    }
+    float* f = &n4[32 * (size_t)it.slot];
+    for (int j = 0; j < 4; ++j) {
+      int32_t child = 0;
+      if (j < cnt) {
+        for (int a = 0; a < 3; ++a) {
+          f[(2 * a) * 4 + j] = list[j].lo[a];
+          f[(2 * a + 1) * 4 + j] = list[j].hi[a];
+        }
+        if (list[j].ref >= 0) {
+          const uint32_t ni = (uint32_t)(n4.size() / 32);
+          n4.resize(n4.size() + 32, 0.0f);
+          f = &n4[32 * (size_t)it.slot];
+          queue.push_back(Item{list[j].ref, ni, it.budget - (uint32_t)(cnt - 1)});
+          kids.emplace_back();
+          ncount.push_back(0);
+          kids[it.slot].push_back(ni);
+          child = (int32_t)ni;
+        } else {
+          child = list[j].ref;
+        }
+      } else {
+        for (int a = 0; a < 6; ++a) f[a * 4 + j] = 1e30f;
+      }
+      std::memcpy(&f[24 + j], &child, 4);
+    }
+    ncount[it.slot] = (uint32_t)cnt;
+  }
+  num4 = (uint32_t)(n4.size() / 32);
+  std::vector<uint32_t> need(num4, 0), dep(num4, 1);
+  for (size_t i = num4; i-- > 0;) {
+    uint32_t m = 0, d = 0;
+    for (uint32_t k : kids[i]) { m = std::max(m, need[k]); d = std::max(d, dep[k]); }
+    need[i] = (ncount[i] - 1) + m;
+    dep[i] = 1 + d;
+  }
+  max_stack = need[0];
+  depth4 = dep[0];
+  return max_stack < need_limit;
 }
 
 double bvh4_area_sum(const float* n4, uint32_t num) {
@@ -224,6 +343,11 @@
 
 bool optimize_bvh4(const float* n4, uint32_t num, int fan, uint32_t need_limit, std::vector<float>& out,
                    TreeOptInfo& info, int passes) {
+  return optimize_bvh4(n4, num, fan, &need_limit, 1, out, info, passes);
+}
+
+bool optimize_bvh4(const float* n4, uint32_t num, int fan, const uint32_t* limits, int num_limits,
+                   std::vector<float>& out, TreeOptInfo& info, int passes) {
   const auto t0 = std::chrono::steady_clock::now();
   info = TreeOptInfo{};
   out.clear();
@@ -246,16 +370,23 @@
   info.passes = (uint32_t)std::max(0, passes);
   std::vector<float> n2;
   emit_bvh2(t, n2);
-  for (int f = std::max(2, std::min(4, fan)); f >= 2; --f) {
-    uint32_t num4 = 0, need = 0, depth4 = 0;
-    collapse_bvh4(n2, out, num4, need, depth4, f);
-    if (need >= need_limit) continue;
-    info.num_nodes = num4;
-    info.need = need;
-    info.depth = depth4;
-    info.fan = (uint32_t)f;
-    info.area_after = bvh4_area_sum(out.data(), num4);
-    return done(true);
+  info.height2 = bvh2_height(n2);
+  const int fan0 = std::max(2, std::min(4, fan));
+  for (int l = 0; l < num_limits; ++l) {
+    const uint32_t need_limit = limits[l];
+    for (int f = fan0; f >= 2; --f) {
+      uint32_t num4 = 0, need = 0, depth4 = 0;
+      collapse_bvh4(n2, out, num4, need, depth4, f);
+      if (need >= need_limit && !(f == fan0 && collapse_bvh4_budget(n2, out, num4, need, depth4, f, need_limit)))
+        continue;
+      info.num_nodes = num4;
+      info.need = need;
+      info.depth = depth4;
+      info.fan = (uint32_t)f;
+      info.limit = need_limit;
+      info.area_after = bvh4_area_sum(out.data(), num4);
+      return done(true);
+    }
   }
   return done(false);
 }
@@ -263,9 +394,15 @@
 bool make_opt_traversal_nodes(const float* n4, uint32_t num, int fan, uint32_t need_limit, bool optimise,
                               int force_key_bits, std::vector<uint32_t>& n64, StackLayout& layout, TreeOptInfo& info,
                               std::vector<float>* walked) {
+  return make_opt_traversal_nodes(n4, num, fan, &need_limit, 1, optimise, force_key_bits, n64, layout, info, walked);
+}
+
+bool make_opt_traversal_nodes(const float* n4, uint32_t num, int fan, const uint32_t* limits, int num_limits,
+                              bool optimise, int force_key_bits, std::vector<uint32_t>& n64, StackLayout& layout,
+                              TreeOptInfo& info, std::vector<float>* walked) {
   info = TreeOptInfo{};
   std::vector<float> opt;
-  if (optimise && optimize_bvh4(n4, num, fan, need_limit, opt, info)) {
+  if (optimise && optimize_bvh4(n4, num, fan, limits, num_limits, opt, info)) {
     if (make_traversal_nodes(opt.data(), info.num_nodes, force_key_bits, n64, layout)) {
       if (walked) walked->swap(opt);
       return true;
diff --git a/pathtracer_gaussiansplatting_amd/csrc/bvh_opt.h b/pathtracer_gaussiansplatting_amd/csrc/bvh_opt.h
--- a/pathtracer_gaussiansplatting_amd/csrc/bvh_opt.h
+++ b/pathtracer_gaussiansplatting_amd/csrc/bvh_opt.h
@@ -16,6 +16,8 @@
   uint32_t depth = 0;
   uint32_t fan = 0;
   uint32_t passes = 0;
+  uint32_t limit = 0;
+  uint32_t height2 = 0;
   double area_before = 0.0;
   double area_after = 0.0;
   double ms = 0.0;
@@ -23,11 +25,21 @@
 
 double bvh4_area_sum(const float* nodes4, uint32_t num_nodes);
 
+uint32_t bvh2_height(const std::vector<float>& nodes2);
+
+bool collapse_bvh4_budget(const std::vector<float>& nodes2, std::vector<float>& nodes4, uint32_t& num_nodes4,
+                          uint32_t& max_stack, uint32_t& depth4, int max_children, uint32_t need_limit);
+
 bool optimize_bvh4(const float* nodes4, uint32_t num_nodes, int fan, uint32_t need_limit, std::vector<float>& out,
                    TreeOptInfo& info, int passes = kTreeOptPasses);
+bool optimize_bvh4(const float* nodes4, uint32_t num_nodes, int fan, const uint32_t* limits, int num_limits,
+                   std::vector<float>& out, TreeOptInfo& info, int passes = kTreeOptPasses);
 
 bool make_opt_traversal_nodes(const float* nodes4, uint32_t num_nodes, int fan, uint32_t need_limit, bool optimise,
                               int force_key_bits, std::vector<uint32_t>& nodes64, StackLayout& layout, TreeOptInfo& info,
                               std::vector<float>* walked = nullptr);
+bool make_opt_traversal_nodes(const float* nodes4, uint32_t num_nodes, int fan, const uint32_t* limits, int num_limits,
+                              bool optimise, int force_key_bits, std::vector<uint32_t>& nodes64, StackLayout& layout,
+                              TreeOptInfo& info, std::vector<float>* walked = nullptr);
 
 }
diff --git a/pathtracer_gaussiansplatting_amd/csrc/pt_device.h b/pathtracer_gaussiansplatting_amd/csrc/pt_device.h
--- a/pathtracer_gaussiansplatting_amd/csrc/pt_device.h
+++ b/pathtracer_gaussiansplatting_amd/csrc/pt_device.h
@@ -26,6 +26,7 @@
   DevTextures tex;
   int32_t uses_textures;
   int32_t deep_stack;
+  int32_t pt_deep_stack;
   uint32_t num_light_cdf;
   uint32_t num_plights;
   int32_t bn_size;
@@ -91,6 +92,10 @@
 #define PTGS_STACK_OVF 9
 #endif
 #define PTGS_STACK_TOTAL (PTGS_STACK + PTGS_STACK_OVF)
+#ifndef PTGS_PT_STACK
+#define PTGS_PT_STACK 30
+#endif
+static_assert(PTGS_PT_STACK >= 2 && PTGS_PT_STACK <= PTGS_STACK, "the megakernel's LDS stack depth");
 #define PTGS_BLOCK 256
 
 PTGS_HD float i2f(int x) { union { int i; float f; } c; c.i = x; return c.f; }
@@ -438,7 +443,7 @@
 #ifndef PTGS_PT_ULOOP_ANY
 #define PTGS_PT_ULOOP_ANY PTGS_PT_ULOOP
 #endif
-template <bool STATS, bool TEX, int SS = PTGS_BLOCK, int OVF = PTGS_STACK_OVF, bool N64 = false, bool CULL = false>
+template <bool STATS, bool TEX, int SS = PTGS_BLOCK, int OVF = PTGS_STACK_OVF, bool N64 = false, bool CULL = false, int LDS = PTGS_STACK>
 __device__ __forceinline__ Hit trace_closest(const DevScene& sc, const Ray& r, uint32_t seed, int* stack,
                                              TraversalCounters& cnt) {
   static_assert(!CULL || N64, "the distance key needs the compact nodes' packed links");
@@ -452,15 +457,15 @@
   int ovf[OVF > 0 ? OVF : 1];
   auto push = [&](int c, float tn) {
     const int x = CULL ? (int)stack_pack((uint32_t)c, tn, kmask) : c;
-    if (OVF == 0 || sp < PTGS_STACK) stack[sp * SS] = x;
-    else ovf[sp - PTGS_STACK] = x;
+    if (OVF == 0 || sp < LDS) stack[sp * SS] = x;
+    else ovf[sp - LDS] = x;
     ++sp;
   };
   auto pop = [&]() -> int {
     if (!CULL) {
       if (!sp) return DONE;
       --sp;
-      return (OVF == 0 || sp < PTGS_STACK) ? stack[sp * SS] : ovf[sp - PTGS_STACK];
+      return (OVF == 0 || sp < LDS) ? stack[sp * SS] : ovf[sp - LDS];
     }
     const float cap = h.t * 1.0000004f;
     uint32_t x;
@@ -468,7 +473,7 @@
       x = (uint32_t)DONE;
       if (sp) {
         --sp;
-        x = (uint32_t)((OVF == 0 || sp < PTGS_STACK) ? stack[sp * SS] : ovf[sp - PTGS_STACK]);
+        x = (uint32_t)((OVF == 0 || sp < LDS) ? stack[sp * SS] : ovf[sp - LDS]);
       }
     } while (stack_bound(x, kmask) > cap);
     return (int)stack_link(x, kmask);
@@ -481,7 +486,7 @@
       uint32_t x = (uint32_t)DONE;
       if (sp) {
         --sp;
-        x = (uint32_t)((OVF == 0 || sp < PTGS_STACK) ? stack[sp * SS] : ovf[sp - PTGS_STACK]);
+        x = (uint32_t)((OVF == 0 || sp < LDS) ? stack[sp * SS] : ovf[sp - LDS]);
       }
       n = CULL ? (int)stack_link(x, kmask) : (int)x;
       again = CULL && stack_bound(x, kmask) > cap;
@@ -601,7 +606,7 @@
   return occ;
 }
 
-template <bool STATS, bool TEX, int SS = PTGS_BLOCK, int OVF = PTGS_STACK_OVF, bool N64 = false>
+template <bool STATS, bool TEX, int SS = PTGS_BLOCK, int OVF = PTGS_STACK_OVF, bool N64 = false, int LDS = PTGS_STACK>
 __device__ __forceinline__ bool trace_any(const DevScene& sc, const Ray& r, uint32_t seed, int* stack,
                                           TraversalCounters& cnt) {
   const Ray rq = node64_ray<N64>(r);
@@ -612,14 +617,14 @@
   const int DONE = 0x7fffffff;
   bool occluded = false;
   auto push = [&](int c) {
-    if (OVF == 0 || sp < PTGS_STACK) stack[sp * SS] = c;
-    else ovf[sp - PTGS_STACK] = c;
+    if (OVF == 0 || sp < LDS) stack[sp * SS] = c;
+    else ovf[sp - LDS] = c;
     ++sp;
   };
   auto pop = [&]() -> int {
     if (!sp) return DONE;
     --sp;
-    return (OVF == 0 || sp < PTGS_STACK) ? stack[sp * SS] : ovf[sp - PTGS_STACK];
+    return (OVF == 0 || sp < LDS) ? stack[sp * SS] : ovf[sp - LDS];
   };
   int leaf = DONE;
   for (;;) {
@@ -678,7 +683,7 @@
 #else
   auto pop_nz = [&]() -> int {
     --sp;
-    return (OVF == 0 || sp < PTGS_STACK) ? stack[sp * SS] : ovf[sp - PTGS_STACK];
+    return (OVF == 0 || sp < LDS) ? stack[sp * SS] : ovf[sp - LDS];
   };
   while (true) {
     while (node >= 0) {
@@ -695,8 +700,8 @@
             next = b.c[j];
             have = true;
           } else {
-            if (OVF == 0 || sp < PTGS_STACK) stack[sp * SS] = b.c[j];
-            else ovf[sp - PTGS_STACK] = b.c[j];
+            if (OVF == 0 || sp < LDS) stack[sp * SS] = b.c[j];
+            else ovf[sp - LDS] = b.c[j];
             ++sp;
           }
         }
@@ -880,13 +885,13 @@
   q.tmax = dist - 0.005f;
 }
 
-template <bool STATS, bool TEX, int SS = PTGS_BLOCK, int OVF = PTGS_STACK_OVF, bool N64 = false>
+template <bool STATS, bool TEX, int SS = PTGS_BLOCK, int OVF = PTGS_STACK_OVF, bool N64 = false, int LDS = PTGS_STACK>
 __device__ __forceinline__ void resolve_shadow(ShadeCtx& c, v3& color, uint32_t seed, const ShadowQuery& q,
                                                TraversalCounters& cnt) {
   if (!(q.flags & SQ_TRACE)) return;
   c.shadow_rays++;
   const Ray r = make_ray(q.o, q.d, 0.001f, q.tmax);
-  float vis = trace_any<STATS, TEX, SS, OVF, N64>(*c.sc, r, seed, c.stack, cnt) ? 0.0f : 1.0f;
+  float vis = trace_any<STATS, TEX, SS, OVF, N64, LDS>(*c.sc, r, seed, c.stack, cnt) ? 0.0f : 1.0f;
   vis = fmaxx(vis, q.trans);
   if (vis > 0.0f && (q.flags & SQ_VALID)) {
     v3 contrib = (q.pre * vis) * q.post;
diff --git a/pathtracer_gaussiansplatting_amd/csrc/pt_kernels.hip b/pathtracer_gaussiansplatting_amd/csrc/pt_kernels.hip
--- a/pathtracer_gaussiansplatting_amd/csrc/pt_kernels.hip
+++ b/pathtracer_gaussiansplatting_amd/csrc/pt_kernels.hip
@@ -46,8 +46,12 @@
 }
 
 #ifndef PTGS_PT_MIN_WAVES
-#define PTGS_PT_MIN_WAVES 4
-#endif
+#define PTGS_PT_MIN_WAVES 5
+#endif
+#ifndef PTGS_PT_DEEP_MIN_WAVES
+#define PTGS_PT_DEEP_MIN_WAVES 4
+#endif
+__host__ __device__ constexpr int pt_lds_stack(bool deep) { return deep ? PTGS_STACK : PTGS_PT_STACK; }
 
 #ifdef PT_STAMP
 #define PT_STAMP_WG 65536
@@ -60,7 +64,7 @@
 }
 
 template <bool STATS, bool TEX, bool DEEP>
-__global__ __launch_bounds__(PTGS_PT_WG, PTGS_PT_MIN_WAVES) void pt_camera_kernel(DevScene sc, CamParams cp, float4* __restrict__ accum,
+__global__ __launch_bounds__(PTGS_PT_WG, DEEP ? PTGS_PT_DEEP_MIN_WAVES : PTGS_PT_MIN_WAVES) void pt_camera_kernel(DevScene sc, CamParams cp, float4* __restrict__ accum,
                                                         uint32_t W, uint32_t H, uint32_t row0, uint32_t row1,
                                                         uint32_t spp, uint32_t frame0, uint32_t stride,
                                                         uint32_t mode, unsigned long long* counters,
@@ -101,7 +105,9 @@
 #endif
   const bool active = (x < W) && (y < row1);
 
-  __shared__ int s_stack[PTGS_STACK * PTGS_PT_WG];
+  constexpr int kLds = pt_lds_stack(DEEP);
+  constexpr int kOvf = DEEP ? PTGS_STACK_TOTAL - kLds : 0;
+  __shared__ int s_stack[kLds * PTGS_PT_WG];
   ShadeCtx c; c.sc = &sc; c.cp = &cp; c.stack = s_stack + threadIdx.x; c.shadow_rays = 0;
   TraversalCounters tc; tc.nodes = 0; tc.tris = 0; tc.hits = 0;
   PT_LANES_INIT(tc);
@@ -152,14 +158,14 @@
         p.depth = depth;
         Ray ray = make_ray(ro, rd, 0.001f, 10000.0f);
         ext_rays++;
-        Hit h = trace_closest<STATS, TEX, PTGS_PT_WG, DEEP ? PTGS_STACK_OVF : 0, PTGS_PT_NODE64 != 0,
-                              PTGS_PT_NODE64 != 0 && PTGS_PT_STACK_CULL != 0>(sc, ray, p.seed, c.stack, tc);
+        Hit h = trace_closest<STATS, TEX, PTGS_PT_WG, kOvf, PTGS_PT_NODE64 != 0,
+                              PTGS_PT_NODE64 != 0 && PTGS_PT_STACK_CULL != 0, kLds>(sc, ray, p.seed, c.stack, tc);
         if (STATS && h.gid != 0xffffffffu) tc.hits++;
         ShadowQuery q;
         q.flags = 0;
         if (h.gid == 0xffffffffu) miss<false>(cp, p);
         else closest_hit<false, TEX>(c, p, ray, h, q);
-        resolve_shadow<STATS, TEX, PTGS_PT_WG, DEEP ? PTGS_STACK_OVF : 0, PTGS_PT_NODE64 != 0>(c, p.color, p.seed, q, tc);
+        resolve_shadow<STATS, TEX, PTGS_PT_WG, kOvf, PTGS_PT_NODE64 != 0, kLds>(c, p.color, p.seed, q, tc);
         acc = acc + p.color * thr;
         acc = vmin(acc, 5.0f);
         if (p.hit_flag < 0.0f) break;
@@ -383,6 +389,16 @@
   ps = PtSched{};
 }
 
+typedef void (*PtCameraKernel)(DevScene, CamParams, float4*, uint32_t, uint32_t, uint32_t, uint32_t, uint32_t, uint32_t,
+                               uint32_t, uint32_t, unsigned long long*, const uint32_t*, uint32_t*);
+static PtCameraKernel pt_camera_instantiation(bool stats, bool tex, bool deep) {
+  static const PtCameraKernel ks[8] = {
+      pt_camera_kernel<false, false, false>, pt_camera_kernel<false, false, true>, pt_camera_kernel<false, true, false>,
+      pt_camera_kernel<false, true, true>,   pt_camera_kernel<true, false, false>, pt_camera_kernel<true, false, true>,
+      pt_camera_kernel<true, true, false>,   pt_camera_kernel<true, true, true>};
+  return ks[(stats ? 4 : 0) + (tex ? 2 : 0) + (deep ? 1 : 0)];
+}
+
 hipError_t launch_pt_camera(const DevScene& sc, const CamParams& cp, float* accum, uint32_t W, uint32_t H,
                             uint32_t row0, uint32_t row1, uint32_t spp, uint32_t frame0, uint32_t stride,
                             uint32_t mode, unsigned long long* counters, bool stats, PtSched* ps,
@@ -424,12 +440,7 @@
     cost = ps->cost;
   }
 #endif
-  static void (*const ks[8])(DevScene, CamParams, float4*, uint32_t, uint32_t, uint32_t, uint32_t, uint32_t, uint32_t,
-                             uint32_t, uint32_t, unsigned long long*, const uint32_t*, uint32_t*) = {
-      pt_camera_kernel<false, false, false>, pt_camera_kernel<false, false, true>, pt_camera_kernel<false, true, false>,
-      pt_camera_kernel<false, true, true>,   pt_camera_kernel<true, false, false>, pt_camera_kernel<true, false, true>,
-      pt_camera_kernel<true, true, false>,   pt_camera_kernel<true, true, true>};
-  auto k = ks[(stats ? 4 : 0) + (sc.uses_textures ? 2 : 0) + (sc.deep_stack ? 1 : 0)];
+  auto k = pt_camera_instantiation(stats, sc.uses_textures != 0, sc.pt_deep_stack != 0);
   hipLaunchKernelGGL(k, grid, block, 0, stream, sc, cp, (float4*)accum, W, H, row0, row1, spp, frame0, stride, mode,
                      counters, order, cost);
   return hipGetLastError();
@@ -464,6 +475,24 @@
 
 }
 
+extern "C" int ptgs_debug_pt_occupancy(unsigned int instantiation, unsigned int out[7]) {
+  const void* k = (const void*)ptgs::pt_camera_instantiation((instantiation & 4u) != 0, (instantiation & 2u) != 0,
+                                                             (instantiation & 1u) != 0);
+  int blocks = 0;
+  hipError_t e = hipOccupancyMaxActiveBlocksPerMultiprocessor(&blocks, k, PTGS_PT_WG, 0);
+  if (e) return (int)e;
+  hipFuncAttributes fa;
+  if ((e = hipFuncGetAttributes(&fa, k))) return (int)e;
+  out[0] = (unsigned int)blocks;
+  out[1] = (unsigned int)fa.sharedSizeBytes;
+  out[2] = (unsigned int)fa.numRegs;
+  out[3] = (unsigned int)fa.localSizeBytes;
+  out[4] = (unsigned int)ptgs::pt_lds_stack((instantiation & 1u) != 0);
+  out[5] = (instantiation & 1u) ? PTGS_PT_DEEP_MIN_WAVES : PTGS_PT_MIN_WAVES;
+  out[6] = PTGS_PT_WG;
+  return 0;
+}
+
 #ifdef PT_LANES
 extern "C" int ptgs_debug_pt_lanes(unsigned long long* host, unsigned int n) {
   if (n > 2u * ptgs::PT_L_COUNT) n = 2u * ptgs::PT_L_COUNT;
diff --git a/pathtracer_gaussiansplatting_amd/renderer.py b/pathtracer_gaussiansplatting_amd/renderer.py
--- a/pathtracer_gaussiansplatting_amd/renderer.py
+++ b/pathtracer_gaussiansplatting_amd/renderer.py
@@ -99,6 +99,12 @@
         t = SceneTreeOpt()
         self._chk(self.lib.ptgs_scene_get_tree_opt(self._h, C.byref(t)), "ptgs_scene_get_tree_opt")
         return t
+
+    def scene_pt_stack(self) -> tuple:
+        lds, need, deep = C.c_uint32(), C.c_uint32(), C.c_uint32()
+        self._chk(self.lib.ptgs_scene_get_pt_stack(self._h, C.byref(lds), C.byref(need), C.byref(deep)),
+                  "ptgs_scene_get_pt_stack")
+        return lds.value, need.value, bool(deep.value)
 
     def trace_camera(self, ubo: Ubo, width: int, height: int, accum, spp: int = 1, frame_stride: int = 1,
                      mode: int = _abi.ACCUM_RUNNING_MEAN, rows: tuple | None = None, stream=None):
```

Result: faster. 7122 Mrays/s, median of 6 (+2.6%).
